# 1pathplanningzzj/pointnet_refine

Hardware: AMD Instinct MI355X
Metric: lane segments/sec (fwd+bwd) at B=4096,N=1024; HBM GB/s vs roofline (higher is better)
Workload: dtype f32 (large GEMMs: 2xfp16-split MFMA, 3 products, fp32 accumulate); 1 GPU; LineRefineNet training step (fwd + deep-supervision L1 + bwd + Adam), B=4096/GPU, N=1024, M=32, C=4; global_batch=4096, points=1024, parallelism=dp1, decoder_chunk=4096

## Files before the change

### include/pointnet_refine_hip.h

```cpp
#ifndef POINTNET_REFINE_HIP_H
#define POINTNET_REFINE_HIP_H

#include <stddef.h>
#include <stdint.h>

#ifdef __cplusplus
extern "C" {
#endif

#define PRH_OK 0
#define PRH_ERR_ARG (-1)
#define PRH_ERR_WORKSPACE (-2)
#define PRH_ERR_HIP (-3)

#define PRH_MAX_LAYERS 8

typedef struct {
  const float* w;
  const float* b;
  const float* gamma;
  const float* beta;
  float* running_mean;
  float* running_var;
  int64_t* num_batches_tracked;
// ... 47 lines not shown
                         int training, float* d_fused, const float* d_gfeat, int d_fused_scratch,
                         const prh_encoder_saved* saved, const prh_encoder_grads* grads,
                         float* d_ctx, void* workspace, size_t workspace_bytes, int device,
                         void* stream);

typedef struct {
  uint16_t* z_cat;
  uint16_t* z_fus;
  uint16_t* gate;
  float* bn_scale;
  float* bn_shift;
  float* bn_mean;
  float* bn_rstd;
  int32_t* argmax;
} prh_encoder_saved_bf16;
size_t prh_encoder_bf16_workspace_bytes(int B, int N, int in_channel, int out_dim, int backward);
int prh_encoder_forward_bf16(const prh_encoder_params* prm, const float* ctx, int B, int N, int training,
                             float momentum, float eps, uint16_t* fused, float* gfeat,
                             const prh_encoder_saved_bf16* saved, void* workspace, size_t workspace_bytes,
                             int device, void* stream);
int prh_encoder_backward_bf16(const prh_encoder_params* prm, const float* ctx, int B, int N, int training,
                              const uint16_t* d_fused, const float* d_gfeat, const prh_encoder_saved_bf16* saved,
                              const prh_encoder_grads* grads, float* d_ctx, void* workspace,
                              size_t workspace_bytes, int device, void* stream);
size_t prh_linear_bf16_workspace_bytes(int rows, int k, int n, int backward);
int prh_linear_forward_bf16(const uint16_t* x, long ldx, const float* w, const float* b, float* y, int rows, int k,
                            int n, int relu, void* workspace, size_t workspace_bytes, int device, void* stream);
int prh_linear_backward_bf16(const uint16_t* x, long ldx, const float* w, const float* dy, uint16_t* dx, float* dw,
                             float* db, int rows, int k, int n, void* workspace, size_t workspace_bytes, int device,
                             void* stream);

int prh_cast_perm_bf16(const float* src, long ld, uint16_t* dst, long rows, int device, void* stream);
int prh_posmem_images(const float* xyz, long ldx, const float* w0, const float* b0, const float* w2, const float* b2,
                      const float* memory, long ldm, long rows, uint16_t* x16, uint16_t* y16, int device, void* stream);
int prh_attn_fold_forward(const float* q, long ldq, const uint16_t* x16, const uint16_t* y16, const float* wk, long ldwk,
                          const float* wv, long ldwv, const float* bv, float* o, long ldo, int B, int M, int N, int H,
                          float scale, int device, void* stream);
int prh_linear_forward_out16(const float* x, long ldx, const float* w, const float* b, uint16_t* y, int rows, int k,
                             int n, void* workspace, size_t workspace_bytes, int device, void* stream);
int prh_linear_backward_dy16(const float* x, long ldx, const float* w, const uint16_t* dy, float* dx, float* dw,
                             float* db, int rows, int k, int n, void* workspace, size_t workspace_bytes, int device,
                             void* stream);
int prh_attn_forward_kv16(const float* q, long ldq, const uint16_t* k, long ldk, const uint16_t* v, long ldv, float* o,
                          long ldo, float* lse, int B, int M, int N, int H, float scale, float dropout_p,
                          unsigned seed, int device, void* stream);
int prh_attn_backward_kv16(const float* q, long ldq, const uint16_t* k, long ldk, const uint16_t* v, long ldv,
                           const float* o, long ldo, const float* lse, const float* dout, long lddo, float* dq,
                           long lddq, uint16_t* dk, long lddk, uint16_t* dv, long lddv, int B, int M, int N, int H,
                           float scale, float dropout_p, unsigned seed, int device, void* stream);

size_t prh_encoder_fused_image_bytes(int planes, int in_channel);
int prh_encoder_fused_prepare(const prh_encoder_params* prm, float eps, const float* proj_w, const float* proj_b,
                              int planes, void* image, size_t image_bytes, int device, void* stream);
size_t prh_encoder_fused_workspace_bytes(int B, int N, int planes);
int prh_encoder_fused_forward(const void* image, int planes, int in_channel, int has_proj, const float* ctx, int B,
                              int N, float* memory, float* fused, float* gfeat, unsigned* saturated, void* workspace,
                              size_t workspace_bytes, int device, void* stream);

size_t prh_linear_forward_workspace_bytes(int rows, int k, int n);
int prh_linear_forward(const float* x, long ldx, const float* w, const float* b, float* y,
                       int rows, int k, int n, int relu, void* workspace, size_t workspace_bytes,
                       int device, void* stream);

int prh_linear_forward_ex(const float* x, long ldx, const float* w, const float* b, float* y,
                          int rows, int k, int n, int relu, const float* x_amax, void* workspace,
                          size_t workspace_bytes, int device, void* stream);

int prh_linear_forward_full(const float* x, long ldx, const float* w, const float* b, const float* resid,
                            long ldres, float* y, int rows, int k, int n, int relu, const float* x_amax,
                            const float* w_amax, float dropout_p, unsigned dropout_seed, void* workspace,
                            size_t workspace_bytes, int device, void* stream);

int prh_linear_forward_amax(const float* x, long ldx, const float* w, const float* b, const float* resid,
                            long ldres, float* y, int rows, int k, int n, int relu, const float* x_amax,
                            const float* w_amax, float dropout_p, unsigned dropout_seed, float* y_amax_out,
                            void* workspace, size_t workspace_bytes, int device, void* stream);

size_t prh_operand_absmax_workspace_bytes(void);
int prh_operand_absmax(const float* x, long ld, long rows, int cols, float* out, void* workspace,
                       size_t workspace_bytes, int device, void* stream);
int prh_relu_mask_absmax(const float* dy, const float* y, float* out, long n, float scale, float* amax_out,
                         void* workspace, size_t workspace_bytes, int device, void* stream);
int prh_linear_uses_operand_maxima(int rows, int k, int n);

int prh_pos_hidden_forward(const float* xyz, long ld, const float* w0, const float* b0, float* h,
                           long rows, int hidden, int device, void* stream);
size_t prh_pos_hidden_forward_workspace_bytes(void);
int prh_pos_hidden_forward_amax(const float* xyz, long ld, const float* w0, const float* b0, float* h,
                                long rows, int hidden, float* h_amax_out, void* workspace, size_t workspace_bytes,
                                int device, void* stream);
size_t prh_pos_hidden_backward_workspace_bytes(long rows, int hidden);
int prh_pos_hidden_backward(const float* xyz, long ld, const float* h, const float* dh, const float* w0,
                            float* dxyz, float* dw0, float* db0, long rows, int hidden, void* workspace,
                            size_t workspace_bytes, int device, void* stream);

int prh_linear_small_forward(const float* x, const float* w, const float* b, float* y, long rows, int k,
                             int n, int device, void* stream);
size_t prh_linear_small_backward_workspace_bytes(long rows, int k, int n);
int prh_linear_small_backward(const float* x, const float* w, const float* dy, float* dx, float* dw,
                              float* db, long rows, int k, int n, void* workspace, size_t workspace_bytes,
                              int device, void* stream);

size_t prh_linear_backward_workspace_bytes(int rows, int k, int n);
int prh_linear_backward(const float* x, long ldx, const float* w, const float* dy, float* dx,
                        float* dw, float* db, int rows, int k, int n, void* workspace,
                        size_t workspace_bytes, int device, void* stream);

int prh_linear_backward_ex(const float* x, long ldx, const float* w, const float* dy, float* dx,
                           float* dw, float* db, int rows, int k, int n, const float* x_amax,
                           const float* dy_amax, void* workspace, size_t workspace_bytes, int device,
                           void* stream);
int prh_linear_backward_full(const float* x, long ldx, const float* w, const float* dy, float* dx,
                             float* dw, float* db, int rows, int k, int n, const float* x_amax,
                             const float* dy_amax, const float* w_amax, void* workspace,
                             size_t workspace_bytes, int device, void* stream);
int prh_linear_backward_amax(const float* x, long ldx, const float* w, const float* dy, float* dx,
                             float* dw, float* db, int rows, int k, int n, const float* x_amax,
                             const float* dy_amax, const float* w_amax, int dx_accumulate, float* dx_amax_out,
                             void* workspace, size_t workspace_bytes, int device, void* stream);

size_t prh_mlp_stack_workspace_bytes(int P, int n_layers, const prh_bn_layer* layers);
int prh_mlp_stack_forward(const prh_bn_layer* layers, int n_layers, int relu_last,
                          const float* x, int P, int training, float momentum, float eps,
                          float* z_cat, float* y, float* bn_scale, float* bn_shift,
                          float* bn_mean, float* bn_rstd, void* workspace,
                          size_t workspace_bytes, int device, void* stream);
int prh_mlp_stack_backward(const prh_bn_layer* layers, int n_layers, int relu_last,
                           const float* x, int P, int training, const float* dy,
                           const float* z_cat, const float* bn_scale, const float* bn_shift,
                           const float* bn_mean, const float* bn_rstd,
                           const prh_bn_layer_grad* grads, float* dx, void* workspace,
                           size_t workspace_bytes, int device, void* stream);

int prh_attn_forward(const float* q, long ldq, const float* k, long ldk, const float* v, long ldv,
                     float* o, long ldo, float* lse, int B, int M, int N, int H, float scale,
                     float dropout_p, unsigned seed, int device, void* stream);
int prh_attn_backward(const float* q, long ldq, const float* k, long ldk, const float* v, long ldv,
                      const float* o, long ldo, const float* lse, const float* dout, long lddo,
                      float* dq, long lddq, float* dk, long lddk, float* dv, long lddv, int B, int M,
                      int N, int H, float scale, float dropout_p, unsigned seed, int device,
                      void* stream);

size_t prh_context_workspace_bytes(int npts, int n_lines, int max_candidates);
int prh_context_build(const float* cloud, int npts, const float* dense, int n_dense, const float* line,
                      int m, int n_lines, float radius, float decay_scale, int n_samples,
                      int max_candidates, unsigned long long seed, float* out, int32_t* counts,
                      float* dbg_weights, void* workspace, size_t workspace_bytes, int device,
                      void* stream);

size_t prh_context_ragged_workspace_bytes(int n_lines, long long n_items);
int prh_context_ragged_count(const float* points, const long long* slice_offsets, int n_slices, const float* dense,
                             int n_dense, const int* line_slice, const unsigned long long* slice_seed, int n_lines,
                             float radius, int32_t* counts, long long* cand_offsets, void* workspace,
                             size_t workspace_bytes, int device, void* stream);
int prh_context_ragged_select(const float* points, const long long* slice_offsets, int n_slices, const float* dense,
                              int n_dense, const float* line, int m, const int* line_slice, int n_lines, float radius,
                              float decay_scale, int n_samples, const int32_t* counts, const long long* cand_offsets,
                              int line0, int line1, int* cand, unsigned* keys, long long cand_capacity, float* out,
                              void* workspace, size_t workspace_bytes, int device, void* stream);

int prh_line_metrics(const double* noisy, const double* refined, int n_lines, int m, const double* gt,
                     const long long* gt_offsets, int n_gt, const int* gt_index, int* info, double* resampled,
                     double* metrics, int device, void* stream);
size_t prh_shift_sweep_workspace_bytes(int n_pred, int n_gt, int n_shifts);
int prh_shift_sweep(const double* pred, int n_pred, const double* gt, int n_gt, const double* shifts, int n_shifts,
                    double* out, void* workspace, size_t workspace_bytes, int device, void* stream);

size_t prh_shift_sweep_ragged_workspace_bytes(const long long* pred_offsets, const long long* shift_offsets,
                                              int n_problems);
int prh_shift_sweep_ragged(const double* pred, const long long* pred_offsets, const double* gt,
                           const long long* gt_offsets, int n_gt_sets, const int* gt_index, const double* shifts,
                           const long long* shift_offsets, int n_problems, double* out, void* workspace,
                           size_t workspace_bytes, int device, void* stream);

size_t prh_drive_slice_workspace_bytes(int npts, int n_slices);
int prh_drive_slice_count(const float* cloud, int npts, const double* poses, int n_slices, double segment_len,
                          double radius, long long* offsets, void* workspace, size_t workspace_bytes, int device,
                          void* stream);
int prh_drive_slice_write(const float* cloud, int npts, const double* poses, int n_slices, double segment_len,
                          double radius, const long long* offsets, double* points, long long* source_index,
                          long long capacity, void* workspace, size_t workspace_bytes, int device, void* stream);
size_t prh_drive_clip_workspace_bytes(int n_slices);
int prh_drive_clip_count(const double* lines, const long long* line_offsets, int n_lines, const double* poses,
                         int n_slices, double segment_len, int* counts, void* workspace, size_t workspace_bytes,
                         int device, void* stream);
int prh_drive_clip_write(const double* lines, const long long* line_offsets, int n_lines, const double* poses,
                         int n_slices, double segment_len, const long long* out_offsets, double* out,
                         void* workspace, size_t workspace_bytes, int device, void* stream);
size_t prh_drive_noise_workspace_bytes(int n_lines);
int prh_drive_noise(const double* lines, const long long* line_offsets, const int* vertex_line, long long n_verts,
                    int n_lines, const int* line_ids, const double* scales, int n_scales, unsigned long long seed,
                    int draw, double* draws_u, double* draws_j, double* out, void* workspace,
                    size_t workspace_bytes, int device, void* stream);

int prh_pcd_group_rows(void);
size_t prh_pcd_format_workspace_bytes(long long n_rows);
int prh_pcd_format_count(const void* points, int is_fp64, long long n_rows, unsigned char* row_bytes,
                         int* group_bytes, long long* status, void* workspace, size_t workspace_bytes, int device,
                         void* stream);
int prh_pcd_format_write(const void* points, int is_fp64, long long n_rows, const unsigned char* row_bytes,
                         const long long* group_offsets, const long long* offsets, int n_slices,
                         unsigned char* text, long long capacity, long long* byte_offsets, int device,
// ... 178 lines not shown
```

### pointnet_refine_amd/_lib.py

```python
from __future__ import annotations

import ctypes as C
import os
import subprocess
import threading

_HERE = os.path.dirname(os.path.abspath(__file__))
_ROOT = os.path.dirname(_HERE)
LIB_PATH = os.environ.get("PRH_LIB_PATH") or os.path.join(_HERE, "libpointnet_refine_hip.so")
_CSRC = os.path.join(_HERE, "csrc")
_SOURCES = [os.path.join(_CSRC, "prh_lib.hip")] + (sorted(
    os.path.join(_CSRC, f) for f in os.listdir(_CSRC) if f.endswith((".hpp", ".h", ".hip")) and f != "prh_lib.hip")
    if os.path.isdir(_CSRC) else [])
_HEADER = os.path.join(_ROOT, "include", "pointnet_refine_hip.h")

PRH_MAX_LAYERS = 8


class BnLayer(C.Structure):
    _fields_ = [("w", C.c_void_p), ("b", C.c_void_p), ("gamma", C.c_void_p), ("beta", C.c_void_p),
                ("running_mean", C.c_void_p), ("running_var", C.c_void_p),
                ("num_batches_tracked", C.c_void_p), ("cin", C.c_int), ("cout", C.c_int)]


class BnLayerGrad(C.Structure):
    _fields_ = [("dw", C.c_void_p), ("db", C.c_void_p), ("dgamma", C.c_void_p), ("dbeta", C.c_void_p)]


class EncoderParams(C.Structure):
    _fields_ = [("in_channel", C.c_int), ("out_dim", C.c_int), ("conv", BnLayer * 5),
                ("fusion", BnLayer), ("gate_w1", C.c_void_p), ("gate_b1", C.c_void_p),
                ("gate_w2", C.c_void_p), ("gate_b2", C.c_void_p)]


class EncoderGrads(C.Structure):
    _fields_ = [("conv", BnLayerGrad * 5), ("fusion", BnLayerGrad), ("d_gate_w1", C.c_void_p),
                ("d_gate_b1", C.c_void_p), ("d_gate_w2", C.c_void_p), ("d_gate_b2", C.c_void_p)]


class EncoderSaved(C.Structure):
    _fields_ = [("z_cat", C.c_void_p), ("z_fus", C.c_void_p), ("gate", C.c_void_p),
                ("bn_scale", C.c_void_p), ("bn_shift", C.c_void_p), ("bn_mean", C.c_void_p),
                ("bn_rstd", C.c_void_p), ("argmax", C.c_void_p), ("op_amax", C.c_void_p)]


class EncoderSavedBf16(C.Structure):
    _fields_ = [("z_cat", C.c_void_p), ("z_fus", C.c_void_p), ("gate", C.c_void_p),
                ("bn_scale", C.c_void_p), ("bn_shift", C.c_void_p), ("bn_mean", C.c_void_p),
                ("bn_rstd", C.c_void_p), ("argmax", C.c_void_p)]


EXPORTS = [
    "prh_encoder_workspace_bytes", "prh_encoder_forward", "prh_encoder_backward",
    "prh_encoder_bf16_workspace_bytes", "prh_encoder_forward_bf16", "prh_encoder_backward_bf16",
    "prh_linear_bf16_workspace_bytes", "prh_linear_forward_bf16", "prh_linear_backward_bf16",
    "prh_linear_forward_out16", "prh_linear_backward_dy16", "prh_attn_forward_kv16", "prh_attn_backward_kv16",
    "prh_encoder_fused_image_bytes", "prh_encoder_fused_prepare", "prh_encoder_fused_workspace_bytes",
    "prh_encoder_fused_forward",
    "prh_linear_forward_workspace_bytes", "prh_linear_forward", "prh_linear_forward_ex",
    "prh_linear_forward_full", "prh_linear_forward_amax", "prh_operand_absmax_workspace_bytes", "prh_operand_absmax",
    "prh_linear_uses_operand_maxima", "prh_linear_backward_full", "prh_linear_backward_amax", "prh_pos_hidden_forward",
    "prh_pos_hidden_forward_workspace_bytes", "prh_pos_hidden_forward_amax", "prh_pos_hidden_backward_workspace_bytes",
    "prh_pos_hidden_backward", "prh_linear_small_forward", "prh_linear_small_backward_workspace_bytes",
    "prh_linear_small_backward",
    "prh_linear_backward_workspace_bytes", "prh_linear_backward", "prh_linear_backward_ex",
    "prh_mlp_stack_workspace_bytes", "prh_mlp_stack_forward", "prh_mlp_stack_backward",
    "prh_test_gemm_nt", "prh_test_gemm_tn_workspace_bytes", "prh_test_gemm_tn",
    "prh_test_gemm_tn_side_workspace_bytes", "prh_test_gemm_tn_side", "prh_test_xcc_map",
    "prh_profile_enable", "prh_profile_count", "prh_profile_reset", "prh_profile_read",
    "prh_attn_forward", "prh_attn_backward", "prh_attn_backward_ex",
    "prh_context_workspace_bytes", "prh_context_build",
    "prh_context_ragged_workspace_bytes", "prh_context_ragged_count", "prh_context_ragged_select",
    "prh_line_metrics", "prh_shift_sweep_workspace_bytes", "prh_shift_sweep",
    "prh_shift_sweep_ragged_workspace_bytes", "prh_shift_sweep_ragged",
    "prh_drive_slice_workspace_bytes", "prh_drive_slice_count", "prh_drive_slice_write",
    "prh_drive_clip_workspace_bytes", "prh_drive_clip_count", "prh_drive_clip_write",
    "prh_drive_noise_workspace_bytes", "prh_drive_noise",
    "prh_match_clip_workspace_bytes", "prh_match_clip_count", "prh_match_clip_write",
    "prh_match_costs_workspace_bytes", "prh_match_costs", "prh_match_max_side", "prh_match_assign",
    "prh_bev_bounds_workspace_bytes", "prh_bev_bounds", "prh_bev_raster", "prh_bev_select_workspace_bytes",
    "prh_bev_select", "prh_bev_tone", "prh_bev_colorize", "prh_bev_crop", "prh_bev_tile", "prh_bev_draw_count",
    "prh_bev_draw_workspace_bytes", "prh_bev_draw",
    "prh_view_bounds_workspace_bytes", "prh_view_bounds", "prh_view_clear", "prh_view_max_views", "prh_view_splat",
    "prh_view_lines", "prh_view_resolve",
    "prh_fuse_max_points", "prh_fuse_tile", "prh_fuse_project_workspace_bytes", "prh_fuse_project",
    "prh_fuse_gather_workspace_bytes", "prh_fuse_gather",
    "prh_link_tile", "prh_link_pairs_per_block", "prh_link_pairs_workspace_bytes", "prh_link_pairs_count",
    "prh_link_pairs_write", "prh_link_stats",
    "prh_link_cum", "prh_link_edges_blocks", "prh_link_edges", "prh_link_edges_compact", "prh_link_label_round",
    "prh_link_tree_init", "prh_link_tree_level",
    "prh_support_max_cells", "prh_support_accumulate",
    "prh_pcd_group_rows", "prh_pcd_format_workspace_bytes", "prh_pcd_format_count", "prh_pcd_format_write",
    "prh_pcd_index_blocks", "prh_pcd_index_count", "prh_pcd_index_write", "prh_pcd_parse_workspace_bytes",
    "prh_pcd_parse", "prh_pcd_unpack14",
    "prh_l1_loss_workspace_bytes", "prh_l1_loss", "prh_adam_step",
    "prh_add_dropout_layernorm_forward", "prh_add_dropout_layernorm_workspace_bytes",
    "prh_add_dropout_layernorm_backward",
    "prh_relu_mask_absmax", "prh_cast_perm_bf16", "prh_posmem_images", "prh_attn_fold_forward", "prh_set_gemm_mode", "prh_get_gemm_mode", "prh_set_dropout_seed_source",
    "prh_last_error", "prh_version",
]

_lock = threading.Lock()
_lib = None


def needs_build() -> bool:
    if not os.path.exists(LIB_PATH):
        return True
    t = os.path.getmtime(LIB_PATH)
    return any(os.path.exists(s) and os.path.getmtime(s) > t for s in _SOURCES + [_HEADER])


def build(force: bool = False, verbose: bool = False) -> str:
    if not force and not needs_build():
        return LIB_PATH
    hipcc = os.environ.get("HIPCC", "/opt/rocm/bin/hipcc")
    cmd = [hipcc, "--offload-arch=gfx950", "-O3", "-std=c++17", "-shared", "-fPIC",
           "-o", LIB_PATH, _SOURCES[0]]
    if verbose:
        print(" ".join(cmd))
    subprocess.run(cmd, check=True)
    return LIB_PATH


def _bind(lib):
    vp, i, f, sz, lg = C.c_void_p, C.c_int, C.c_float, C.c_size_t, C.c_long
    lib.prh_last_error.restype = C.c_char_p
    lib.prh_version.restype = C.c_char_p
    lib.prh_encoder_workspace_bytes.restype = sz
    lib.prh_encoder_workspace_bytes.argtypes = [i, i, i, i, i]
    lib.prh_encoder_forward.restype = i
    lib.prh_encoder_forward.argtypes = [C.POINTER(EncoderParams), vp, i, i, i, f, f, vp, vp,
                                        C.POINTER(EncoderSaved), vp, sz, i, vp]
    lib.prh_encoder_backward.restype = i
    lib.prh_encoder_backward.argtypes = [C.POINTER(EncoderParams), vp, i, i, i, vp, vp, i,
                                         C.POINTER(EncoderSaved), C.POINTER(EncoderGrads), vp, vp,
                                         sz, i, vp]
    lib.prh_encoder_bf16_workspace_bytes.restype = sz
    lib.prh_encoder_bf16_workspace_bytes.argtypes = [i, i, i, i, i]
    lib.prh_encoder_forward_bf16.restype = i
    lib.prh_encoder_forward_bf16.argtypes = [C.POINTER(EncoderParams), vp, i, i, i, f, f, vp, vp,
                                             C.POINTER(EncoderSavedBf16), vp, sz, i, vp]
    lib.prh_encoder_backward_bf16.restype = i
    lib.prh_encoder_backward_bf16.argtypes = [C.POINTER(EncoderParams), vp, i, i, i, vp, vp,
                                              C.POINTER(EncoderSavedBf16), C.POINTER(EncoderGrads), vp, vp,
                                              sz, i, vp]
    lib.prh_linear_bf16_workspace_bytes.restype = sz
    lib.prh_linear_bf16_workspace_bytes.argtypes = [i, i, i, i]
    lib.prh_linear_forward_bf16.restype = i
    lib.prh_linear_forward_bf16.argtypes = [vp, lg, vp, vp, vp, i, i, i, i, vp, sz, i, vp]
    lib.prh_linear_backward_bf16.restype = i
    lib.prh_linear_backward_bf16.argtypes = [vp, lg, vp, vp, vp, vp, vp, i, i, i, vp, sz, i, vp]
    lib.prh_linear_forward_out16.restype = i
    lib.prh_linear_forward_out16.argtypes = [vp, lg, vp, vp, vp, i, i, i, vp, sz, i, vp]
    lib.prh_linear_backward_dy16.restype = i
    lib.prh_linear_backward_dy16.argtypes = [vp, lg, vp, vp, vp, vp, vp, i, i, i, vp, sz, i, vp]
    lib.prh_attn_forward_kv16.restype = i
    lib.prh_attn_forward_kv16.argtypes = [vp, lg, vp, lg, vp, lg, vp, lg, vp, i, i, i, i, f, f, C.c_uint, i, vp]
    lib.prh_attn_backward_kv16.restype = i
    lib.prh_attn_backward_kv16.argtypes = [vp, lg, vp, lg, vp, lg, vp, lg, vp, vp, lg, vp, lg, vp, lg, vp, lg,
                                           i, i, i, i, f, f, C.c_uint, i, vp]
    lib.prh_encoder_fused_image_bytes.restype = sz
    lib.prh_encoder_fused_image_bytes.argtypes = [i, i]
    lib.prh_encoder_fused_prepare.restype = i
    lib.prh_encoder_fused_prepare.argtypes = [C.POINTER(EncoderParams), f, vp, vp, i, vp, sz, i, vp]
    lib.prh_encoder_fused_workspace_bytes.restype = sz
    lib.prh_encoder_fused_workspace_bytes.argtypes = [i, i, i]
    lib.prh_encoder_fused_forward.restype = i
    lib.prh_encoder_fused_forward.argtypes = [vp, i, i, i, vp, i, i, vp, vp, vp, vp, vp, sz, i, vp]
    lib.prh_linear_forward.restype = i
    lib.prh_linear_forward.argtypes = [vp, lg, vp, vp, vp, i, i, i, i, vp, sz, i, vp]
    lib.prh_linear_forward_ex.restype = i
    lib.prh_linear_forward_ex.argtypes = [vp, lg, vp, vp, vp, i, i, i, i, vp, vp, sz, i, vp]
    lib.prh_linear_forward_full.restype = i
    lib.prh_linear_forward_full.argtypes = [vp, lg, vp, vp, vp, lg, vp, i, i, i, i, vp, vp, f, C.c_uint, vp, sz, i, vp]
    lib.prh_linear_forward_amax.restype = i
    lib.prh_linear_forward_amax.argtypes = [vp, lg, vp, vp, vp, lg, vp, i, i, i, i, vp, vp, f, C.c_uint, vp, vp, sz, i, vp]
    lib.prh_linear_backward_amax.restype = i
    lib.prh_linear_backward_amax.argtypes = [vp, lg, vp, vp, vp, vp, vp, i, i, i, vp, vp, vp, i, vp, vp, sz, i, vp]
    lib.prh_pos_hidden_forward_workspace_bytes.restype = sz
    lib.prh_pos_hidden_forward_workspace_bytes.argtypes = []
    lib.prh_pos_hidden_forward_amax.restype = i
    lib.prh_pos_hidden_forward_amax.argtypes = [vp, lg, vp, vp, vp, lg, i, vp, vp, sz, i, vp]
    lib.prh_operand_absmax_workspace_bytes.restype = sz
    lib.prh_operand_absmax_workspace_bytes.argtypes = []
    lib.prh_operand_absmax.restype = i
    lib.prh_operand_absmax.argtypes = [vp, lg, lg, i, vp, vp, sz, i, vp]
    lib.prh_linear_uses_operand_maxima.restype = i
    lib.prh_linear_uses_operand_maxima.argtypes = [i, i, i]
    lib.prh_linear_backward_full.restype = i
    lib.prh_linear_backward_full.argtypes = [vp, lg, vp, vp, vp, vp, vp, i, i, i, vp, vp, vp, vp, sz, i, vp]
    lib.prh_pos_hidden_forward.restype = i
    lib.prh_pos_hidden_forward.argtypes = [vp, lg, vp, vp, vp, lg, i, i, vp]
    lib.prh_pos_hidden_backward_workspace_bytes.restype = sz
    lib.prh_pos_hidden_backward_workspace_bytes.argtypes = [lg, i]
    lib.prh_pos_hidden_backward.restype = i
    lib.prh_pos_hidden_backward.argtypes = [vp, lg, vp, vp, vp, vp, vp, vp, lg, i, vp, sz, i, vp]
    lib.prh_linear_small_forward.restype = i
    lib.prh_linear_small_forward.argtypes = [vp, vp, vp, vp, lg, i, i, i, vp]
    lib.prh_linear_small_backward_workspace_bytes.restype = sz
    lib.prh_linear_small_backward_workspace_bytes.argtypes = [lg, i, i]
    lib.prh_linear_small_backward.restype = i
    lib.prh_linear_small_backward.argtypes = [vp, vp, vp, vp, vp, vp, lg, i, i, vp, sz, i, vp]
    lib.prh_linear_backward_ex.restype = i
    lib.prh_linear_backward_ex.argtypes = [vp, lg, vp, vp, vp, vp, vp, i, i, i, vp, vp, vp, sz, i, vp]
    lib.prh_linear_forward_workspace_bytes.restype = sz
    lib.prh_linear_forward_workspace_bytes.argtypes = [i, i, i]
    lib.prh_linear_backward_workspace_bytes.restype = sz
    lib.prh_linear_backward_workspace_bytes.argtypes = [i, i, i]
    lib.prh_linear_backward.restype = i
    lib.prh_linear_backward.argtypes = [vp, lg, vp, vp, vp, vp, vp, i, i, i, vp, sz, i, vp]
    lib.prh_mlp_stack_workspace_bytes.restype = sz
    lib.prh_mlp_stack_workspace_bytes.argtypes = [i, i, C.POINTER(BnLayer)]
    lib.prh_mlp_stack_forward.restype = i
    lib.prh_mlp_stack_forward.argtypes = [C.POINTER(BnLayer), i, i, vp, i, i, f, f, vp, vp, vp, vp,
                                          vp, vp, vp, sz, i, vp]
    lib.prh_mlp_stack_backward.restype = i
    lib.prh_mlp_stack_backward.argtypes = [C.POINTER(BnLayer), i, i, vp, i, i, vp, vp, vp, vp, vp,
                                           vp, C.POINTER(BnLayerGrad), vp, vp, sz, i, vp]
    lib.prh_attn_forward.restype = i
    lib.prh_attn_forward.argtypes = [vp, lg, vp, lg, vp, lg, vp, lg, vp, i, i, i, i, f, f, C.c_uint, i, vp]
    lib.prh_attn_backward.restype = i
    lib.prh_attn_backward.argtypes = [vp, lg, vp, lg, vp, lg, vp, lg, vp, vp, lg, vp, lg, vp, lg, vp, lg,
                                      i, i, i, i, f, f, C.c_uint, i, vp]
    lib.prh_context_workspace_bytes.restype = C.c_size_t
    lib.prh_context_workspace_bytes.argtypes = [i, i, i]
    lib.prh_context_build.restype = i
    lib.prh_context_build.argtypes = [vp, i, vp, i, vp, i, i, f, f, i, i, C.c_ulonglong, vp, vp, vp, vp,
                                      C.c_size_t, i, vp]
    lib.prh_context_ragged_workspace_bytes.restype = sz
    lib.prh_context_ragged_workspace_bytes.argtypes = [i, C.c_longlong]
    lib.prh_context_ragged_count.restype = i
    lib.prh_context_ragged_count.argtypes = [vp, vp, i, vp, i, vp, vp, i, f, vp, vp, vp, sz, i, vp]
    lib.prh_context_ragged_select.restype = i
    lib.prh_context_ragged_select.argtypes = [vp, vp, i, vp, i, vp, i, vp, i, f, f, i, vp, vp, i, i, vp, vp,
                                              C.c_longlong, vp, vp, sz, i, vp]
    lib.prh_line_metrics.restype = i
    lib.prh_line_metrics.argtypes = [vp, vp, i, i, vp, vp, i, vp, vp, vp, vp, i, vp]
    lib.prh_shift_sweep_workspace_bytes.restype = sz
    lib.prh_shift_sweep_workspace_bytes.argtypes = [i, i, i]
    lib.prh_shift_sweep.restype = i
    lib.prh_shift_sweep.argtypes = [vp, i, vp, i, vp, i, vp, vp, sz, i, vp]
    lib.prh_shift_sweep_ragged_workspace_bytes.restype = sz
    lib.prh_shift_sweep_ragged_workspace_bytes.argtypes = [vp, vp, i]
    lib.prh_shift_sweep_ragged.restype = i
    lib.prh_shift_sweep_ragged.argtypes = [vp, vp, vp, vp, i, vp, vp, vp, i, vp, vp, sz, i, vp]
    ll, dbl = C.c_longlong, C.c_double
    lib.prh_drive_slice_workspace_bytes.restype = sz
    lib.prh_drive_slice_workspace_bytes.argtypes = [i, i]
    lib.prh_drive_slice_count.restype = i
    lib.prh_drive_slice_count.argtypes = [vp, i, vp, i, dbl, dbl, vp, vp, sz, i, vp]
    lib.prh_drive_slice_write.restype = i
    lib.prh_drive_slice_write.argtypes = [vp, i, vp, i, dbl, dbl, vp, vp, vp, ll, vp, sz, i, vp]
    lib.prh_drive_clip_workspace_bytes.restype = sz
    lib.prh_drive_clip_workspace_bytes.argtypes = [i]
    lib.prh_drive_clip_count.restype = i
    lib.prh_drive_clip_count.argtypes = [vp, vp, i, vp, i, dbl, vp, vp, sz, i, vp]
    lib.prh_drive_clip_write.restype = i
    lib.prh_drive_clip_write.argtypes = [vp, vp, i, vp, i, dbl, vp, vp, vp, sz, i, vp]
    lib.prh_drive_noise_workspace_bytes.restype = sz
    lib.prh_drive_noise_workspace_bytes.argtypes = [i]
    lib.prh_drive_noise.restype = i
# ... 188 lines not shown
```

### pointnet_refine_amd/csrc/prh_gemm.hpp

```cpp
#pragma once
#include <hip/hip_runtime.h>
#include <type_traits>
#include <stdint.h>

namespace prh {

typedef float f32x16 __attribute__((ext_vector_type(16)));

enum { PRO_NONE = 0, PRO_BNRELU = 1, PRO_BNBWD = 2, PRO_GATE1 = 3 };
enum { EPI_BIAS = 0, EPI_BIAS_STATS = 1, EPI_GATE = 2, EPI_DGRAD = 3 };

enum {
  F_RELU_OUT = 1,
  F_ACCUM = 2,
  F_MASK = 4,
  F_STATS = 8,
  F_STORE_GATE = 16,
  F_E1_ROWVEC = 32,
  F_RESID = 64,
  F_DROPOUT = 256,
  F_POOL = 128,
};

struct NTParams {
// ... 271 lines not shown
                                              int mrows, int rb, int lane, const float* biasp) {
  const int q = lane >> 4, l15 = lane & 15;
#pragma unroll
  for (int nb = 0; nb < 4; ++nb) {
    const int col = cbase + nb * 16 + l15;
    const bool cok = col < p.N;
    const float bias = (biasp != nullptr && cok) ? biasp[col] : 0.f;
    float s = 0.f;
#pragma unroll
    for (int mb = 0; mb < MB; ++mb)
#pragma unroll
      for (int r = 0; r < 4; ++r)
        if (mb * 16 + q * 4 + r < mrows) s += acc[mb][nb][r] + bias;
    s += __shfl_xor(s, 16);
    s += __shfl_xor(s, 32);
    const int nrows = mrows < 0 ? 0 : (mrows > MB * 16 ? MB * 16 : mrows);
    const float mean = nrows > 0 ? s / (float)nrows : 0.f;
    float m2 = 0.f;
#pragma unroll
    for (int mb = 0; mb < MB; ++mb)
#pragma unroll
      for (int r = 0; r < 4; ++r) {
        const float dlt = acc[mb][nb][r] + bias - mean;
        if (mb * 16 + q * 4 + r < mrows) m2 = fmaf(dlt, dlt, m2);
      }
    m2 += __shfl_xor(m2, 16);
    m2 += __shfl_xor(m2, 32);
    if (q == 0 && cok) {
      p.ws_a[(size_t)rb * p.N + col] = s;
      p.ws_b[(size_t)rb * p.N + col] = m2;
    }
    if (p.ws_c != nullptr) {
      float mx = -3.0e38f, mn = 3.0e38f;
#pragma unroll
      for (int mb = 0; mb < MB; ++mb)
#pragma unroll
        for (int r = 0; r < 4; ++r)
          if (mb * 16 + q * 4 + r < mrows) {
            mx = fmaxf(mx, acc[mb][nb][r] + bias); mn = fminf(mn, acc[mb][nb][r] + bias);
          }
      mx = fmaxf(fmaxf(mx, __shfl_xor(mx, 16)), 0.f - 3.0e38f);
      mx = fmaxf(mx, __shfl_xor(mx, 32));
      mn = fminf(mn, __shfl_xor(mn, 16));
      mn = fminf(mn, __shfl_xor(mn, 32));
      if (q == 0 && cok) {
        p.ws_c[(size_t)rb * p.N + col] = mx;
        p.ws_d[(size_t)rb * p.N + col] = mn;
      }
    }
  }
}

__device__ __forceinline__ unsigned pack_bf16x2(float a, float b) {
  typedef float v2f __attribute__((ext_vector_type(2)));
  typedef __bf16 v2b __attribute__((ext_vector_type(2)));
  v2f v = {a, b};
  v2b h = __builtin_convertvector(v, v2b);
  return __builtin_bit_cast(unsigned, h);
}
__device__ __forceinline__ float bf16_lo(unsigned u) { return __uint_as_float(u << 16); }
__device__ __forceinline__ float bf16_hi(unsigned u) { return __uint_as_float(u & 0xffff0000u); }
__device__ __forceinline__ float bf16_round(float x) { return bf16_lo(pack_bf16x2(x, 0.f)); }
template <bool H>
__device__ __forceinline__ float4 ld4e(const char* base, int off) {
  if (H) {
    const uint2 u = *reinterpret_cast<const uint2*>(base + (size_t)off * 2);
    return make_float4(bf16_lo(u.x), bf16_hi(u.x), bf16_lo(u.y), bf16_hi(u.y));
  }
  return *reinterpret_cast<const float4*>(base + (size_t)off * 4);
}
template <bool H>
__device__ __forceinline__ void st4e(char* base, int off, float4 v) {
  if (H) *reinterpret_cast<uint2*>(base + (size_t)off * 2) = make_uint2(pack_bf16x2(v.x, v.y), pack_bf16x2(v.z, v.w));
  else *reinterpret_cast<float4*>(base + (size_t)off * 4) = v;
}

typedef char* __restrict__ epi_wptr_r;
typedef const char* __restrict__ epi_rptr_r;
template <int EPI, int MT, class ACC, bool C16, bool AMAX = false>
__device__ __forceinline__ void nt_epilogue_vec_r2(ACC& acc, const NTParams& p, int rbase_,
                                                int cbase, int rb, int lane, float* scratch,
                                                bool bias_done = false,
                                                float* wave_amax = nullptr) {
  static_assert(!AMAX || (EPI == EPI_BIAS && !C16), "output maximum: EPI_BIAS with fp32 storage");
  typedef typename std::conditional<AMAX, char*, epi_wptr_r>::type wptr;
  typedef typename std::conditional<AMAX, const char*, epi_rptr_r>::type rptr;
  const int rbase = __builtin_amdgcn_readfirstlane(rbase_);
  const float* biasp = bias_done ? nullptr : p.bias;
  constexpr int ES = C16 ? 2 : 4;
  const bool rowvec = EPI == EPI_DGRAD && (p.flags & F_E1_ROWVEC) != 0;
  const int ees = (C16 && !rowvec) ? 2 : 4;
  wptr Cb = reinterpret_cast<char*>(p.C) + (size_t)rbase * p.ldc * ES;
  rptr Eb = p.E1 != nullptr ? reinterpret_cast<const char*>(p.E1) + (size_t)rbase * p.lde1 * ees : nullptr;
  const int ldc = (int)p.ldc, lde1 = (int)p.lde1;
  const int mrows = p.M - rbase;
  const int rr = lane >> 4, c4 = (lane & 15) * 4;
  const int col4 = cbase + c4;
  const bool c4ok = col4 < p.N;
  float4 bias4 = zero4(), es4 = zero4(), et4 = zero4();
  if (c4ok) {
    if (biasp != nullptr) bias4 = ldg4(biasp + col4);
    if ((EPI == EPI_DGRAD && (p.flags & F_MASK) != 0) || EPI == EPI_GATE) {
      es4 = ldg4(p.es + col4);
      et4 = ldg4(p.et + col4);
    }
  }
  char* __restrict__ C2b = (EPI == EPI_GATE && p.C2 != nullptr) ? reinterpret_cast<char*>(p.C2) + (size_t)rbase * p.ldc2 * ES : nullptr;
  const int ldc2 = (int)p.ldc2;

  if (EPI == EPI_BIAS_STATS) epi_col_stats(acc, p, cbase, mrows, rb, lane, biasp);

  const bool mask = (p.flags & F_MASK) != 0, accum = (p.flags & F_ACCUM) != 0;
  const bool stats = EPI == EPI_DGRAD && (p.flags & F_STATS) != 0;
  const bool resid = EPI == EPI_BIAS && (p.flags & F_RESID) != 0;
  const unsigned dseed = (EPI == EPI_BIAS && (p.flags & F_DROPOUT) != 0) ? epi_seed(p) : 0u;
  const bool need_z = (EPI == EPI_DGRAD && (mask || stats)) || EPI == EPI_GATE || resid;
  float4 s1 = zero4(), s2 = zero4();
  const bool pool = EPI == EPI_GATE && (p.flags & F_POOL) != 0;
  float pmx[4] = {-1.f, -1.f, -1.f, -1.f}, psm[4] = {0.f, 0.f, 0.f, 0.f};
  int pix[4] = {0, 0, 0, 0};
  const int col4c = col4 < p.N ? col4 : (p.N - 4);
  rptr Cl = mrows > 0 ? Cb : reinterpret_cast<const char*>(p.C);
  rptr El = mrows > 0 ? Eb : reinterpret_cast<const char*>(p.E1);
  const bool acc_old = EPI == EPI_DGRAD && accum;
  float amx = 0.f;
  constexpr int NB = 2 * MT;
  float4 zz[2][4], oo[2][4];
  auto issue = [&](int b, float4 (&z)[4], float4 (&o)[4]) {
    const char* Em = El; const char* Cm = Cl;
    asm volatile("" : "+s"(Em), "+s"(Cm) : : "memory");
    int lrc[4];
#pragma unroll
    for (int i = 0; i < 4; ++i) {
      z[i] = zero4(); o[i] = zero4();
      int r = (b >> 1) * 32 + ((b & 1) * 4 + i) * 4 + rr;
      r = r < mrows ? r : mrows - 1;
      lrc[i] = r < 0 ? 0 : r;
    }
    if (need_z) {
      if (rowvec) {
#pragma unroll
        for (int i = 0; i < 4; ++i) {
          const float s = *reinterpret_cast<const float*>(Em + (size_t)(lrc[i] * lde1) * 4);
          z[i] = make_float4(s, s, s, s);
        }
      } else {
#pragma unroll
        for (int i = 0; i < 4; ++i) z[i] = ld4e<C16>(Em, lrc[i] * lde1 + col4c);
      }
    }
    if (acc_old) {
#pragma unroll
      for (int i = 0; i < 4; ++i) o[i] = ld4e<C16>(Cm, lrc[i] * ldc + col4c);
    }
  };
  issue(0, zz[0], oo[0]);
#pragma unroll
  for (int b = 0; b < NB; ++b) {
    const int mt = b >> 1, hb = b & 1;
    if (b + 1 < NB) issue(b + 1, zz[(b + 1) & 1], oo[(b + 1) & 1]);
    if (hb == 0) epi_block_to_scratch(acc, mt, scratch, lane);
#pragma unroll
    for (int i = 0; i < 4; ++i) {
      const int it = hb * 4 + i;
      const int lrow = it * 4 + rr;
      const int lr = mt * 32 + lrow;
      const bool ok = lr < mrows && c4ok;
      float4 v = *reinterpret_cast<const float4*>(scratch + lrow * EPI_LDW + c4);
      v.x += bias4.x; v.y += bias4.y; v.z += bias4.z; v.w += bias4.w;
      const float4 z = zz[b & 1][i];
      const float4 o = oo[b & 1][i];
      if (EPI == EPI_DGRAD) {
        v.x += o.x; v.y += o.y; v.z += o.z; v.w += o.w;
        if (mask) {
          v.x = fmaf(z.x, es4.x, et4.x) > 0.f ? v.x : 0.f;
          v.y = fmaf(z.y, es4.y, et4.y) > 0.f ? v.y : 0.f;
          v.z = fmaf(z.z, es4.z, et4.z) > 0.f ? v.z : 0.f;
          v.w = fmaf(z.w, es4.w, et4.w) > 0.f ? v.w : 0.f;
        }
        if (C16) {
          v.x = bf16_round(v.x); v.y = bf16_round(v.y); v.z = bf16_round(v.z); v.w = bf16_round(v.w);
        }
        const float4 q = ok ? v : zero4();
        s1.x += q.x; s1.y += q.y; s1.z += q.z; s1.w += q.w;
        s2.x = fmaf(q.x, z.x, s2.x); s2.y = fmaf(q.y, z.y, s2.y);
        s2.z = fmaf(q.z, z.z, s2.z); s2.w = fmaf(q.w, z.w, s2.w);
      } else if (EPI == EPI_GATE) {
        float4 m;
        m.x = 0.5f + 0.5f / (1.f + __expf(-v.x)); m.y = 0.5f + 0.5f / (1.f + __expf(-v.y));
        m.z = 0.5f + 0.5f / (1.f + __expf(-v.z)); m.w = 0.5f + 0.5f / (1.f + __expf(-v.w));
        v.x = fmaxf(fmaf(z.x, es4.x, et4.x), 0.f) * m.x; v.y = fmaxf(fmaf(z.y, es4.y, et4.y), 0.f) * m.y;
        v.z = fmaxf(fmaf(z.z, es4.z, et4.z), 0.f) * m.z; v.w = fmaxf(fmaf(z.w, es4.w, et4.w), 0.f) * m.w;
        if (ok && (p.flags & F_STORE_GATE) != 0) st4e<C16>(C2b, lr * ldc2 + col4, m);
        if (pool && ok) {
          if (C16) { v.x = bf16_round(v.x); v.y = bf16_round(v.y); v.z = bf16_round(v.z); v.w = bf16_round(v.w); }
          const float vv[4] = {v.x, v.y, v.z, v.w};
#pragma unroll
          for (int e = 0; e < 4; ++e) {
            if (vv[e] > pmx[e]) { pmx[e] = vv[e]; pix[e] = lr; }
            psm[e] += vv[e];
          }
        }
      } else {
        if (resid) { v.x += z.x; v.y += z.y; v.z += z.z; v.w += z.w; }
        if ((p.flags & F_RELU_OUT) != 0) {
          v.x = fmaxf(v.x, 0.f); v.y = fmaxf(v.y, 0.f); v.z = fmaxf(v.z, 0.f); v.w = fmaxf(v.w, 0.f);
        }
        if (EPI == EPI_BIAS && (p.flags & F_DROPOUT) != 0) {
          const unsigned rw = (unsigned)(rbase + lr), c0 = (unsigned)col4;
          v.x = epi_keep(dseed, rw, c0, p.drop_thresh) ? v.x * p.drop_scale : 0.f;
          v.y = epi_keep(dseed, rw, c0 + 1, p.drop_thresh) ? v.y * p.drop_scale : 0.f;
          v.z = epi_keep(dseed, rw, c0 + 2, p.drop_thresh) ? v.z * p.drop_scale : 0.f;
          v.w = epi_keep(dseed, rw, c0 + 3, p.drop_thresh) ? v.w * p.drop_scale : 0.f;
        }
      }
      if (ok) st4e<C16>(Cb, lr * ldc + col4, v);
      if (AMAX && ok) amx = fmaxf(fmaxf(amx, fmaxf(fabsf(v.x), fabsf(v.y))), fmaxf(fabsf(v.z), fabsf(v.w)));
    }
    if (EPI == EPI_DGRAD)
      asm volatile("" : "+v"(s1.x), "+v"(s1.y), "+v"(s1.z), "+v"(s1.w), "+v"(s2.x), "+v"(s2.y), "+v"(s2.z), "+v"(s2.w));
  }
  if (pool) {
#pragma unroll
    for (int e = 0; e < 4; ++e)
#pragma unroll
      for (int o = 16; o <= 32; o <<= 1) {
        const float ov = __shfl_xor(pmx[e], o);
        const int oi = __shfl_xor(pix[e], o);
        psm[e] += __shfl_xor(psm[e], o);
        if (ov > pmx[e] || (ov == pmx[e] && oi < pix[e])) { pmx[e] = ov; pix[e] = oi; }
      }
    if (lane < 16 && c4ok) {
      *reinterpret_cast<float4*>(p.ws_a + (size_t)rb * p.N + col4) = make_float4(pmx[0], pmx[1], pmx[2], pmx[3]);
      *reinterpret_cast<float4*>(p.ws_b + (size_t)rb * p.N + col4) = make_float4(psm[0], psm[1], psm[2], psm[3]);
      *reinterpret_cast<int4*>(p.ws_c + (size_t)rb * p.N + col4) = make_int4(pix[0], pix[1], pix[2], pix[3]);
    }
  }
  if (stats) {
    s1.x += __shfl_xor(s1.x, 16); s1.y += __shfl_xor(s1.y, 16); s1.z += __shfl_xor(s1.z, 16); s1.w += __shfl_xor(s1.w, 16);
    s2.x += __shfl_xor(s2.x, 16); s2.y += __shfl_xor(s2.y, 16); s2.z += __shfl_xor(s2.z, 16); s2.w += __shfl_xor(s2.w, 16);
    s1.x += __shfl_xor(s1.x, 32); s1.y += __shfl_xor(s1.y, 32); s1.z += __shfl_xor(s1.z, 32); s1.w += __shfl_xor(s1.w, 32);
    s2.x += __shfl_xor(s2.x, 32); s2.y += __shfl_xor(s2.y, 32); s2.z += __shfl_xor(s2.z, 32); s2.w += __shfl_xor(s2.w, 32);
    if (lane < 16 && c4ok) {
      *reinterpret_cast<float4*>(p.ws_a + (size_t)rb * p.N + col4) = s1;
      *reinterpret_cast<float4*>(p.ws_b + (size_t)rb * p.N + col4) = s2;
    }
  }
  if (AMAX) {
#pragma unroll
    for (int o = 32; o > 0; o >>= 1) amx = fmaxf(amx, __shfl_xor(amx, o));
    *wave_amax = amx;
  }
}

template <int EPI, int MT, class ACC, bool C16 = false, bool AMAX = false>
__device__ __forceinline__ void nt_epilogue_vec(ACC& acc, const NTParams& p, int rbase_,
                                                int cbase, int rb, int lane, float* scratch,
                                                bool bias_done = false,
                                                float* wave_amax = nullptr) {
  if constexpr (!C16) {
    nt_epilogue_vec_r2<EPI, MT, ACC, false, AMAX>(acc, p, rbase_, cbase, rb, lane, scratch, bias_done, wave_amax);
    return;
  }
  const int rbase = __builtin_amdgcn_readfirstlane(rbase_);
  const float* biasp = bias_done ? nullptr : p.bias;
  constexpr int ES = C16 ? 2 : 4;
  const bool rowvec = EPI == EPI_DGRAD && (p.flags & F_E1_ROWVEC) != 0;
  const int ees = (C16 && !rowvec) ? 2 : 4;
  char* __restrict__ Cb = reinterpret_cast<char*>(p.C) + (size_t)rbase * p.ldc * ES;
  const char* __restrict__ Eb = p.E1 != nullptr ? reinterpret_cast<const char*>(p.E1) + (size_t)rbase * p.lde1 * ees : nullptr;
  const int ldc = (int)p.ldc, lde1 = (int)p.lde1;
  const int mrows = p.M - rbase;
  const int rr = lane >> 4, c4 = (lane & 15) * 4;
  const int col4 = cbase + c4;
  const bool c4ok = col4 < p.N;
  float4 bias4 = zero4(), es4 = zero4(), et4 = zero4();
  if (c4ok) {
    if (biasp != nullptr) bias4 = ldg4(biasp + col4);
    if ((EPI == EPI_DGRAD && (p.flags & F_MASK) != 0) || EPI == EPI_GATE) {
      es4 = ldg4(p.es + col4);
      et4 = ldg4(p.et + col4);
    }
  }
  char* __restrict__ C2b = (EPI == EPI_GATE && p.C2 != nullptr) ? reinterpret_cast<char*>(p.C2) + (size_t)rbase * p.ldc2 * ES : nullptr;
  const int ldc2 = (int)p.ldc2;

  if (EPI == EPI_BIAS_STATS) epi_col_stats(acc, p, cbase, mrows, rb, lane, biasp);

  const bool mask = (p.flags & F_MASK) != 0, accum = (p.flags & F_ACCUM) != 0;
  const bool stats = EPI == EPI_DGRAD && (p.flags & F_STATS) != 0;
  const bool resid = EPI == EPI_BIAS && (p.flags & F_RESID) != 0;
  const unsigned dseed = (EPI == EPI_BIAS && (p.flags & F_DROPOUT) != 0) ? epi_seed(p) : 0u;
  const bool need_z = (EPI == EPI_DGRAD && (mask || stats)) || EPI == EPI_GATE || resid;
  float4 s1 = zero4(), s2 = zero4();
  const bool pool = EPI == EPI_GATE && (p.flags & F_POOL) != 0;
  float pmx[4] = {-1.f, -1.f, -1.f, -1.f}, psm[4] = {0.f, 0.f, 0.f, 0.f};
  int pix[4] = {0, 0, 0, 0};
  const bool acc_old = EPI == EPI_DGRAD && accum;
  const int vrows = mrows < 0 ? 0 : (mrows > 32 * MT ? 32 * MT : mrows);
  auto mkrs = [&](const void* base, long ld, int es_, int width) {
    const long ext = (base != nullptr && vrows > 0) ? ((long)(vrows - 1) * ld + width) * es_ : 0;
    return __builtin_amdgcn_make_buffer_rsrc(const_cast<void*>(base), 0, (int)ext, 0x00020000);
// ... 402 lines not shown
```

### pointnet_refine_amd/csrc/prh_gemm_h2.hpp

```cpp
#pragma once
#include "prh_gemm_s3.hpp"

namespace prh {

constexpr int H2_BK = 32;
constexpr int H2_PLANE = 256 * H2_BK * 2;
constexpr int H2_OPER = 2 * H2_PLANE;
constexpr int H2_STAGE = 2 * H2_OPER;
constexpr int H2_LDS = 2 * H2_STAGE;

__device__ __forceinline__ int h2_off(int row, int k) {
  return row * 64 + ((((k >> 3) ^ (-(row >> 2))) & 3) << 4) + ((k & 7) << 1);
}

inline size_t h2_weight_bytes(int N, int K) {
  return S3_WHDR + (size_t)((N + 255) / 256) * ((K + H2_BK - 1) / H2_BK) * H2_OPER;
}

__global__ __launch_bounds__(256) void prep_weights_h2_kernel(const float* __restrict__ W, int N,
                                                              int K, long ldw, char* __restrict__ out,
                                                              const float* __restrict__ amax) {
  const int KT = (K + H2_BK - 1) / H2_BK;
  const int NT_ = (N + 255) / 256;
  const long total = (long)NT_ * 256 * KT * 4;
  const long i = (long)blockIdx.x * blockDim.x + threadIdx.x;
  if (i >= total) return;
  const int chunk = (int)(i & 3);
  long t = i >> 2;
  const int k_tile = (int)(t % KT); t /= KT;
  const int row = (int)(t & 255);
  const int n_tile = (int)(t >> 8);
  const int n = n_tile * 256 + row;
  const float S = pow2_scale(load_amax(amax));
  float v[8];
#pragma unroll
  for (int j = 0; j < 8; ++j) {
    const int k = k_tile * H2_BK + chunk * 8 + j;
    v[j] = (n < N && k < K) ? W[(size_t)n * ldw + k] * S : 0.f;
  }
  uint4 h, l;
  split2h(v[0], v[1], h.x, l.x);
  split2h(v[2], v[3], h.y, l.y);
  split2h(v[4], v[5], h.z, l.z);
  split2h(v[6], v[7], h.w, l.w);
  char* base = out + ((size_t)n_tile * KT + k_tile) * H2_OPER + h2_off(row, chunk * 8);
  *reinterpret_cast<uint4*>(base) = h;
  *reinterpret_cast<uint4*>(base + H2_PLANE) = l;
}

template <int I0 = 0, int I1 = 8>
__device__ __forceinline__ void h2_compute(f32x4 (&acc)[8][4], const char* st, int wm, int wn, int l15,
                                           int kc) {
  f16x8 wh[4], wl[4];
#pragma unroll
  for (int j = 0; j < 4; ++j) {
    const char* q = st + H2_OPER + h2_off(wn + j * 16 + l15, kc * 8);
    wh[j] = *reinterpret_cast<const f16x8*>(q);
    wl[j] = *reinterpret_cast<const f16x8*>(q + H2_PLANE);
  }
#pragma unroll
  for (int i = I0; i < I1; ++i) {
    const char* q = st + h2_off(wm + i * 16 + l15, kc * 8);
    const f16x8 ah = *reinterpret_cast<const f16x8*>(q);
    const f16x8 al = *reinterpret_cast<const f16x8*>(q + H2_PLANE);
#pragma unroll
    for (int j = 0; j < 4; ++j) {
      acc[i][j] = __builtin_amdgcn_mfma_f32_16x16x32_f16(al, wh[j], acc[i][j], 0, 0, 0);
      acc[i][j] = __builtin_amdgcn_mfma_f32_16x16x32_f16(ah, wl[j], acc[i][j], 0, 0, 0);
      acc[i][j] = __builtin_amdgcn_mfma_f32_16x16x32_f16(ah, wh[j], acc[i][j], 0, 0, 0);
    }
  }
}

template <int PRO, int EPI, bool PP = false, bool AMAX = false>
__global__ __launch_bounds__(512, 2) void gemm_nt_h2_kernel(const NTParams p,
                                                            const char* __restrict__ Wp) {
  static_assert(PRO == PRO_NONE || PRO == PRO_BNRELU || PRO == PRO_GATE1, "prologue not supported");
  static_assert(!AMAX || (PRO == PRO_NONE && EPI == EPI_BIAS), "output maximum: plain EPI_BIAS launches only");
  extern __shared__ __attribute__((aligned(16))) char smem[];
#ifdef PRH_STAMP
  unsigned t_acc[4] = {0u, 0u, 0u, 0u};
  unsigned long long t_prev = __builtin_amdgcn_s_memtime();
#endif
  const int tid = threadIdx.x, lane = tid & 63, wave = tid >> 6;
  const int l15 = lane & 15, kc = lane >> 4;
  const int wm = (wave >> 2) * 128, wn = (wave & 3) * 64;
  const int vb = xcd_remap(blockIdx.x, gridDim.x);
  const int tile_n = vb % p.tiles_n, tile_m = vb / p.tiles_n;
  const int m0 = tile_m * 256, n0 = tile_n * 256;
  const int KT = (p.K + H2_BK - 1) / H2_BK;

  const int sc = (tid & 7) * 4;
  const int sr = tid >> 3;
  const int KP = (KT + 2) * H2_BK;
  float* coef = reinterpret_cast<float*>(smem + H2_LDS);
  const float sA = pow2_scale(load_amax(p.amaxA));
  const float unscale = 1.f / (sA * pow2_scale(load_amax(p.amaxW)));

  f32x4 acc[8][4];
#pragma unroll
  for (int i = 0; i < 8; ++i)
#pragma unroll
    for (int j = 0; j < 4; ++j)
#pragma unroll
      for (int r = 0; r < 4; ++r) acc[i][j][r] = 0.f;

  float4 ra[2][4];
  const char* wsrc = Wp + (size_t)tile_n * KT * H2_OPER + tid * 16;
  const unsigned lds0 = (unsigned)(unsigned long)((__attribute__((address_space(3))) char*)smem);
  const unsigned wdst = __builtin_amdgcn_readfirstlane(lds0 + H2_OPER + wave * 1024);
  auto dma_w = [&](int kt, int stage) {
    const char* q = wsrc + (size_t)(kt < KT ? kt : KT - 1) * H2_OPER;
#pragma unroll
    for (int pc = 0; pc < 4; ++pc) glds16(q + pc * 8192, wdst + stage * H2_STAGE + pc * 8192);
  };
  constexpr int NA = PRO == PRO_GATE1 ? 0 : 4;
  int arows = p.M - m0; arows = arows > 256 ? 256 : arows;
  const __amdgpu_buffer_rsrc_t rsA = __builtin_amdgcn_make_buffer_rsrc(
      (void*)(p.A + (size_t)m0 * p.lda), 0,
      PRO == PRO_GATE1 ? 0 : (int)(((size_t)(arows - 1) * p.lda + p.K) * 4), 0x00020000);
  int voA[4];
  float gi[4] = {0.f, 0.f, 0.f, 0.f};
#pragma unroll
  for (int j = 0; j < 4; ++j) {
    voA[j] = ((sr + 64 * j) * (int)p.lda + sc) * 4;
    if (PRO == PRO_GATE1) {
      const int row = m0 + sr + 64 * j;
      gi[j] = row < p.M ? p.A[(size_t)row * p.lda] : 0.f;
    }
  }
  auto load_tile = [&](int kt, float4 (&r)[4]) {
    if (PRO == PRO_GATE1) return;
    const int so = kt * (H2_BK * 4);
#pragma unroll
    for (int j = 0; j < 4; ++j)
      r[j] = __builtin_bit_cast(float4, __builtin_amdgcn_raw_buffer_load_b128(rsA, voA[j] + so, 0, 0));
  };
  auto store_tile = [&](int kt, char* st, const float4 (&r_)[4]) {
    const int k = kt * H2_BK + sc;
    const bool kok = k < p.K || PRO != PRO_NONE;
    float4 ka = zero4(), kb = zero4();
    if (PRO != PRO_NONE) {
      ka = *reinterpret_cast<const float4*>(coef + k);
      kb = *reinterpret_cast<const float4*>(coef + KP + k);
    }
#pragma unroll
    for (int j = 0; j < 4; ++j) {
      const int r = sr + 64 * j;
      float4 v;
      if (PRO == PRO_GATE1) v = pro_apply<PRO>(make_float4(gi[j], 0.f, 0.f, 0.f), zero4(), ka, kb, zero4());
      else v = pro_apply<PRO>(r_[j], zero4(), ka, kb, zero4());
      v.x = kok ? v.x : 0.f; v.y = kok ? v.y : 0.f; v.z = kok ? v.z : 0.f; v.w = kok ? v.w : 0.f;
      if (PRO == PRO_NONE) { v.x *= sA; v.y *= sA; v.z *= sA; v.w *= sA; }
      uint2 h, l;
      split2h(v.x, v.y, h.x, l.x);
      split2h(v.z, v.w, h.y, l.y);
      char* q = st + h2_off(r, sc);
      *reinterpret_cast<uint2*>(q) = h;
      *reinterpret_cast<uint2*>(q + H2_PLANE) = l;
    }
  };
// ... 478 lines not shown
```

### pointnet_refine_amd/csrc/prh_kernels.hpp

```cpp
#pragma once
#include <hip/hip_runtime.h>
#include <stdint.h>

namespace prh {

constexpr int BN_SLICES = 32;

__global__ __launch_bounds__(256) void bn_stage1_kernel(const float* __restrict__ ws_a,
                                                        const float* __restrict__ ws_b, int R,
                                                        long ld, int N, int tile_rows, int P,
                                                        int forward, double* __restrict__ out) {
  __shared__ double red[3][8][33];
  const int c = threadIdx.x & 31, g = threadIdx.x >> 5;
  const int col = blockIdx.x * 32 + c, sl = blockIdx.y;
  const int per = (R + BN_SLICES - 1) / BN_SLICES;
  const int r0 = sl * per, r1 = (r0 + per < R) ? r0 + per : R;
  const bool ok = col < N;
  double a = 0.0, b = 0.0, n = 0.0;
  if (ok)
    for (int i = r0 + g; i < r1; i += 8) {
      a += (double)ws_a[(size_t)i * ld + col];
      if (forward) {
        int ni = P - i * tile_rows;
        ni = ni > tile_rows ? tile_rows : (ni < 0 ? 0 : ni);
// ... 62 lines not shown
    running_var[col] = (float)((1.0 - momentum) * (double)running_var[col] + momentum * unb);
  }
}

__global__ __launch_bounds__(256) void act_amax_kernel(const float* __restrict__ ws_c,
                                                       const float* __restrict__ ws_d, int R, long ld, int N,
                                                       const float* __restrict__ scale,
                                                       const float* __restrict__ shift,
                                                       float* __restrict__ part) {
  __shared__ float red[256];
  const int c = threadIdx.x & 31, g = threadIdx.x >> 5;
  const int sl = blockIdx.y;
  const int per = (R + BN_SLICES - 1) / BN_SLICES;
  const int r0 = sl * per, r1 = (r0 + per < R) ? r0 + per : R;
  float a = 0.f;
  for (int col = blockIdx.x * 32 + c; col < N; col += gridDim.x * 32) {
    float mx = -3.0e38f, mn = 3.0e38f;
    for (int i = r0 + g; i < r1; i += 8) {
      mx = fmaxf(mx, ws_c[(size_t)i * ld + col]);
      mn = fminf(mn, ws_d[(size_t)i * ld + col]);
    }
    if (mx >= mn) {
      const float sc = scale[col], sh = shift[col];
      a = fmaxf(a, fmaxf(fmaf(mx, sc, sh), fmaf(mn, sc, sh)));
    }
  }
  red[threadIdx.x] = a;
  __syncthreads();
  for (int s = 128; s > 0; s >>= 1) {
    if (threadIdx.x < s) red[threadIdx.x] = fmaxf(red[threadIdx.x], red[threadIdx.x + s]);
    __syncthreads();
  }
  if (threadIdx.x == 0) part[blockIdx.y * gridDim.x + blockIdx.x] = red[0];
}
__global__ void max_of_kernel(const float* __restrict__ v, int n, float* __restrict__ out) {
  float m = 0.f;
  for (int i = 0; i < n; ++i) m = fmaxf(m, v[i]);
  *out = m;
}

__global__ void bn_eval_coeffs_kernel(const float* gamma, const float* beta, const float* rm,
                                      const float* rv, float eps, int N, float* mean_out,
                                      float* rstd_out, float* scale_out, float* shift_out) {
  const int c = blockIdx.x * blockDim.x + threadIdx.x;
  if (c >= N) return;
  const float rstd = 1.0f / sqrtf(rv[c] + eps);
  const float sc = gamma[c] * rstd;
  mean_out[c] = rm[c];
  rstd_out[c] = rstd;
  scale_out[c] = sc;
  shift_out[c] = beta[c] - rm[c] * sc;
}

__global__ void bn_bwd_finalize_kernel(const double* __restrict__ sl, int P, int N,
                                       const float* __restrict__ gamma,
                                       const float* __restrict__ mean,
                                       const float* __restrict__ rstd, int training, float* ca,
                                       float* cb, float* cc, float* dgamma, float* dbeta,
                                       float* dbias) {
  const int col = blockIdx.x * blockDim.x + threadIdx.x;
  if (col >= N) return;
  double Sdy = 0.0, Sdyz = 0.0;
  for (int s = 0; s < BN_SLICES; ++s) {
    const double* r = sl + ((size_t)s * 3) * N;
    Sdy += r[col];
    Sdyz += r[(size_t)N + col];
  }
  const double mu = mean[col], rs = rstd[col], gm = gamma[col];
  const double dg = (Sdyz - mu * Sdy) * rs;
  if (dgamma != nullptr) dgamma[col] = (float)dg;
  if (dbeta != nullptr) dbeta[col] = (float)Sdy;
  double a = gm * rs, b = 0.0, cst = 0.0;
  if (training) {
    const double m1 = Sdy / (double)P, m2 = dg / (double)P;
    b = -a * m2 * rs;
    cst = a * (m2 * mu * rs - m1);
  }
  ca[col] = (float)a;
  cb[col] = (float)b;
  cc[col] = (float)cst;
  if (dbias != nullptr) dbias[col] = (float)(a * Sdy + b * (double)P * mu + cst * (double)P);
}

__global__ __launch_bounds__(1024) void partials_reduce_kernel(
    const float* __restrict__ ws_a, const float* __restrict__ ws_b, int R2, int N, float* out_a,
    float* out_b) {
  __shared__ double red[2][32][33];
  const int c = threadIdx.x & 31, g = threadIdx.x >> 5;
  const int col = blockIdx.x * 32 + c;
  const bool ok = col < N;
  double s1 = 0.0, s2 = 0.0;
  if (ok)
    for (int i = g; i < R2; i += 32) {
      s1 += (double)ws_a[(size_t)i * N + col];
      if (ws_b != nullptr) s2 += (double)ws_b[(size_t)i * N + col];
    }
  red[0][g][c] = s1;
  red[1][g][c] = s2;
  __syncthreads();
  if (g == 0 && ok) {
    double a = 0.0, b = 0.0;
    for (int j = 0; j < 32; ++j) {
      a += red[0][j][c];
      b += red[1][j][c];
    }
    if (out_a != nullptr) out_a[col] = (float)a;
    if (out_b != nullptr) out_b[col] = (float)b;
  }
}

__global__ __launch_bounds__(256) void pool_kernel(const float* __restrict__ F, int N, int C,
                                                   float* gfeat, int32_t* argmax) {
  __shared__ float smax[4][64];
  __shared__ int sidx[4][64];
  __shared__ float ssum[4][64];
  const int c = threadIdx.x & 63, g = threadIdx.x >> 6;
  const int col = blockIdx.x * 64 + c, b = blockIdx.y;
  float mx = -INFINITY, sum = 0.f;
  int ix = 0;
  if (col < C) {
    const float* base = F + (size_t)b * N * C + col;
    for (int n = g; n < N; n += 4) {
      const float v = base[(size_t)n * C];
      sum += v;
      if (v > mx) { mx = v; ix = n; }
    }
  }
  smax[g][c] = mx; sidx[g][c] = ix; ssum[g][c] = sum;
  __syncthreads();
  if (g == 0 && col < C) {
    for (int j = 1; j < 4; ++j) {
      const float v = smax[j][c];
      const int i2 = sidx[j][c];
      if (v > mx || (v == mx && i2 < ix)) { mx = v; ix = i2; }
      sum += ssum[j][c];
    }
    gfeat[(size_t)b * 2 * C + col] = mx;
    gfeat[(size_t)b * 2 * C + C + col] = sum / (float)N;
    if (argmax != nullptr) argmax[(size_t)b * C + col] = ix;
  }
}

__global__ __launch_bounds__(256) void pool_tiles_kernel(const float* __restrict__ pmax,
                                                         const float* __restrict__ psum,
                                                         const int* __restrict__ pidx, int tiles_per_seg,
                                                         int N, int C, float* gfeat, int32_t* argmax) {
  const int col = blockIdx.x * 256 + threadIdx.x, b = blockIdx.y;
  if (col >= C) return;
  float mx = -INFINITY, sum = 0.f;
  int ix = 0;
  for (int t = 0; t < tiles_per_seg; ++t) {
    const size_t o = ((size_t)b * tiles_per_seg + t) * C + col;
    const float v = pmax[o];
    if (v > mx) { mx = v; ix = t * 128 + pidx[o]; }
    sum += psum[o];
  }
  gfeat[(size_t)b * 2 * C + col] = mx;
  gfeat[(size_t)b * 2 * C + C + col] = sum / (float)N;
  if (argmax != nullptr) argmax[(size_t)b * C + col] = ix;
}

__global__ __launch_bounds__(256) void combine_bwd_kernel(
    const float* dF, const float* __restrict__ d_gfeat, const int32_t* __restrict__ argmax,
    const float* __restrict__ zf, float* gate, const float* __restrict__ s,
    const float* __restrict__ t, int P, int N, int C, float* dy_out, float* ws_a, float* ws_b) {
  __shared__ float r1[4][64], r2[4][64];
  const int c = threadIdx.x & 63, g = threadIdx.x >> 6;
  const int col = blockIdx.y * 64 + c;
  const int row0 = blockIdx.x * 64 + g * 16;
  float s1 = 0.f, s2 = 0.f;
  if (col < C) {
    const float sc = s[col], sh = t[col];
    for (int i = 0; i < 16; ++i) {
      const int row = row0 + i;
      if (row >= P) break;
      const size_t off = (size_t)row * C + col;
      float d = dF != nullptr ? dF[off] : 0.f;
      if (d_gfeat != nullptr) {
// ... 613 lines not shown
```

### pointnet_refine_amd/csrc/prh_lib.hip

```cpp
#include "../../include/pointnet_refine_hip.h"

#include <hip/hip_runtime.h>
#include <stdarg.h>
#include <stdio.h>
#include <string.h>

#include <mutex>
#include <vector>

#include <stdlib.h>

#include "prh_gemm.hpp"
#include "prh_attn.hpp"
#include "prh_attn16.hpp"
#include "prh_gemm_s3.hpp"
#include "prh_gemm_h2.hpp"
#include "prh_b16.hpp"
#include "prh_small.hpp"
#include "prh_attnfold.hpp"
#include "prh_fused.hpp"
#include "prh_context.hpp"
#include "prh_metrics.hpp"
#include "prh_drive.hpp"
#include "prh_match.hpp"
// ... 55 lines not shown
    r = &g_prof.recs[g_prof.used++];
    snprintf(r->name, sizeof(r->name), "%s", name);
    r->flops = flops; r->bytes = bytes;
    (void)hipEventRecord(r->e0, st);
  }
  ~ProfScope() { if (r) (void)hipEventRecord(r->e1, st); }
};

inline size_t align_up(size_t x, size_t a) { return (x + a - 1) / a * a; }
inline int cdiv(long a, long b) { return (int)((a + b - 1) / b); }

struct Arena {
  char* base; size_t size; size_t off = 0; bool ok = true;
  Arena(void* b, size_t s) : base((char*)b), size(s) {}
  Arena() : base(nullptr), size((size_t)-1) {}
  float* f(size_t n) {
    off = align_up(off, 256);
    const size_t bytes = n * sizeof(float);
    if (base != nullptr && off + bytes > size) { ok = false; return nullptr; }
    float* p = base ? (float*)(base + off) : nullptr;
    off += bytes;
    return p;
  }
};

const unsigned* g_seed_src = nullptr;
int g_gemm_mode = -1;
inline int gemm_mode() {
  if (g_gemm_mode < 0) {
    const char* e = getenv("PRH_GEMM");
    g_gemm_mode = PRH_GEMM_DEFAULT;
    if (e != nullptr && strcmp(e, "fp32") == 0) g_gemm_mode = 0;
    else if (e != nullptr && strcmp(e, "split") == 0) g_gemm_mode = 1;
    else if (e != nullptr && strcmp(e, "bf16op") == 0) g_gemm_mode = 2;
    else if (e != nullptr && strcmp(e, "split16") == 0) g_gemm_mode = 3;
    else if (e != nullptr && (strcmp(e, "bf16") == 0 || strcmp(e, "bf16s") == 0)) g_gemm_mode = 4;
  }
  return g_gemm_mode;
}
struct Cores {
  int mode, core;
  bool split() const { return core != 0; }
  int attn_prec() const { return mode == 0 ? -1 : 0; }
  const char* tag() const { return core == 2 ? "b1" : (core == 3 ? "h2" : "s3"); }
};
inline Cores cores_of(int mode) { return Cores{mode, mode == 4 ? 2 : mode}; }
inline Cores stack_cores(int mode) { return mode == 4 ? Cores{4, 3} : cores_of(mode); }
bool g_h2_pp = [] { const char* e = getenv("PRH_H2_PP"); return e && strcmp(e, "1") == 0; }();

template <int PRO>
int measure_absmax(const float* A, long lda, const float* A2, long lda2, const float* pa,
                   const float* pb, const float* pc, long rows, int cols, float* slot, float* part,
                   hipStream_t st) {
  if (rows <= 0 || cols <= 0) {
    hipLaunchKernelGGL(absmax_final_kernel, dim3(1), dim3(256), 0, st, part, 0, slot);
    LAUNCH_CHECK();
    return PRH_OK;
  }
  const int vec = ((cols & 3) == 0 && (PRO == PRO_GATE1 || (lda & 3) == 0) &&
                   (PRO != PRO_BNBWD || (lda2 & 3) == 0)) ? 1 : 0;
  long blocks = cdiv(rows, 4L * 8);
  blocks = blocks < 1 ? 1 : (blocks > ABSMAX_MAX_BLOCKS ? ABSMAX_MAX_BLOCKS : blocks);
  hipLaunchKernelGGL((absmax_kernel<PRO>), dim3((unsigned)blocks), dim3(256), 0, st, A, lda, A2, lda2,
                     pa, pb, pc, rows, cols, vec, part);
  LAUNCH_CHECK();
  hipLaunchKernelGGL(absmax_final_kernel, dim3(1), dim3(256), 0, st, part, (int)blocks, slot);
  LAUNCH_CHECK();
  return PRH_OK;
}
inline bool nt_use_s3(Cores c, int M, int N, int K) {
  return c.split() && K >= 64 && K <= 4096 && N >= 128 && M >= 512 &&
         (long)cdiv(M, S3_BM) * cdiv(N, S3_BN) >= 32;
}
inline bool tn_use_s3(Cores c, int P, int Mo, int Ni) { return c.split() && Mo >= 128 && Ni >= 64 && P >= 8192; }

int materialize_dz(float* dy, long lddy, const float* z, long ldz, const float* ka, const float* kb,
                   const float* kc, long rows, int cols, float* hdr, hipStream_t st) {
  long blocks = cdiv(rows, 4L * 8);
  blocks = blocks < 1 ? 1 : (blocks > ABSMAX_MAX_BLOCKS ? ABSMAX_MAX_BLOCKS : blocks);
  hipLaunchKernelGGL(bn_bwd_apply_kernel, dim3((unsigned)blocks), dim3(256), 0, st, dy, lddy, z, ldz, ka,
                     kb, kc, rows, cols, hdr + 64);
  LAUNCH_CHECK();
  hipLaunchKernelGGL(absmax_final_kernel, dim3(1), dim3(256), 0, st, hdr + 64, (int)blocks, hdr);
  LAUNCH_CHECK();
  return PRH_OK;
}
inline bool dz_in_place(Cores c, int cols, long lddy, long ldz) {
  return c.core == 3 && (cols & 3) == 0 && (lddy & 3) == 0 && (ldz & 3) == 0;
}

struct StatInfo { int count = 0; int rows = 64; long ld = 0; long off = 0; };
inline int stat_tiles_max(int P) { return 2 * cdiv(P, BM); }

template <typename K, typename... More>
int allow_big_lds(K kernel, More... more) {
  HIP_TRY(hipFuncSetAttribute(reinterpret_cast<const void*>(kernel),
                              hipFuncAttributeMaxDynamicSharedMemorySize, 160 * 1024));
  if constexpr (sizeof...(more) > 0) return allow_big_lds(more...);
  else return PRH_OK;
}
inline size_t nt_s3_lds(int K, int pro) {
  const int KP = (cdiv(K, S3_BK) + 2) * S3_BK;
  return (size_t)S3_LDS + (pro == PRO_NONE ? 0 : (pro == PRO_BNBWD ? 3 : 2) * (size_t)KP * 4);
}
template <int PRO, int EPI, int PLANES>
void launch_nt_s3(const NTParams& p, long tiles, const char* img, hipStream_t st) {
  hipLaunchKernelGGL((gemm_nt_s3_kernel<PRO, EPI, PLANES>), dim3((unsigned)tiles), dim3(512), nt_s3_lds(p.K, PRO), st, p, img);
}
template <int PROA, int PROB, int PLANES>
void launch_tn_s3(const TNParams& p, long blocks, hipStream_t st) {
  hipLaunchKernelGGL((gemm_tn_s3_kernel<PROA, PROB, PLANES>), dim3((unsigned)blocks), dim3(512), S3_LDS, st, p);
}
static_assert(8 * 32 * EPI_LDW * 4 <= S3_LDS, "epilogue scratch must fit in the stage buffers");

template <int PRO, int EPI, bool A16, bool C16>
int launch_nt_b16(NTParams& p, hipStream_t st, StatInfo* si = nullptr) {
  if (p.M <= 0 || p.N <= 0) return PRH_OK;
  const bool rowvec = (p.flags & F_E1_ROWVEC) != 0;
  if ((p.K & 7) || (PRO != PRO_GATE1 && (p.lda & (A16 ? 7 : 3))) || (p.ldw & 3) || (p.N & 3) || (p.ldc & 3) ||
      (p.E1 != nullptr && !rowvec && (p.lde1 & 3)) || (p.C2 != nullptr && (p.ldc2 & 3)) || p.wprep == nullptr)
    return fail(PRH_ERR_ARG, "gemm_nt_b16: K %% 8, N %% 4 and aligned leading dimensions required (K=%d N=%d lda=%ld ldc=%ld)",
                p.K, p.N, p.lda, p.ldc);
  if (rowvec && C16) return fail(PRH_ERR_ARG, "gemm_nt_b16: a row-vector E1 comes with fp32 outputs");
  const int KT = cdiv(p.K, B16_BK), NTl = cdiv(p.N, 256);
  const size_t lds = (size_t)H2_LDS + (PRO == PRO_NONE ? 0 : 2 * (size_t)(KT + 2) * B16_BK * 4);
  if (lds > 160 * 1024) return fail(PRH_ERR_ARG, "gemm_nt_b16: K=%d too deep for the prologue coefficient image", p.K);
  const long th = (long)NTl * 256 * KT * 8;
  hipLaunchKernelGGL(prep_weights_b16_kernel, dim3((unsigned)cdiv(th, 256)), dim3(256), 0, st, p.W, p.N, p.K, p.ldw,
                     p.wprep + S3_WHDR);
  LAUNCH_CHECK();
  p.tiles_n = NTl;
  static const int attr = allow_big_lds(gemm_nt_b16_kernel<PRO, EPI, A16, C16>);
  if (attr != PRH_OK) return attr;
  char nm[64];
  snprintf(nm, sizeof(nm), "gemm_nt_b16<%d,%d> K=%d N=%d", PRO, EPI, p.K, p.N);
  const double ea = A16 ? 2.0 : 4.0, ec = C16 ? 2.0 : 4.0;
  const double by = ea * (double)p.M * p.K * (PRO == PRO_GATE1 ? 0 : 1) +
                    ec * (double)p.M * p.N * (EPI == EPI_GATE ? 3 : (EPI == EPI_DGRAD ? 2 : 1)) + 4.0 * (double)p.N * p.K;
  ProfScope ps(nm, 2.0 * p.M * (double)p.N * p.K, by, st);
  if constexpr (PRO == PRO_NONE && A16) {
    if ((p.K % B16_BK) == 0 && (reinterpret_cast<uintptr_t>(p.A) & 15) == 0) {
      static const int attr_d = allow_big_lds(gemm_nt_b16d_kernel<EPI, C16>);
      if (attr_d != PRH_OK) return attr_d;
      hipLaunchKernelGGL((gemm_nt_b16d_kernel<EPI, C16>), dim3((unsigned)(NTl * cdiv(p.M, 256))), dim3(512), (size_t)B16D_LDS, st,
                         p, (const char*)(p.wprep + S3_WHDR));
      LAUNCH_CHECK();
      if (si) { si->count = 2 * cdiv(p.M, 256); si->rows = 128; }
      return PRH_OK;
    }
  }
  hipLaunchKernelGGL((gemm_nt_b16_kernel<PRO, EPI, A16, C16>), dim3((unsigned)(NTl * cdiv(p.M, 256))), dim3(512), lds, st,
                     p, (const char*)(p.wprep + S3_WHDR));
  LAUNCH_CHECK();
  if (si) { si->count = 2 * cdiv(p.M, 256); si->rows = 128; }
  return PRH_OK;
}
inline bool nt_b16_generic_ok(const NTParams& p) {
  return p.wprep != nullptr && (p.K & 7) == 0 && p.K >= 64 && p.K <= 8192 && (p.lda & 3) == 0 && (p.N & 3) == 0 &&
         (p.ldc & 3) == 0 && (p.E1 == nullptr || (p.lde1 & 3) == 0) && p.M >= 512 && p.N >= 64 &&
         (long)cdiv(p.M, 256) * cdiv(p.N, 256) >= 16;
}

struct TNPlan16 { int tiles_m, tiles_n, splits, rows_per_split; };
inline TNPlan16 tn_plan_b16(int P, int Mo, int Ni, long maxld) {
  TNPlan16 pl;
  pl.tiles_m = cdiv(Mo, 256); pl.tiles_n = cdiv(Ni, 256);
// ... 84 lines not shown
  p.tiles_n = cdiv(p.N, TN * 32);
  const long tiles = (long)p.tiles_n * cdiv(p.M, TM * 32);
  char nm[64];
  snprintf(nm, sizeof(nm), "gemm_small<%d%d%d,%s,%d> K=%d N=%d", TM, TN, KS, NN ? "nn" : "nt", EPI, p.K, p.N);
  const double by = 4.0 * ((double)p.M * p.K + (double)p.M * p.N * ((p.flags & F_RESID) || EPI == EPI_DGRAD ? 2 : 1) + (double)p.N * p.K);
  ProfScope ps(nm, 2.0 * p.M * (double)p.N * p.K, by, st);
  hipLaunchKernelGGL((gemm_small_kernel<TM, TN, KS, NN, EPI>), dim3((unsigned)tiles), dim3(256), (small_lds<TM, TN, KS>()), st, p);
  LAUNCH_CHECK();
  return PRH_OK;
}
template <bool NN, int EPI = EPI_BIAS>
int launch_small(NTParams& p, hipStream_t st) {
  p.flags &= ~F_POOL;
  const bool n64 = !NN || (p.N & 63) == 0;
  if (n64 && (long)cdiv(p.M, 64) * cdiv(p.N, 64) >= 192) return launch_small_cfg<2, 2, 1, NN, EPI>(p, st);
  if (n64 && (long)cdiv(p.M, 32) * cdiv(p.N, 64) >= 192) return launch_small_cfg<1, 2, 2, NN, EPI>(p, st);
  return launch_small_cfg<1, 1, 4, NN, EPI>(p, st);
}
constexpr int TN_SMALL_MAX_P = 16384;
inline bool small_tn_dims_ok(int P, int Mo, int Ni) {
  return P >= 64 && P <= TN_SMALL_MAX_P && (P & 63) == 0 && (Mo & 63) == 0 && (Ni & 63) == 0;
}
inline void small_tn_plan(int P, int Mo, int Ni, int& splits, int& rps) {
  const int tiles = (Mo / 64) * (Ni / 64), chunks = P / 64;
  int s = cdiv(512, tiles);
  s = s > chunks ? chunks : (s < 1 ? 1 : s);
  rps = cdiv(chunks, s) * 64;
  splits = cdiv(P, rps);
}

inline size_t nt_amax_part_floats(int M, int N) {
  const size_t t = (size_t)cdiv(M < 1 ? 1 : M, S3_BM) * cdiv(N < 1 ? 1 : N, S3_BN);
  return (t > (size_t)ABSMAX_MAX_BLOCKS ? t : (size_t)ABSMAX_MAX_BLOCKS) + 64;
}
template <int PRO, int EPI>
int launch_nt_core(Cores c, NTParams& p, hipStream_t st, StatInfo* si, float* amax_part, long* amax_tiles) {
  if (p.M <= 0 || p.N <= 0) return PRH_OK;
  if ((p.K & 3) || (PRO != PRO_GATE1 && (p.lda & 3)) || (p.ldw & 3) ||
      (PRO == PRO_BNBWD && (p.lda2 & 3)))
    return fail(PRH_ERR_ARG, "gemm_nt: K/lda/ldw must be multiples of 4 (K=%d lda=%ld ldw=%ld)",
                p.K, p.lda, p.ldw);
  if constexpr (PRO == PRO_NONE && EPI == EPI_BIAS) {
    if (c.mode == 4 && c.core == 2 && nt_b16_generic_ok(p)) return launch_nt_b16<PRO_NONE, EPI_BIAS, false, false>(p, st, si);
  }
  const bool want_pool = (p.flags & F_POOL) != 0;
  p.flags &= ~F_POOL;
  char nm[64];
  const double by = 4.0 * ((double)p.M * p.K * (PRO == PRO_BNBWD ? 2 : (PRO == PRO_GATE1 ? 0 : 1)) +
                           (double)p.M * p.N * (EPI == EPI_GATE ? 3 : (EPI == EPI_DGRAD ? 2 : 1)) +
                           (double)p.N * p.K);
  {
    if (p.wprep != nullptr && nt_use_s3(c, p.M, p.N, p.K) && p.lda <= 65536 && p.lda2 <= 65536 &&
        !(EPI == EPI_GATE && ((p.N | (int)p.ldc | (int)p.lde1 | (int)p.ldc2) & 3) != 0)) {
      const int KT = cdiv(p.K, S3_BK), NTl = cdiv(p.N, S3_BN);
      const long th = (long)NTl * 256 * KT * 2;
      float* hdr = reinterpret_cast<float*>(p.wprep);
      const char* img = p.wprep + S3_WHDR;
      if (c.core == 3) {
        if (p.amaxW == nullptr) {
          TRY_RC((measure_absmax<PRO_NONE>(p.W, p.ldw, nullptr, 0, nullptr, nullptr, nullptr, p.N, p.K, hdr, hdr + 64, st)));
          p.amaxW = hdr;
        }
        if (p.amaxA == nullptr) {
          TRY_RC((measure_absmax<PRO>(p.A, p.lda, p.A2, p.lda2, p.pa, p.pb, p.pc, p.M, p.K, hdr + 1, hdr + 64, st)));
          p.amaxA = hdr + 1;
        }
      }
      if constexpr (PRO == PRO_NONE || PRO == PRO_BNRELU || PRO == PRO_GATE1) {
        const bool vec_ok = ((p.N | (int)p.ldc) & 3) == 0 && (p.E1 == nullptr || ((int)p.lde1 & 3) == 0) &&
                            (p.flags & F_E1_ROWVEC) == 0 && (p.C2 == nullptr || ((int)p.ldc2 & 3) == 0);
        const int KT2 = cdiv(p.K, H2_BK);
        const size_t lds = (size_t)H2_LDS + (PRO == PRO_NONE ? 0 : 2 * (size_t)(KT2 + 2) * H2_BK * 4);
        if (c.core == 3 && vec_ok && lds <= 160 * 1024) {
          const long th2 = (long)NTl * 256 * KT2 * 4;
          hipLaunchKernelGGL(prep_weights_h2_kernel, dim3((unsigned)cdiv(th2, 256)), dim3(256), 0, st, p.W,
                             p.N, p.K, p.ldw, p.wprep + S3_WHDR, p.amaxW);
          LAUNCH_CHECK();
          p.tiles_n = NTl;
          if (want_pool) p.flags |= F_POOL;
          static const int attr_h2 = allow_big_lds(gemm_nt_h2_kernel<PRO, EPI>, gemm_nt_h2_kernel<PRO, EPI, true>);
          if (attr_h2 != PRH_OK) return attr_h2;
          snprintf(nm, sizeof(nm), "gemm_nt_h2<%d,%d> K=%d N=%d", PRO, EPI, p.K, p.N);
          ProfScope ps(nm, 2.0 * p.M * (double)p.N * p.K, by, st);
          if constexpr (PRO == PRO_NONE && EPI == EPI_BIAS) {
            if (amax_part != nullptr) {
              static const int attr_am = allow_big_lds(gemm_nt_h2_kernel<PRO, EPI, false, true>);
              if (attr_am != PRH_OK) return attr_am;
              const long wgs = (long)NTl * cdiv(p.M, 256);
              p.ws_a = amax_part;
              hipLaunchKernelGGL((gemm_nt_h2_kernel<PRO, EPI, false, true>), dim3((unsigned)wgs), dim3(512), lds, st, p, img);
              LAUNCH_CHECK();
              *amax_tiles = wgs;
              return PRH_OK;
            }
          }
          if (g_h2_pp)
            hipLaunchKernelGGL((gemm_nt_h2_kernel<PRO, EPI, true>), dim3((unsigned)(NTl * cdiv(p.M, 256))), dim3(512),
                               lds, st, p, img);
          else
            hipLaunchKernelGGL((gemm_nt_h2_kernel<PRO, EPI>), dim3((unsigned)(NTl * cdiv(p.M, 256))), dim3(512),
                               lds, st, p, img);
          LAUNCH_CHECK();
          if (si) { si->count = 2 * cdiv(p.M, S3_BM); si->rows = 128; }
          return PRH_OK;
        }
      }
      hipLaunchKernelGGL(prep_weights_s3_kernel, dim3((unsigned)cdiv(th, 256)), dim3(256), 0, st,
                         p.W, p.N, p.K, p.ldw, 0, p.wprep + S3_WHDR, c.core == 3 ? p.amaxW : nullptr);
      LAUNCH_CHECK();
      p.tiles_n = NTl;
      const long tiles = (long)NTl * cdiv(p.M, S3_BM);
      static const int attr_rc = allow_big_lds(gemm_nt_s3_kernel<PRO, EPI, 3>, gemm_nt_s3_kernel<PRO, EPI, 1>,
                                               gemm_nt_s3_kernel<PRO, EPI, 2>);
      if (attr_rc != PRH_OK) return attr_rc;
      snprintf(nm, sizeof(nm), "gemm_nt_%s<%d,%d> K=%d N=%d", c.core == 3 ? "h2g1" : c.tag(), PRO, EPI, p.K, p.N);
      ProfScope ps(nm, 2.0 * p.M * (double)p.N * p.K, by, st);
      switch (c.core) {
        case 2: launch_nt_s3<PRO, EPI, 1>(p, tiles, img, st); break;
        case 3: launch_nt_s3<PRO, EPI, 2>(p, tiles, img, st); break;
        default: launch_nt_s3<PRO, EPI, 3>(p, tiles, img, st);
      }
      LAUNCH_CHECK();
      if (si) { si->count = 2 * cdiv(p.M, S3_BM); si->rows = 128; }
      return PRH_OK;
    }
  }
  if constexpr (PRO == PRO_NONE && EPI == EPI_BIAS) {
    if (small_nt_ok(p, false)) return launch_small<false>(p, st);
  }
  p.tiles_n = cdiv(p.N, BN);
  const long tiles = (long)p.tiles_n * cdiv(p.M, BM);
  snprintf(nm, sizeof(nm), "gemm_nt<%d,%d> K=%d N=%d", PRO, EPI, p.K, p.N);
  ProfScope ps(nm, 2.0 * p.M * (double)p.N * p.K, by, st);
  if (p.N <= 64)
    hipLaunchKernelGGL((gemm_nt_kernel<PRO, EPI, true>), dim3((unsigned)tiles), dim3(256), 0, st, p);
  else
    hipLaunchKernelGGL((gemm_nt_kernel<PRO, EPI>), dim3((unsigned)tiles), dim3(256), 0, st, p);
  LAUNCH_CHECK();
  if (si) { si->count = 2 * cdiv(p.M, BM); si->rows = 64; }
  return PRH_OK;
}

template <int PRO, int EPI>
int launch_nt(Cores c, NTParams& p, hipStream_t st, StatInfo* si = nullptr, float* amax_out = nullptr,
              float* amax_part = nullptr) {
  long tiles = 0;
  TRY_RC((launch_nt_core<PRO, EPI>(c, p, st, si, amax_part, &tiles)));
  if (amax_out == nullptr) return PRH_OK;
  if (tiles > 0) {
    hipLaunchKernelGGL(absmax_final_kernel, dim3(1), dim3(256), 0, st, (const float*)amax_part, (int)tiles, amax_out);
    LAUNCH_CHECK();
    return PRH_OK;
  }
  return measure_absmax<PRO_NONE>(p.C, p.ldc, nullptr, 0, nullptr, nullptr, nullptr, p.M, p.N, amax_out, amax_part, st);
}

constexpr int TN_S3_MAX_LD = 4096;
struct TNPlan { int tiles_m, tiles_n, splits, rows_per_split; bool s3; };
inline TNPlan tn_plan(Cores c, int P, int Mo, int Ni, bool allow_s3, long maxld = TN_S3_MAX_LD) {
  TNPlan pl;
  pl.s3 = allow_s3 && tn_use_s3(c, P, Mo, Ni);
  const int tile = pl.s3 ? 256 : 128, bk = pl.s3 ? S3_BK : BK;
  pl.tiles_m = cdiv(Mo, tile);
  pl.tiles_n = cdiv(Ni, tile);
  const int tiles = pl.tiles_m * pl.tiles_n;
  int s = cdiv(pl.s3 ? (P >= 262144 ? 768 : 256) : 1024, tiles);
  if (pl.s3) {
// ... 586 lines not shown
}
const char* prh_version(void) { return "pointnet_refine_hip 0.3 (gfx950: fp32 MFMA 32x32x2 + split-fp16 / split-bf16 MFMA 32x32x16 cores)"; }

size_t prh_linear_forward_workspace_bytes(int rows, int k, int n) {
  return align_up(s3_weight_bytes(n, k) + 512, 256) + nt_amax_part_floats(rows, n) * sizeof(float) + 256;
}

int prh_linear_forward_ex(const float* x, long ldx, const float* w, const float* b, float* y,
                          int rows, int k, int n, int relu, const float* x_amax, void* workspace,
                          size_t workspace_bytes, int device, void* stream) {
  return prh_linear_forward_full(x, ldx, w, b, nullptr, 0, y, rows, k, n, relu, x_amax, nullptr, 0.f, 0u, workspace,
                                 workspace_bytes, device, stream);
}
int prh_linear_forward_full(const float* x, long ldx, const float* w, const float* b, const float* resid,
                            long ldres, float* y, int rows, int k, int n, int relu, const float* x_amax,
                            const float* w_amax, float dropout_p, unsigned dropout_seed, void* workspace,
                            size_t workspace_bytes, int device, void* stream) {
  return prh_linear_forward_amax(x, ldx, w, b, resid, ldres, y, rows, k, n, relu, x_amax, w_amax, dropout_p,
                                 dropout_seed, nullptr, workspace, workspace_bytes, device, stream);
}
int prh_linear_forward_amax(const float* x, long ldx, const float* w, const float* b, const float* resid,
                            long ldres, float* y, int rows, int k, int n, int relu, const float* x_amax,
                            const float* w_amax, float dropout_p, unsigned dropout_seed, float* y_amax_out,
                            void* workspace, size_t workspace_bytes, int device, void* stream) {
  if (!x || !w || !y || rows < 0 || k <= 0 || n <= 0 || (resid != nullptr && ldres < n))
    return fail(PRH_ERR_ARG, "linear_forward_full: bad argument");
  if (y_amax_out != nullptr && (workspace == nullptr || workspace_bytes < prh_linear_forward_workspace_bytes(rows, k, n)))
    return fail(PRH_ERR_WORKSPACE, "linear_forward_amax: workspace too small (%zu bytes)", workspace_bytes);
  if (!(dropout_p >= 0.f && dropout_p < 1.f)) return fail(PRH_ERR_ARG, "linear_forward_full: dropout_p must be in [0,1)");
  HIP_TRY(hipSetDevice(device));
  NTParams p; memset(&p, 0, sizeof(p));
  p.A = x; p.lda = ldx; p.W = w; p.ldw = k; p.C = y; p.ldc = n;
  p.M = rows; p.N = n; p.K = k; p.bias = b; p.flags = (relu ? F_RELU_OUT : 0) | (resid ? F_RESID : 0);
  p.E1 = resid; p.lde1 = ldres;
  if (dropout_p > 0.f) {
    p.flags |= F_DROPOUT;
    p.drop_seed = dropout_seed; p.drop_thresh = (unsigned)((double)dropout_p * 4294967296.0);
    p.drop_scale = 1.f / (1.f - dropout_p); p.seed_src = g_seed_src;
  }
  p.amaxW = w_amax;
  if (workspace != nullptr && workspace_bytes >= s3_weight_bytes(n, k) + 256)
    p.wprep = (char*)(((uintptr_t)workspace + 255) & ~(uintptr_t)255);
  p.amaxA = x_amax;
  float* part = nullptr;
  if (y_amax_out != nullptr)
    part = reinterpret_cast<float*>((((uintptr_t)workspace + 255) & ~(uintptr_t)255) + align_up(s3_weight_bytes(n, k) + 512, 256));
  return launch_nt<PRO_NONE, EPI_BIAS>(cores_of(gemm_mode()), p, (hipStream_t)stream, nullptr, y_amax_out, part);
}
int prh_linear_forward(const float* x, long ldx, const float* w, const float* b, float* y,
                       int rows, int k, int n, int relu, void* workspace, size_t workspace_bytes,
                       int device, void* stream) {
  return prh_linear_forward_ex(x, ldx, w, b, y, rows, k, n, relu, nullptr, workspace, workspace_bytes, device,
                               stream);
}

size_t prh_operand_absmax_workspace_bytes(void) { return (size_t)ABSMAX_MAX_BLOCKS * sizeof(float) + 256; }
int prh_operand_absmax(const float* x, long ld, long rows, int cols, float* out, void* workspace,
                       size_t workspace_bytes, int device, void* stream) {
  if (!x || !out || rows < 0 || cols <= 0 || ld < cols) return fail(PRH_ERR_ARG, "operand_absmax: bad argument");
  HIP_TRY(hipSetDevice(device));
  Arena a(workspace, workspace_bytes);
  float* part = a.f(ABSMAX_MAX_BLOCKS);
  if (!a.ok) return fail(PRH_ERR_WORKSPACE, "operand_absmax: workspace too small (%zu bytes)", workspace_bytes);
  TRY_RC((measure_absmax<PRO_NONE>(x, ld, nullptr, 0, nullptr, nullptr, nullptr, rows, cols, out, part,
                                   (hipStream_t)stream)));
  return PRH_OK;
}
int prh_relu_mask_absmax(const float* dy, const float* y, float* out, long n, float scale, float* amax_out, void* workspace,
                         size_t workspace_bytes, int device, void* stream) {
  if (!dy || !y || !out || !amax_out || n < 0 || (n & 3)) return fail(PRH_ERR_ARG, "relu_mask_absmax: bad argument");
  HIP_TRY(hipSetDevice(device));
  Arena a(workspace, workspace_bytes);
  float* part = a.f(ABSMAX_MAX_BLOCKS);
  if (!a.ok) return fail(PRH_ERR_WORKSPACE, "relu_mask_absmax: workspace too small (%zu bytes)", workspace_bytes);
  hipStream_t st = (hipStream_t)stream;
  long blocks = cdiv(n / 4, 256L * 4);
  blocks = blocks < 1 ? 1 : (blocks > ABSMAX_MAX_BLOCKS ? ABSMAX_MAX_BLOCKS : blocks);
  hipLaunchKernelGGL(relu_mask_amax_kernel, dim3((unsigned)blocks), dim3(256), 0, st, dy, y, out, (size_t)(n / 4), scale, part);
  LAUNCH_CHECK();
  hipLaunchKernelGGL(absmax_final_kernel, dim3(1), dim3(256), 0, st, (const float*)part, (int)blocks, amax_out);
  LAUNCH_CHECK();
  return PRH_OK;
}
int prh_linear_uses_operand_maxima(int rows, int k, int n) {
  const Cores c = cores_of(gemm_mode());
  return (c.mode == 3 && (nt_use_s3(c, rows, n, k) || nt_use_s3(c, rows, k, n) || tn_use_s3(c, rows, n, k))) ? 1 : 0;
}

static int pos_hidden_blocks(long P, int H) {
  const long rpp = 256 / (H / 4);
  long nb = (P + rpp * 16 - 1) / (rpp * 16);
  return (int)(nb < 1 ? 1 : (nb > 1024 ? 1024 : nb));
}
static bool pos_hidden_ok(int H) { return H >= 4 && H <= 1024 && (H & (H - 1)) == 0; }
int prh_pos_hidden_forward(const float* xyz, long ld, const float* w0, const float* b0, float* h,
                           long rows, int hidden, int device, void* stream) {
  if (!xyz || !w0 || !h || rows < 0 || ld < 3) return fail(PRH_ERR_ARG, "pos_hidden_forward: bad argument");
  if (!pos_hidden_ok(hidden))
    return fail(PRH_ERR_ARG, "pos_hidden_forward: hidden=%d must be a power of two in [4, 1024]", hidden);
  HIP_TRY(hipSetDevice(device));
  if (rows == 0) return PRH_OK;
  const long rpp = 256 / (hidden / 4);
  long nb = (rows + rpp * 4 - 1) / (rpp * 4);
  if (nb > 8192) nb = 8192;
  hipLaunchKernelGGL(pos_hidden_fwd_kernel, dim3((unsigned)nb), dim3(256), 0, (hipStream_t)stream, xyz, ld,
                     w0, b0, h, rows, hidden);
  LAUNCH_CHECK();
  return PRH_OK;
}
size_t prh_pos_hidden_forward_workspace_bytes(void) { return (size_t)8192 * sizeof(float) + 256; }
int prh_pos_hidden_forward_amax(const float* xyz, long ld, const float* w0, const float* b0, float* h,
                                long rows, int hidden, float* h_amax_out, void* workspace, size_t workspace_bytes,
                                int device, void* stream) {
  if (h_amax_out == nullptr) return prh_pos_hidden_forward(xyz, ld, w0, b0, h, rows, hidden, device, stream);
  if (!xyz || !w0 || !h || rows < 0 || ld < 3) return fail(PRH_ERR_ARG, "pos_hidden_forward: bad argument");
  if (!pos_hidden_ok(hidden))
    return fail(PRH_ERR_ARG, "pos_hidden_forward: hidden=%d must be a power of two in [4, 1024]", hidden);
  HIP_TRY(hipSetDevice(device));
  Arena a(workspace, workspace_bytes);
  float* part = a.f(8192);
  if (!a.ok || workspace == nullptr) return fail(PRH_ERR_WORKSPACE, "pos_hidden_forward_amax: workspace too small (%zu bytes)", workspace_bytes);
  hipStream_t st = (hipStream_t)stream;
  const long rpp = 256 / (hidden / 4);
  long nb = (rows + rpp * 4 - 1) / (rpp * 4);
  if (nb > 8192) nb = 8192;
  if (rows > 0) {
    hipLaunchKernelGGL(pos_hidden_fwd_amax_kernel, dim3((unsigned)nb), dim3(256), 0, st, xyz, ld, w0, b0, h, rows,
                       hidden, part);
    LAUNCH_CHECK();
  }
  hipLaunchKernelGGL(absmax_final_kernel, dim3(1), dim3(256), 0, st, (const float*)part, (int)(rows > 0 ? nb : 0), h_amax_out);
  LAUNCH_CHECK();
  return PRH_OK;
}
size_t prh_pos_hidden_backward_workspace_bytes(long rows, int hidden) {
  if (!pos_hidden_ok(hidden)) return 0;
  return (size_t)pos_hidden_blocks(rows, hidden) * 4 * hidden * sizeof(float) + 256;
}
int prh_pos_hidden_backward(const float* xyz, long ld, const float* h, const float* dh, const float* w0,
                            float* dxyz, float* dw0, float* db0, long rows, int hidden, void* workspace,
                            size_t workspace_bytes, int device, void* stream) {
  if (!xyz || !h || !dh || rows < 0 || ld < 3) return fail(PRH_ERR_ARG, "pos_hidden_backward: bad argument");
  if (dxyz != nullptr && (w0 == nullptr || hidden > 256))
    return fail(PRH_ERR_ARG, "pos_hidden_backward: point gradients need w0 and hidden <= 256 (hidden=%d)", hidden);
  if (!pos_hidden_ok(hidden))
    return fail(PRH_ERR_ARG, "pos_hidden_backward: hidden=%d must be a power of two in [4, 1024]", hidden);
  HIP_TRY(hipSetDevice(device));
  Arena a(workspace, workspace_bytes);
  const int nb = pos_hidden_blocks(rows, hidden);
  float* part = a.f((size_t)nb * 4 * hidden);
  if (!a.ok) return fail(PRH_ERR_WORKSPACE, "pos_hidden_backward: workspace too small (%zu bytes)", workspace_bytes);
  hipStream_t st = (hipStream_t)stream;
  hipLaunchKernelGGL(dxyz != nullptr ? pos_hidden_bwd_kernel<true> : pos_hidden_bwd_kernel<false>, dim3((unsigned)nb),
                     dim3(256), 0, st, xyz, ld, h, dh, part, rows, hidden, w0, dxyz);
  LAUNCH_CHECK();
  hipLaunchKernelGGL(pos_hidden_final_kernel, dim3((unsigned)cdiv(4 * hidden, 16)), dim3(256), 0, st,
                     (const float*)part, nb, hidden, dw0, db0);
  LAUNCH_CHECK();
  return PRH_OK;
}

static bool linear_small_ok(int k, int n) {
  const int lpr = k / 4;
  return n >= 1 && n <= 4 && (k & 3) == 0 && lpr >= 1 && lpr <= 64 && (lpr & (lpr - 1)) == 0;
}
static int linear_small_blocks(long rows, int k) {
  const long rpp = 256 / (k / 4);
  long nb = (rows + rpp * 8 - 1) / (rpp * 8);
  return (int)(nb < 1 ? 1 : (nb > 1024 ? 1024 : nb));
}
int prh_linear_small_forward(const float* x, const float* w, const float* b, float* y, long rows, int k,
                             int n, int device, void* stream) {
  if (!x || !w || !y || rows < 0) return fail(PRH_ERR_ARG, "linear_small_forward: bad argument");
  if (!linear_small_ok(k, n))
    return fail(PRH_ERR_ARG, "linear_small_forward: needs n <= 4 and k/4 a power of two <= 64 (k=%d n=%d)", k, n);
  HIP_TRY(hipSetDevice(device));
  if (rows == 0) return PRH_OK;
  const long rpp = 256 / (k / 4);
  long nb = (rows + rpp * 4 - 1) / (rpp * 4);
  if (nb > 4096) nb = 4096;
  hipStream_t st = (hipStream_t)stream;
  switch (n) {
    case 1: hipLaunchKernelGGL(linear_small_fwd_kernel<1>, dim3((unsigned)nb), dim3(256), 0, st, x, w, b, y, rows, k); break;
    case 2: hipLaunchKernelGGL(linear_small_fwd_kernel<2>, dim3((unsigned)nb), dim3(256), 0, st, x, w, b, y, rows, k); break;
    case 3: hipLaunchKernelGGL(linear_small_fwd_kernel<3>, dim3((unsigned)nb), dim3(256), 0, st, x, w, b, y, rows, k); break;
    default: hipLaunchKernelGGL(linear_small_fwd_kernel<4>, dim3((unsigned)nb), dim3(256), 0, st, x, w, b, y, rows, k); break;
  }
  LAUNCH_CHECK();
  return PRH_OK;
}
size_t prh_linear_small_backward_workspace_bytes(long rows, int k, int n) {
  if (!linear_small_ok(k, n)) return 0;
  return (size_t)linear_small_blocks(rows, k) * ((size_t)n * k + n) * sizeof(float) + 256;
}
int prh_linear_small_backward(const float* x, const float* w, const float* dy, float* dx, float* dw,
                              float* db, long rows, int k, int n, void* workspace, size_t workspace_bytes,
                              int device, void* stream) {
  if (!x || !w || !dy || rows < 0) return fail(PRH_ERR_ARG, "linear_small_backward: bad argument");
  if (!linear_small_ok(k, n))
    return fail(PRH_ERR_ARG, "linear_small_backward: needs n <= 4 and k/4 a power of two <= 64 (k=%d n=%d)", k, n);
  HIP_TRY(hipSetDevice(device));
  Arena a(workspace, workspace_bytes);
  const int nb = linear_small_blocks(rows, k);
  const int n_el = n * k + n;
  float* part = a.f((size_t)nb * n_el);
  if (!a.ok) return fail(PRH_ERR_WORKSPACE, "linear_small_backward: workspace too small (%zu bytes)", workspace_bytes);
  hipStream_t st = (hipStream_t)stream;
  switch (n) {
    case 1: hipLaunchKernelGGL(linear_small_bwd_kernel<1>, dim3((unsigned)nb), dim3(256), 0, st, x, w, dy, dx, part, rows, k); break;
    case 2: hipLaunchKernelGGL(linear_small_bwd_kernel<2>, dim3((unsigned)nb), dim3(256), 0, st, x, w, dy, dx, part, rows, k); break;
    case 3: hipLaunchKernelGGL(linear_small_bwd_kernel<3>, dim3((unsigned)nb), dim3(256), 0, st, x, w, dy, dx, part, rows, k); break;
    default: hipLaunchKernelGGL(linear_small_bwd_kernel<4>, dim3((unsigned)nb), dim3(256), 0, st, x, w, dy, dx, part, rows, k); break;
  }
  LAUNCH_CHECK();
  hipLaunchKernelGGL(partial_rows_final_kernel, dim3((unsigned)cdiv(n_el, 16)), dim3(256), 0, st,
                     (const float*)part, nb, n_el, dw, n * k, db);
  LAUNCH_CHECK();
  return PRH_OK;
}

size_t prh_linear_backward_workspace_bytes(int rows, int k, int n) {
  Arena a; LinearBwdWS w;
  linear_bwd_carve(cores_of(gemm_mode()), a, w, rows, k, n);
  return a.off + 256;
}

int prh_linear_backward_ex(const float* x, long ldx, const float* w, const float* dy, float* dx,
                           float* dw, float* db, int rows, int k, int n, const float* x_amax,
                           const float* dy_amax_in, void* workspace, size_t workspace_bytes, int device,
                           void* stream) {
  return prh_linear_backward_full(x, ldx, w, dy, dx, dw, db, rows, k, n, x_amax, dy_amax_in, nullptr, workspace,
                                  workspace_bytes, device, stream);
}
int prh_linear_backward_full(const float* x, long ldx, const float* w, const float* dy, float* dx,
                             float* dw, float* db, int rows, int k, int n, const float* x_amax,
                             const float* dy_amax_in, const float* w_amax, void* workspace,
                             size_t workspace_bytes, int device, void* stream) {
  return prh_linear_backward_amax(x, ldx, w, dy, dx, dw, db, rows, k, n, x_amax, dy_amax_in, w_amax, 0, nullptr,
                                  workspace, workspace_bytes, device, stream);
}
int prh_linear_backward_amax(const float* x, long ldx, const float* w, const float* dy, float* dx,
                             float* dw, float* db, int rows, int k, int n, const float* x_amax,
                             const float* dy_amax_in, const float* w_amax, int dx_accumulate, float* dx_amax_out,
                             void* workspace, size_t workspace_bytes, int device, void* stream) {
  if (!x || !w || !dy || rows < 0 || k <= 0 || n <= 0) return fail(PRH_ERR_ARG, "linear_backward: bad argument");
  if ((dx_accumulate || dx_amax_out != nullptr) && dx == nullptr)
    return fail(PRH_ERR_ARG, "linear_backward_amax: dx_accumulate / dx_amax_out need dx");
  if ((k & 3) || (n & 3)) return fail(PRH_ERR_ARG, "linear_backward: k=%d and n=%d must be multiples of 4", k, n);
  HIP_TRY(hipSetDevice(device));
  hipStream_t st = (hipStream_t)stream;
  const Cores c = cores_of(gemm_mode());
  Arena a(workspace, workspace_bytes);
  LinearBwdWS lw;
  linear_bwd_carve(c, a, lw, rows, k, n);
  if (!a.ok) return fail(PRH_ERR_WORKSPACE, "linear_backward: workspace too small (%zu bytes)", workspace_bytes);
  float *wT = lw.wT, *slab = lw.slab, *cslab = lw.cslab;
  const float* dy_amax = dy_amax_in;
  bool dx_done = false;
  const bool big16 = c.mode == 4 && rows >= 512 && (long)cdiv(rows, 256) * cdiv(k, 256) >= 16;
  if (dx != nullptr && !big16) {
    NTParams p; memset(&p, 0, sizeof(p));
    p.A = dy; p.lda = n; p.W = w; p.ldw = k; p.C = dx; p.ldc = k; p.M = rows; p.N = k; p.K = n;
    if (dx_accumulate) { p.flags = F_RESID; p.E1 = dx; p.lde1 = k; }
    if (small_nt_ok(p, true) && !(nt_use_s3(c, rows, k, n))) {
      TRY((launch_small<true>(p, st)));
      if (dx_amax_out != nullptr)
        TRY_RC((measure_absmax<PRO_NONE>(dx, k, nullptr, 0, nullptr, nullptr, nullptr, rows, k, dx_amax_out, lw.dxpart, st)));
      dx_done = true;
    }
  }
  if (dx != nullptr && !dx_done) {
    TRY(transpose(w, n, k, wT, st));
    NTParams p; memset(&p, 0, sizeof(p));
    p.A = dy; p.lda = n; p.W = wT; p.ldw = n; p.C = dx; p.ldc = k; p.M = rows; p.N = k; p.K = n;
    p.wprep = lw.wprep;
    p.amaxA = dy_amax;
    p.amaxW = w_amax;
    if (dx_accumulate) { p.flags = F_RESID; p.E1 = dx; p.lde1 = k; }
    TRY((launch_nt<PRO_NONE, EPI_BIAS>(c, p, st, nullptr, dx_amax_out,
                                      (dx_accumulate || dx_amax_out != nullptr) ? lw.dxpart : nullptr)));
    dy_amax = p.amaxA;
  }
  if (dw != nullptr || db != nullptr) {
    TNParams t; memset(&t, 0, sizeof(t));
    t.amaxA = dy_amax;
    t.amaxB = x_amax;
    t.A = dy; t.lda = n; t.B = x; t.ldb = ldx; t.P = rows; t.Mo = n; t.Ni = k;
    TRY((launch_tn<PRO_NONE, PRO_NONE>(c, t, slab, cslab, dw, (long)k, db, st)));
  }
  return PRH_OK;
}
int prh_linear_backward(const float* x, long ldx, const float* w, const float* dy, float* dx,
                        float* dw, float* db, int rows, int k, int n, void* workspace,
                        size_t workspace_bytes, int device, void* stream) {
  return prh_linear_backward_ex(x, ldx, w, dy, dx, dw, db, rows, k, n, nullptr, nullptr, workspace,
                                workspace_bytes, device, stream);
}

size_t prh_mlp_stack_workspace_bytes(int P, int n_layers, const prh_bn_layer* layers) {
  if (n_layers < 1 || n_layers > PRH_MAX_LAYERS) return 0;
  Arena a; MlpWS m;
  mlp_carve(stack_cores(gemm_mode()), a, m, P, layers, n_layers);
  return a.off + 256;
}

int prh_mlp_stack_forward(const prh_bn_layer* layers, int n_layers, int relu_last,
                          const float* x, int P, int training, float momentum, float eps,
                          float* z_cat, float* y, float* bn_scale, float* bn_shift,
                          float* bn_mean, float* bn_rstd, void* workspace,
                          size_t workspace_bytes, int device, void* stream) {
  TRY(check_stack(layers, n_layers));
  const Cores c = stack_cores(gemm_mode());
  if (!x || !z_cat || !y || !bn_scale || !bn_shift || !bn_mean || !bn_rstd || P <= 0)
    return fail(PRH_ERR_ARG, "mlp_stack_forward: bad argument");
  if (training && P < 2) return fail(PRH_ERR_ARG, "Expected more than 1 value per channel when training");
  HIP_TRY(hipSetDevice(device));
  hipStream_t st = (hipStream_t)stream;
  StackDims d = stack_dims(layers, n_layers);
  Arena a(workspace, workspace_bytes);
  MlpWS m;
  mlp_carve(c, a, m, P, layers, n_layers);
  if (!a.ok) return fail(PRH_ERR_WORKSPACE, "mlp_stack_forward: workspace too small (%zu bytes)", workspace_bytes);
  StackWS& w = m.w;
  const long ldz = d.off[n_layers];
  TRY(stack_forward(c, layers, n_layers, x, P, training, momentum, eps, z_cat, ldz, bn_scale,
                    bn_shift, bn_mean, bn_rstd, w, st));
  const int L = n_layers, co = layers[L - 1].cout;
  hipLaunchKernelGGL(bn_apply_kernel, dim3(cdiv(P, 64), cdiv(co, 64)), dim3(256), 0, st,
                     z_cat + d.off[L - 1], ldz, bn_scale + d.off[L - 1], bn_shift + d.off[L - 1], P,
                     co, relu_last, y, (long)co);
  LAUNCH_CHECK();
  return PRH_OK;
}

int prh_mlp_stack_backward(const prh_bn_layer* layers, int n_layers, int relu_last,
                           const float* x, int P, int training, const float* dy,
                           const float* z_cat, const float* bn_scale, const float* bn_shift,
                           const float* bn_mean, const float* bn_rstd,
                           const prh_bn_layer_grad* grads, float* dx, void* workspace,
                           size_t workspace_bytes, int device, void* stream) {
  TRY(check_stack(layers, n_layers));
  const Cores c = stack_cores(gemm_mode());
  if (!x || !dy || !z_cat || P <= 0) return fail(PRH_ERR_ARG, "mlp_stack_backward: bad argument");
  HIP_TRY(hipSetDevice(device));
  hipStream_t st = (hipStream_t)stream;
  StackDims d = stack_dims(layers, n_layers);
  const int L = n_layers;
  Arena a(workspace, workspace_bytes);
  MlpWS m;
  mlp_carve(c, a, m, P, layers, L);
  StackWS& w = m.w;
  StackBwdScratch& sc = m.sc;
  const long ldz = d.off[L];
  float* dy_cat = m.dy_cat;
  if (!a.ok) return fail(PRH_ERR_WORKSPACE, "mlp_stack_backward: workspace too small (%zu bytes)", workspace_bytes);
  if (d.cin0p != d.cin0) {
    TRY(copy_cols(x, d.cin0, d.cin0, w.xpad, d.cin0p, d.cin0p, (size_t)P, st));
    TRY(copy_cols(layers[0].w, d.cin0, d.cin0, w.w0pad, d.cin0p, d.cin0p, (size_t)layers[0].cout, st));
  }
  if (L > 1) HIP_TRY(hipMemsetAsync(dy_cat, 0, (size_t)P * ldz * sizeof(float), st));
  const int co = layers[L - 1].cout, o = d.off[L - 1];
  hipLaunchKernelGGL(bn_dy_stats_kernel, dim3(cdiv(P, 64), cdiv(co, 64)), dim3(256), 0, st, dy,
                     (long)co, z_cat + o, ldz, bn_scale + o, bn_shift + o, P, co, relu_last,
// ... 124 lines not shown
  EncWS ews;
  if (d_fused_scratch && (d_fused == nullptr || d_gfeat != nullptr))
    return fail(PRH_ERR_ARG, "encoder_backward: d_fused_scratch needs d_fused and no d_gfeat");
  enc_carve(c, a, ews, P, prm->conv, cat, od, d_fused_scratch ? 2 : 1);
  StackWS& w = ews.w;
  StackBwdScratch& sc = ews.sc;
  float *fslab = ews.fslab, *fcslab = ews.fcslab, *dy_cat = ews.dy_cat, *dU = ews.dU, *dyf = d_fused_scratch ? d_fused : ews.dyf;
  float *gsum_a = ews.gsum_a, *gsum_b = ews.gsum_b;
  if (!a.ok) return fail(PRH_ERR_WORKSPACE, "encoder_backward: workspace too small (%zu bytes)", workspace_bytes);
  StackDims d = stack_dims(prm->conv, 5);
  if (d.cin0p != d.cin0) {
    TRY(copy_cols(ctx, d.cin0, d.cin0, w.xpad, d.cin0p, d.cin0p, (size_t)P, st));
    TRY(copy_cols(prm->conv[0].w, d.cin0, d.cin0, w.w0pad, d.cin0p, d.cin0p, (size_t)prm->conv[0].cout, st));
  }

  hipLaunchKernelGGL(combine_bwd_kernel, dim3(cdiv(P, 64), cdiv(od, 64)), dim3(256), 0, st, d_fused,
                     d_gfeat, sv->argmax, sv->z_fus, sv->gate, sv->bn_scale + cat,
                     sv->bn_shift + cat, P, N, od, dyf, w.ws_a, w.ws_b);
  LAUNCH_CHECK();
  hipLaunchKernelGGL(bn_stage1_kernel, dim3(cdiv(od, 32), BN_SLICES), dim3(256), 0, st, w.ws_a, w.ws_b,
                     cdiv(P, 64), (long)od, od, 64, P, 0, w.stat2);
  LAUNCH_CHECK();
  hipLaunchKernelGGL(bn_bwd_finalize_kernel, dim3(cdiv(od, 128)), dim3(128), 0, st, w.stat2, P, od,
                     prm->fusion.gamma, sv->bn_mean + cat, sv->bn_rstd + cat,
                     training, sc.ca, sc.cb, sc.cc, gr->fusion.dgamma, gr->fusion.dbeta,
                     gr->fusion.db);
  LAUNCH_CHECK();
  float* dG = sv->gate;

  StatInfo si5;
  const float* dzf_amax = nullptr;
  const bool matf = dz_in_place(c, od, (long)od, (long)od);
  if (matf) {
    TRY(materialize_dz(dyf, (long)od, sv->z_fus, (long)od, sc.ca, sc.cb, sc.cc, P, od, sc.hdr[0], st));
    dzf_amax = sc.hdr[0];
  }
  HeldWgrad hf;
  if (gr->fusion.dw) {
    TNParams t; memset(&t, 0, sizeof(t));
    t.A = dyf; t.lda = od; t.A2 = sv->z_fus; t.lda2 = od; t.pa = sc.ca; t.pb = sc.cb; t.pc = sc.cc;
    t.B = sv->z_cat; t.ldb = cat; t.qa = sv->bn_scale; t.qb = sv->bn_shift;
    t.P = P; t.Mo = od; t.Ni = cat;
    t.amaxA = dzf_amax;
    if (training && c.mode == 3 && sv->op_amax != nullptr) t.amaxB = sv->op_amax + 5;
    if (matf && dz_in_place(c, od, (long)cat, (long)cat) &&
        tn_side_ok(c, t, side_job(dy_cat + d.off[4], (long)cat, sv->z_cat + d.off[4], (long)cat, sc, P, od, sc.hdr[1]))) {
      hf.on = true; hf.t = t; hf.slab = fslab; hf.colslab = fcslab; hf.out = gr->fusion.dw; hf.ldc = (long)cat;
    } else if (matf) TRY((launch_tn<PRO_NONE, PRO_BNRELU>(c, t, fslab, fcslab, gr->fusion.dw, (long)cat, nullptr, st)));
    else TRY((launch_tn<PRO_BNBWD, PRO_BNRELU>(c, t, fslab, fcslab, gr->fusion.dw, (long)cat, nullptr, st)));
    dzf_amax = t.amaxA;
  }
  {
    TRY(transpose(prm->fusion.w, od, cat, sc.wT, st));
    NTParams p; memset(&p, 0, sizeof(p));
    p.amaxA = dzf_amax;
    p.A = dyf; p.lda = od; p.A2 = sv->z_fus; p.lda2 = od; p.pa = sc.ca; p.pb = sc.cb; p.pc = sc.cc;
    p.W = sc.wT; p.ldw = od; p.M = P; p.N = cat; p.K = od;
    p.C = dy_cat; p.ldc = cat; p.E1 = sv->z_cat; p.lde1 = cat; p.es = sv->bn_scale; p.et = sv->bn_shift;
    p.wprep = w.wprep;
    p.ws_a = w.ws_a; p.ws_b = w.ws_b;
    p.flags = F_MASK | F_STATS;
    if (matf) TRY((launch_nt<PRO_NONE, EPI_DGRAD>(c, p, st, &si5)));
    else TRY((launch_nt<PRO_BNBWD, EPI_DGRAD>(c, p, st, &si5)));
    si5.ld = cat; si5.off = d.off[4];
  }
  float* dx = d_ctx;
  TRY(stack_backward(c, prm->conv, 5, ctx, P, training, dy_cat, (long)cat, sv->z_cat, (long)cat,
                     sv->bn_scale, sv->bn_shift, sv->bn_mean, sv->bn_rstd, gr->conv, dx, w, sc, si5,
                     st, sv->op_amax, &hf));

  {
    TNParams t; memset(&t, 0, sizeof(t));
    t.A = dG; t.lda = od; t.B = ctx + 3; t.ldb = C; t.qa = prm->gate_w1; t.qb = prm->gate_b1;
    t.P = P; t.Mo = od; t.Ni = 64;
    TRY((launch_tn<PRO_NONE, PRO_GATE1>(c, t, fslab, fcslab, gr->d_gate_w2, 64L, gr->d_gate_b2, st)));
    TRY(transpose(prm->gate_w2, od, 64, sc.wT, st));
    NTParams p; memset(&p, 0, sizeof(p));
    p.A = dG; p.lda = od; p.W = sc.wT; p.ldw = od; p.M = P; p.N = 64; p.K = od;
    p.C = dU; p.ldc = 64; p.E1 = ctx + 3; p.lde1 = C; p.es = prm->gate_w1; p.et = prm->gate_b1;
    p.ws_a = w.ws_a; p.ws_b = w.ws_b;
    p.flags = F_MASK | F_STATS | F_E1_ROWVEC;
    StatInfo sig;
    TRY((launch_nt<PRO_NONE, EPI_DGRAD>(c, p, st, &sig)));
    hipLaunchKernelGGL(partials_reduce_kernel, dim3(2), dim3(1024), 0, st, w.ws_a, w.ws_b,
                       sig.count, 64, gr->d_gate_b1 ? gr->d_gate_b1 : gsum_a,
                       gr->d_gate_w1 ? gr->d_gate_w1 : gsum_b);
    LAUNCH_CHECK();
    if (d_ctx != nullptr) {
      hipLaunchKernelGGL(gate1_dctx_kernel, dim3(cdiv(P, 4)), dim3(256), 0, st, dU, P, 64,
                         prm->gate_w1, d_ctx, (long)C);
      LAUNCH_CHECK();
    }
  }
  return PRH_OK;
}


size_t prh_encoder_bf16_workspace_bytes(int B, int N, int in_channel, int out_dim, int backward) {
  const int ch[6] = {in_channel, 64, 128, 256, 512, out_dim};
  Arena a; Enc16WS e;
  enc16_carve(a, e, B * N, ch, 64 + 128 + 256 + 512 + out_dim, out_dim, backward != 0);
  return a.off + 256;
}

int prh_encoder_forward_bf16(const prh_encoder_params* prm, const float* ctx, int B, int N, int training,
                             float momentum, float eps, uint16_t* fused, float* gfeat,
                             const prh_encoder_saved_bf16* sv, void* workspace, size_t workspace_bytes,
                             int device, void* stream) {
  TRY(check_encoder(prm));
  if (!ctx || !fused || !sv || !sv->z_cat || !sv->z_fus || !sv->bn_scale || !sv->bn_shift || !sv->bn_mean ||
      !sv->bn_rstd || B <= 0 || N <= 0)
    return fail(PRH_ERR_ARG, "encoder_forward_bf16: bad argument");
  if ((long)B * N > 1000000000L) return fail(PRH_ERR_ARG, "encoder_forward_bf16: B*N too large");
  const int P = B * N;
  if (training && P < 2) return fail(PRH_ERR_ARG, "Expected more than 1 value per channel when training");
  for (int l = 0; l < 5; ++l)
    if (prm->conv[l].cout % 8) return fail(PRH_ERR_ARG, "encoder_forward_bf16: channel widths must be multiples of 8");
  if (prm->out_dim % 8) return fail(PRH_ERR_ARG, "encoder_forward_bf16: out_dim must be a multiple of 8");
  HIP_TRY(hipSetDevice(device));
  hipStream_t st = (hipStream_t)stream;
  const int cat = enc_cat(prm), od = prm->out_dim, C = prm->in_channel, c0p = cin_pad8(C);
  const int ch[6] = {C, prm->conv[0].cout, prm->conv[1].cout, prm->conv[2].cout, prm->conv[3].cout, od};
  Arena a(workspace, workspace_bytes);
  Enc16WS w;
  enc16_carve(a, w, P, ch, cat, od, false);
  if (!a.ok) return fail(PRH_ERR_WORKSPACE, "encoder_forward_bf16: workspace too small (%zu bytes)", workspace_bytes);
  StackDims d = stack_dims(prm->conv, 5);
  u16* z_cat = sv->z_cat;
  const bool c1_fp32 = conv_in_fp32_ok(C, prm->conv[0].cout);
  if (!c1_fp32) {
    TRY(cast_b16(ctx, C, C, w.xpad, c0p, c0p, (size_t)P, st));
    TRY(copy_cols(prm->conv[0].w, C, C, w.w0pad, c0p, c0p, (size_t)prm->conv[0].cout, st));
  }
  for (int l = 0; l < 5; ++l) {
    const prh_bn_layer& ly = prm->conv[l];
    NTParams p; memset(&p, 0, sizeof(p));
    p.M = P; p.N = ly.cout; p.bias = ly.b; p.C = f16p(z_cat + d.off[l]); p.ldc = cat;
    p.ws_a = w.ws_a; p.ws_b = w.ws_b; p.wprep = w.wprep;
    StatInfo si;
    if (l == 0 && c1_fp32) {
      hipLaunchKernelGGL((conv_in_b16_kernel<64>), dim3(cdiv(P, 128)), dim3(256), 0, st, ctx, C, ly.w, ly.b, z_cat, (long)cat, P,
                         training, w.ws_a, w.ws_b);
      LAUNCH_CHECK();
      si.count = cdiv(P, 128); si.rows = 128;
    } else if (l == 0) {
      p.A = f16p(w.xpad); p.lda = c0p; p.W = w.w0pad; p.ldw = c0p; p.K = c0p;
      if (training) TRY((launch_nt_b16<PRO_NONE, EPI_BIAS_STATS, true, true>(p, st, &si)));
      else TRY((launch_nt_b16<PRO_NONE, EPI_BIAS, true, true>(p, st)));
    } else {
      p.A = f16p(z_cat + d.off[l - 1]); p.lda = cat; p.W = ly.w; p.ldw = ly.cin; p.K = ly.cin;
      p.pa = sv->bn_scale + d.off[l - 1]; p.pb = sv->bn_shift + d.off[l - 1];
      if (training) TRY((launch_nt_b16<PRO_BNRELU, EPI_BIAS_STATS, true, true>(p, st, &si)));
      else TRY((launch_nt_b16<PRO_BNRELU, EPI_BIAS, true, true>(p, st)));
    }
    TRY(bn_coeffs(ly, P, training, momentum, eps, w.ws_a, w.ws_b, w.stat2, si, sv->bn_mean + d.off[l],
                  sv->bn_rstd + d.off[l], sv->bn_scale + d.off[l], sv->bn_shift + d.off[l], st));
  }
  {
    NTParams p; memset(&p, 0, sizeof(p));
    p.A = f16p(z_cat); p.lda = cat; p.W = prm->fusion.w; p.ldw = cat; p.K = cat;
    p.pa = sv->bn_scale; p.pb = sv->bn_shift;
    p.M = P; p.N = od; p.bias = prm->fusion.b; p.C = f16p(sv->z_fus); p.ldc = od;
    p.ws_a = w.ws_a; p.ws_b = w.ws_b; p.wprep = w.wprep;
    StatInfo si;
    if (training) TRY((launch_nt_b16<PRO_BNRELU, EPI_BIAS_STATS, true, true>(p, st, &si)));
    else TRY((launch_nt_b16<PRO_BNRELU, EPI_BIAS, true, true>(p, st)));
    TRY(bn_coeffs(prm->fusion, P, training, momentum, eps, w.ws_a, w.ws_b, w.stat2, si, sv->bn_mean + cat,
                  sv->bn_rstd + cat, sv->bn_scale + cat, sv->bn_shift + cat, st));
  }
  {
// ... 65 lines not shown
  if (gr->fusion.dw) {
    TNParams t; memset(&t, 0, sizeof(t));
    t.A = f16p(w.dyf); t.lda = od; t.B = f16p(z_cat); t.ldb = cat; t.qa = sv->bn_scale; t.qb = sv->bn_shift;
    t.P = P; t.Mo = od; t.Ni = cat;
    TRY((launch_tn_b16<PRO_BNRELU>(t, w.slab, w.cslab, gr->fusion.dw, (long)cat, nullptr, st)));
  }
  StatInfo si;
  {
    TRY(transpose(prm->fusion.w, od, cat, w.wT, st));
    NTParams p; memset(&p, 0, sizeof(p));
    p.A = f16p(w.dyf); p.lda = od; p.W = w.wT; p.ldw = od; p.M = P; p.N = cat; p.K = od;
    p.C = f16p(w.dy_cat); p.ldc = cat; p.E1 = f16p(z_cat); p.lde1 = cat; p.es = sv->bn_scale; p.et = sv->bn_shift;
    p.wprep = w.wprep; p.ws_a = w.ws_a; p.ws_b = w.ws_b;
    p.flags = F_MASK | F_STATS;
    TRY((launch_nt_b16<PRO_NONE, EPI_DGRAD, true, true>(p, st, &si)));
    si.ld = cat; si.off = d.off[4];
  }
  for (int l = 4; l >= 0; --l) {
    const prh_bn_layer& ly = prm->conv[l];
    const int co = ly.cout, o = d.off[l];
    hipLaunchKernelGGL(bn_stage1_kernel, dim3(cdiv(co, 32), BN_SLICES), dim3(256), 0, st, w.ws_a + si.off, w.ws_b + si.off,
                       si.count, si.ld ? si.ld : (long)co, co, 64, P, 0, w.stat2);
    LAUNCH_CHECK();
    hipLaunchKernelGGL(bn_bwd_finalize_kernel, dim3(cdiv(co, 128)), dim3(128), 0, st, w.stat2, P, co, ly.gamma,
                       sv->bn_mean + o, sv->bn_rstd + o, training, w.ca, w.cb, w.cc, gr->conv[l].dgamma,
                       gr->conv[l].dbeta, gr->conv[l].db);
    LAUNCH_CHECK();
    TRY(bn_bwd_apply16(w.dy_cat + o, cat, z_cat + o, cat, w.ca, w.cb, w.cc, P, co, st));
    if (gr->conv[l].dw) {
      TNParams t; memset(&t, 0, sizeof(t));
      t.A = f16p(w.dy_cat + o); t.lda = cat; t.P = P; t.Mo = co;
      if (l == 0 && c1_fp32) {
        const int rpb = cdiv(cdiv(P, C1_WGRAD_BLOCKS), 4) * 4, nb = cdiv(P, rpb);
        hipLaunchKernelGGL((conv_in_wgrad_b16_kernel<64>), dim3(nb), dim3(256), 0, st, (const u16*)(w.dy_cat + o), (long)cat,
                           ctx, C, P, rpb, w.c1part);
        LAUNCH_CHECK();
        hipLaunchKernelGGL(slab_reduce_kernel, dim3(cdiv((long)co * C, 256)), dim3(256), 0, st, (const float*)w.c1part, nb, co, C,
                           gr->conv[0].dw, (long)C);
        LAUNCH_CHECK();
      } else if (l == 0) {
        t.B = f16p(w.xpad); t.ldb = c0p; t.Ni = c0p;
        float* out = c0p == C ? gr->conv[0].dw : w.wT;
        TRY((launch_tn_b16<PRO_NONE>(t, w.slab, w.cslab, out, (long)c0p, nullptr, st)));
        if (c0p != C) TRY(copy_cols(w.wT, c0p, C, gr->conv[0].dw, C, C, (size_t)co, st));
      } else {
        t.B = f16p(z_cat + d.off[l - 1]); t.ldb = cat; t.Ni = ly.cin;
        t.qa = sv->bn_scale + d.off[l - 1]; t.qb = sv->bn_shift + d.off[l - 1];
        TRY((launch_tn_b16<PRO_BNRELU>(t, w.slab, w.cslab, gr->conv[l].dw, (long)ly.cin, nullptr, st)));
      }
    }
    if (l > 0) {
      TRY(transpose(ly.w, co, ly.cin, w.wT, st));
      NTParams p; memset(&p, 0, sizeof(p));
      p.A = f16p(w.dy_cat + o); p.lda = cat; p.W = w.wT; p.ldw = co; p.M = P; p.N = ly.cin; p.K = co;
      p.C = f16p(w.dy_cat + d.off[l - 1]); p.ldc = cat;
      p.E1 = f16p(z_cat + d.off[l - 1]); p.lde1 = cat;
      p.es = sv->bn_scale + d.off[l - 1]; p.et = sv->bn_shift + d.off[l - 1];
      p.ws_a = w.ws_a; p.ws_b = w.ws_b; p.wprep = w.wprep;
      p.flags = F_ACCUM | F_MASK | F_STATS;
      TRY((launch_nt_b16<PRO_NONE, EPI_DGRAD, true, true>(p, st, &si)));
      si.ld = 0; si.off = 0;
    } else if (d_ctx != nullptr) {
      TRY(transpose(w.w0pad, co, c0p, w.wT, st));
      NTParams p; memset(&p, 0, sizeof(p));
      p.A = f16p(w.dy_cat + o); p.lda = cat; p.W = w.wT; p.ldw = co; p.M = P; p.N = C; p.K = co;
      p.C = d_ctx; p.ldc = C; p.wprep = w.wprep; p.flags = 0;
      if (C % 4) return fail(PRH_ERR_ARG, "encoder_backward_bf16: d_ctx needs in_channel %% 4 == 0");
      TRY((launch_nt_b16<PRO_NONE, EPI_DGRAD, true, false>(p, st)));
    }
  }
  {
    TNParams t; memset(&t, 0, sizeof(t));
    t.A = f16p(dG); t.lda = od; t.B = ctx + 3; t.ldb = C; t.qa = prm->gate_w1; t.qb = prm->gate_b1;
    t.P = P; t.Mo = od; t.Ni = 64;
    TRY((launch_tn_b16<PRO_GATE1>(t, w.slab, w.cslab, gr->d_gate_w2, 64L, gr->d_gate_b2, st)));
    TRY(transpose(prm->gate_w2, od, 64, w.wT, st));
    NTParams p; memset(&p, 0, sizeof(p));
    p.A = f16p(dG); p.lda = od; p.W = w.wT; p.ldw = od; p.M = P; p.N = 64; p.K = od;
    p.C = w.dU; p.ldc = 64; p.E1 = ctx + 3; p.lde1 = C; p.es = prm->gate_w1; p.et = prm->gate_b1;
    p.ws_a = w.ws_a; p.ws_b = w.ws_b; p.wprep = w.wprep;
    p.flags = F_MASK | F_STATS | F_E1_ROWVEC;
    StatInfo sig;
    TRY((launch_nt_b16<PRO_NONE, EPI_DGRAD, true, false>(p, st, &sig)));
    hipLaunchKernelGGL(partials_reduce_kernel, dim3(2), dim3(1024), 0, st, w.ws_a, w.ws_b, sig.count, 64,
                       gr->d_gate_b1 ? gr->d_gate_b1 : w.gsum_a, gr->d_gate_w1 ? gr->d_gate_w1 : w.gsum_b);
    LAUNCH_CHECK();
    if (d_ctx != nullptr) {
      hipLaunchKernelGGL(gate1_dctx_kernel, dim3(cdiv(P, 4)), dim3(256), 0, st, w.dU, P, 64, prm->gate_w1, d_ctx, (long)C);
      LAUNCH_CHECK();
    }
  }
  return PRH_OK;
}

size_t prh_linear_bf16_workspace_bytes(int rows, int k, int n, int backward) {
  Arena a; Lin16WS w;
  lin16_carve(a, w, rows, k, n, backward != 0);
  return a.off + 256;
}
int prh_linear_forward_bf16(const uint16_t* x, long ldx, const float* w, const float* b, float* y, int rows, int k,
                            int n, int relu, void* workspace, size_t workspace_bytes, int device, void* stream) {
  if (!x || !w || !y || rows < 0 || k <= 0 || n <= 0) return fail(PRH_ERR_ARG, "linear_forward_bf16: bad argument");
  HIP_TRY(hipSetDevice(device));
  Arena a(workspace, workspace_bytes); Lin16WS lw;
  lin16_carve(a, lw, rows, k, n, false);
  if (!a.ok) return fail(PRH_ERR_WORKSPACE, "linear_forward_bf16: workspace too small (%zu bytes)", workspace_bytes);
  NTParams p; memset(&p, 0, sizeof(p));
  p.A = f16p(x); p.lda = ldx; p.W = w; p.ldw = k; p.C = y; p.ldc = n; p.M = rows; p.N = n; p.K = k; p.bias = b;
  p.flags = relu ? F_RELU_OUT : 0; p.wprep = lw.wprep;
  return launch_nt_b16<PRO_NONE, EPI_BIAS, true, false>(p, (hipStream_t)stream);
}
int prh_linear_backward_bf16(const uint16_t* x, long ldx, const float* w, const float* dy, uint16_t* dx, float* dw,
                             float* db, int rows, int k, int n, void* workspace, size_t workspace_bytes, int device,
                             void* stream) {
  if (!x || !w || !dy || rows < 0 || k <= 0 || n <= 0) return fail(PRH_ERR_ARG, "linear_backward_bf16: bad argument");
  if ((k & 7) || (n & 7)) return fail(PRH_ERR_ARG, "linear_backward_bf16: k=%d and n=%d must be multiples of 8", k, n);
  HIP_TRY(hipSetDevice(device));
  hipStream_t st = (hipStream_t)stream;
  Arena a(workspace, workspace_bytes); Lin16WS lw;
  lin16_carve(a, lw, rows, k, n, true);
  if (!a.ok) return fail(PRH_ERR_WORKSPACE, "linear_backward_bf16: workspace too small (%zu bytes)", workspace_bytes);
  TRY(cast_b16(dy, n, n, lw.dy16, n, n, (size_t)rows, st));
  if (dx != nullptr) {
    TRY(transpose(w, n, k, lw.wT, st));
    NTParams p; memset(&p, 0, sizeof(p));
    p.A = f16p(lw.dy16); p.lda = n; p.W = lw.wT; p.ldw = n; p.C = f16p(dx); p.ldc = k; p.M = rows; p.N = k; p.K = n;
    p.wprep = lw.wprep;
    TRY((launch_nt_b16<PRO_NONE, EPI_BIAS, true, true>(p, st)));
  }
  if (dw != nullptr || db != nullptr) {
    TNParams t; memset(&t, 0, sizeof(t));
    t.A = f16p(lw.dy16); t.lda = n; t.B = f16p(x); t.ldb = ldx; t.P = rows; t.Mo = n; t.Ni = k;
    TRY((launch_tn_b16<PRO_NONE>(t, lw.slab, lw.cslab, dw, (long)k, db, st)));
  }
  return PRH_OK;
}

int prh_linear_forward_out16(const float* x, long ldx, const float* w, const float* b, uint16_t* y, int rows, int k,
                             int n, void* workspace, size_t workspace_bytes, int device, void* stream) {
  if (!x || !w || !y || rows < 0 || k <= 0 || n <= 0) return fail(PRH_ERR_ARG, "linear_forward_out16: bad argument");
  HIP_TRY(hipSetDevice(device));
  Arena a(workspace, workspace_bytes); Lin16WS lw;
  lin16_carve(a, lw, rows, k, n, false);
  if (!a.ok) return fail(PRH_ERR_WORKSPACE, "linear_forward_out16: workspace too small (%zu bytes)", workspace_bytes);
  NTParams p; memset(&p, 0, sizeof(p));
  p.A = x; p.lda = ldx; p.W = w; p.ldw = k; p.C = f16p(y); p.ldc = n; p.M = rows; p.N = n; p.K = k; p.bias = b;
  p.wprep = lw.wprep;
  return launch_nt_b16<PRO_NONE, EPI_BIAS, false, true>(p, (hipStream_t)stream);
}
int prh_linear_backward_dy16(const float* x, long ldx, const float* w, const uint16_t* dy, float* dx, float* dw,
                             float* db, int rows, int k, int n, void* workspace, size_t workspace_bytes, int device,
                             void* stream) {
  if (!x || !w || !dy || rows < 0 || k <= 0 || n <= 0) return fail(PRH_ERR_ARG, "linear_backward_dy16: bad argument");
  if ((k & 7) || (n & 7)) return fail(PRH_ERR_ARG, "linear_backward_dy16: k=%d and n=%d must be multiples of 8", k, n);
  HIP_TRY(hipSetDevice(device));
  hipStream_t st = (hipStream_t)stream;
  Arena a(workspace, workspace_bytes); Lin16WS lw;
  lin16_carve(a, lw, rows, k, n, true);
  if (!a.ok) return fail(PRH_ERR_WORKSPACE, "linear_backward_dy16: workspace too small (%zu bytes)", workspace_bytes);
  if (dx != nullptr) {
    TRY(transpose(w, n, k, lw.wT, st));
    NTParams p; memset(&p, 0, sizeof(p));
    p.A = f16p(dy); p.lda = n; p.W = lw.wT; p.ldw = n; p.C = dx; p.ldc = k; p.M = rows; p.N = k; p.K = n;
    p.wprep = lw.wprep;
    TRY((launch_nt_b16<PRO_NONE, EPI_BIAS, true, false>(p, st)));
  }
  if (dw != nullptr || db != nullptr) {
    TRY(cast_b16(x, ldx, k, lw.dy16, k, k, (size_t)rows, st));
    TNParams t; memset(&t, 0, sizeof(t));
// ... 1692 lines not shown
```

### pointnet_refine_amd/model.py

```python
from __future__ import annotations

import torch
import torch.nn as nn
import torch.nn.functional as F

from . import ops


def _warn_saturated(e):
    import warnings
    warnings.warn(f"{e} - falling back to the per-layer HIP kernels for this call", RuntimeWarning, stacklevel=3)


def _bn_buffers(bn: nn.BatchNorm1d):
    return [bn.running_mean, bn.running_var, bn.num_batches_tracked]


def _attn(q, k, v, heads, dropout_p):
    seed = int(torch.randint(0, 2 ** 31 - 1, (1,)).item()) if dropout_p > 0.0 else 0
    return ops.attention(q, k, v, heads, dropout_p, seed)


def _add_norm(x, r, norm, drop, training):
    if not norm.elementwise_affine:
# ... 60 lines not shown
        gfeat, fused = self.forward_pointmajor(x.transpose(2, 1).contiguous(), True)
        if fused.dtype != x.dtype:
            fused = fused.to(x.dtype)
        return gfeat, fused.transpose(2, 1)


class PositionalEncoding(nn.Module):

    def __init__(self, in_dim=3, out_dim=256):
        super().__init__()
        self.mlp = nn.Sequential(nn.Linear(in_dim, out_dim), nn.ReLU(), nn.Linear(out_dim, out_dim))

    def hidden(self, xyz):
        l0, l2 = self.mlp[0], self.mlp[2]
        if l0.in_features != 3 or not ops.pos_hidden_supported(l0.out_features) or l2.out_features % 4:
            raise RuntimeError(f"pointnet_refine_amd: PositionalEncoding({l0.in_features}, {l2.out_features}) is not "
                               "supported by the HIP path (3-wide points, power-of-two hidden width <= 1024)")
        return ops.pos_hidden_with_amax(xyz, l0.weight, l0.bias)

    def forward(self, xyz, resid=None):
        l2 = self.mlp[2]
        h, h_amax = self.hidden(xyz)
        if resid is None:
            return ops.linear(h, l2.weight, l2.bias, h_amax)
        y, y_amax = ops.linear_with_amax(h, l2.weight, l2.bias, h_amax, False, resid)
        ops.amax_note(y, y_amax)
        return y


class DetrTransformerDecoderLayer(nn.Module):

    def __init__(self, d_model=256, nhead=8, dim_feedforward=1024, dropout=0.1):
        super().__init__()
        for name in ("self_attn", "cross_attn"):
            self.add_module(name, nn.MultiheadAttention(d_model, nhead, dropout=dropout, batch_first=True))
        self.linear1 = nn.Linear(d_model, dim_feedforward)
        self.dropout = nn.Dropout(dropout)
        self.linear2 = nn.Linear(dim_feedforward, d_model)
        for k in (1, 2, 3):
            self.add_module(f"norm{k}", nn.LayerNorm(d_model))
        for k in (1, 2, 3):
            self.add_module(f"dropout{k}", nn.Dropout(dropout))
        self.activation = F.relu

    def with_pos_embed(self, tensor, pos):
        return tensor if pos is None else tensor + pos

    def forward(self, tgt, memory, query_pos=None, pos=None):
        ca, d = self.cross_attn, self.cross_attn.embed_dim
        k_proj = _lin(self.with_pos_embed(memory, pos), ca.in_proj_weight[d:2 * d], ca.in_proj_bias[d:2 * d])
        v_proj = _lin(memory, ca.in_proj_weight[2 * d:], ca.in_proj_bias[2 * d:])
        return self.forward_projected(tgt, k_proj, v_proj, query_pos=query_pos)

    def forward_projected(self, tgt, k_proj, v_proj, query_pos=None, kv_block=None):
        sa = self.self_attn
        d, h = sa.embed_dim, sa.num_heads
        B, M, _ = tgt.shape
        qk_in = self.with_pos_embed(tgt, query_pos)
        qk = _lin(qk_in, sa.in_proj_weight[:2 * d], sa.in_proj_bias[:2 * d])
        vv = _lin(tgt, sa.in_proj_weight[2 * d:], sa.in_proj_bias[2 * d:])
        pdrop_sa = sa.dropout if self.training else 0.0
        seed_sa = int(torch.randint(0, 2 ** 31 - 1, (1,)).item()) if pdrop_sa > 0.0 else 0
        o = ops.attention_self_packed(qk, vv, h, pdrop_sa, seed_sa)
        tgt2 = _lin(o, sa.out_proj.weight, sa.out_proj.bias)
        tgt = _add_norm(tgt, tgt2, self.norm1, self.dropout1, self.training)
        ca = self.cross_attn
        qp = _lin(self.with_pos_embed(tgt, query_pos), ca.in_proj_weight[:d], ca.in_proj_bias[:d])
        pdrop = ca.dropout if self.training else 0.0
        if kv_block is not None and kv_block[0] == "fold":
            o = ops.attention_folded(qp, k_proj, v_proj, ca.in_proj_weight[d:2 * d], ca.in_proj_weight[2 * d:],
                                     ca.in_proj_bias[2 * d:], h)
        elif kv_block is not None:
            token, arena, blk = kv_block
            seed = int(torch.randint(0, 2 ** 31 - 1, (1,)).item()) if pdrop > 0.0 else 0
            o = ops.attention_block(qp, k_proj, v_proj, token, arena, blk, h, pdrop, seed)
        else:
            o = _attn(qp, k_proj, v_proj, h, pdrop)
        tgt2 = _lin(o, ca.out_proj.weight, ca.out_proj.bias)
        tgt = _add_norm(tgt, tgt2, self.norm2, self.dropout2, self.training)
        if self.activation is not F.relu:
            raise RuntimeError("pointnet_refine_amd: the FFN activation is ReLU (src/model.py:95), fused into the GEMM epilogue")
        pd = self.dropout.p if self.training else 0.0
        seed = int(torch.randint(0, 2 ** 31 - 1, (1,)).item()) if pd > 0.0 else 0
        hid, hid_amax = ops.linear_with_amax(tgt, self.linear1.weight, self.linear1.bias, None, True, None, pd, seed)
        tgt2 = ops.linear(hid, self.linear2.weight, self.linear2.bias, hid_amax)
        tgt = _add_norm(tgt, tgt2, self.norm3, self.dropout3, self.training)
        return tgt


class LineRefineNet(nn.Module):

    def __init__(self, num_line_points=32, feature_dim=1024):
        super().__init__()
        d = self.d_model = 256
        L = self.num_decoder_layers = 6
        self.context_encoder = MultiScalePointNetEncoder(in_channel=4, out_dim=feature_dim)
        self.context_proj = nn.Linear(feature_dim, d)
        stack, widths = [], (3, 64, 128, d)
        for k in range(1, 4):
            stack += [nn.Conv1d(widths[k - 1], widths[k], kernel_size=1), nn.BatchNorm1d(widths[k])]
            if k < 3:
                stack.append(nn.ReLU())
        self.point_mlp = nn.Sequential(*stack)
        self.pos_emb = PositionalEncoding(in_dim=3, out_dim=d)
        self.decoder_layers = nn.ModuleList(
            DetrTransformerDecoderLayer(d_model=d, nhead=8, dim_feedforward=1024) for _ in range(L))
        self.reg_branches = nn.ModuleList(
            nn.Sequential(nn.Linear(d, 128), nn.ReLU(), nn.Linear(128, 3)) for _ in range(L))

    def encode_context(self, context, defer_check=False):
        enc = self.context_encoder
        if context.dim() != 3:
            raise RuntimeError(f"Expected 3D (batched) input, but got input of size: {list(context.shape)}")
        if enc._fused_ok(context) and tuple(self.context_proj.weight.shape) == (256, 1024):
            try:
                memory, _, _ = ops.encoder_eval_fused(context, enc._param_list(), enc._bn_buffer_list(), enc.bn1.eps,
                                                      self.context_proj.weight, self.context_proj.bias,
                                                      precision=enc.inference_precision, check=not defer_check)
                self._fused_pending = defer_check
                return memory
            except ops.FusedSaturation as e:
                _warn_saturated(e)
        _, fused, fused_amax = ops.encoder_with_amax(context, enc._param_list(), enc._bn_buffer_list(), False,
                                                     enc.training, enc.bn1.momentum, enc.bn1.eps)
        memory, mem_amax = ops.linear_with_amax(fused, self.context_proj.weight, self.context_proj.bias, fused_amax)
        ops.amax_note(memory, mem_amax)
        return memory

    def encode_line(self, noisy_line):
        B, M, _ = noisy_line.shape
        pm = self.point_mlp
        layers = [(pm[0].weight, pm[0].bias, pm[1].weight, pm[1].bias),
                  (pm[3].weight, pm[3].bias, pm[4].weight, pm[4].bias),
                  (pm[6].weight, pm[6].bias, pm[7].weight, pm[7].bias)]
        buffers = _bn_buffers(pm[1]) + _bn_buffers(pm[4]) + _bn_buffers(pm[7])
        y = ops.mlp_stack(noisy_line.reshape(B * M, -1), layers, buffers, relu_last=False,
                          training=self.training, momentum=pm[1].momentum, eps=pm[1].eps)
        return y.reshape(B, M, -1)

    fold_kv_inference = True

    def _fold_ok(self, memory, noisy_line):
        return (self.fold_kv_inference and not self.training and not torch.is_grad_enabled() and memory.is_cuda
                and ops.bf16_mode() and self.d_model == 256 and noisy_line.shape[1] <= 32
                and self.decoder_layers[0].cross_attn.num_heads == 8)

    def decode(self, context, noisy_line, memory, tgt):
        d = self.d_model
        layers = self.decoder_layers
        fold = self._fold_ok(memory, noisy_line)
        if fold:
            l0, l2 = self.pos_emb.mlp[0], self.pos_emb.mlp[2]
            if tuple(l0.weight.shape) == (256, 3) and tuple(l2.weight.shape) == (256, 256):
                k_all, v_all = ops.posmem_images(context[:, :, :3], memory, l0.weight, l0.bias, l2.weight, l2.bias)
            else:
                mempos = self.pos_emb(context[:, :, :3], resid=memory)
                k_all, v_all = ops.cast_perm_bf16(mempos), ops.cast_perm_bf16(memory)
        span = (not fold and ops.producer_maxima_on(memory.is_cuda) and memory.dtype == torch.float32
                and context.dtype == torch.float32)
        if not fold and not span:
            mempos = self.pos_emb(context[:, :, :3], resid=memory)
        cat = ops.cat_rows
        if d != 256:
            raise RuntimeError("pointnet_refine_amd: the decoder kernels are built for d_model = 256 (src/model.py:141)")
        if not fold:
            wk = cat([l.cross_attn.in_proj_weight[d:2 * d] for l in layers])
            bk = cat([l.cross_attn.in_proj_bias[d:2 * d] for l in layers])
            wv = cat([l.cross_attn.in_proj_weight[2 * d:] for l in layers])
# ... 58 lines not shown
```

### pointnet_refine_amd/ops.py

```python
from __future__ import annotations

import ctypes as C
import math
import threading
import weakref
from typing import List, Optional, Sequence

import torch

from . import _lib as L

_workspaces = {}


def _ws(device: torch.device, nbytes: int) -> torch.Tensor:
    key = (device.index, torch.cuda.current_stream(device).cuda_stream)
    t = _workspaces.get(key)
    if t is None or t.numel() < nbytes:
        _workspaces.pop(key, None)
        t = None
        t = torch.empty(int(nbytes * 1.05) + 4096, dtype=torch.uint8, device=device)
        _workspaces[key] = t
    return t

# ... 311 lines not shown
        x2 = x.reshape(-1, k)
        if not x2.is_contiguous():
            x2 = x2.contiguous()
        w = w.contiguous()
        rows = x2.shape[0]
        y = torch.empty((rows, n), dtype=torch.float32, device=x.device)
        ws = _ws(x.device, L.lib().prh_linear_bf16_workspace_bytes(rows, k, n, 0))
        L.check(L.lib().prh_linear_forward_bf16(_p(x2), k, _p(w), _p(b), _p(y), rows, k, n, 0, _p(ws), ws.numel(),
                                                x.device.index, _stream(x.device)), "prh_linear_forward_bf16")
        ctx.save_for_backward(x2, w)
        ctx.bf16_in, ctx.relu, ctx.has_resid, ctx.has_bias, ctx.xshape = True, False, False, b is not None, x.shape
        return y.reshape(*x.shape[:-1], n)

    @staticmethod
    def _backward_bf16(ctx, dy):
        x2, w = ctx.saved_tensors
        n, k = w.shape
        rows, dev = x2.shape[0], x2.device
        dy2 = dy.reshape(rows, n).float().contiguous()
        need_dx, need_dw, need_db = ctx.needs_input_grad[0], ctx.needs_input_grad[1], ctx.has_bias and ctx.needs_input_grad[2]
        dx = torch.empty_like(x2) if need_dx else None
        dw, tw = _grad_buf(ctx.w_sink, w.shape, dev, need_dw)
        db, tb = _grad_buf(ctx.b_sink, (n,), dev, need_db)
        ws = _ws(dev, L.lib().prh_linear_bf16_workspace_bytes(rows, k, n, 1))
        L.check(L.lib().prh_linear_backward_bf16(_p(x2), k, _p(w), _p(dy2), _p(dx), _p(dw), _p(db), rows, k, n, _p(ws),
                                                 ws.numel(), dev.index, _stream(dev)), "prh_linear_backward_bf16")
        return (dx.reshape(ctx.xshape) if need_dx else None), _grad_ret(dw, tw), _grad_ret(db, tb), None, None, None, None, None

    @staticmethod
    def backward(ctx, dy):
        if ctx.bf16_in:
            return LinearFn._backward_bf16(ctx, dy)
        if ctx.relu:
            x2, w, y = ctx.saved_tensors
        else:
            x2, w = ctx.saved_tensors
        n, k = w.shape
        rows = x2.shape[0]
        if n % 4:
            raise RuntimeError("pointnet_refine_amd.linear backward: out_features must be a multiple of 4")
        dy2 = dy.reshape(rows, n)
        hint = _hint_take(dy)
        dy_amax = hint if (hint is not None and dy2.data_ptr() == dy.data_ptr()) else None
        if not dy2.is_contiguous():
            dy2 = dy2.contiguous()
        dev = x2.device
        if ctx.relu:
            if dy2.dtype != torch.float32:
                dy2 = dy2.float()
            masked = torch.empty_like(dy2)
            dy_amax = torch.empty(1, dtype=torch.float32, device=dev)
            wsm = _ws(dev, L.lib().prh_operand_absmax_workspace_bytes())
            L.check(L.lib().prh_relu_mask_absmax(_p(dy2), _p(y), _p(masked), dy2.numel(), float(ctx.drop_scale), _p(dy_amax), _p(wsm),
                                                 wsm.numel(), dev.index, _stream(dev)), "prh_relu_mask_absmax")
            dy2 = masked
        need_dx, need_dw, need_db = ctx.needs_input_grad[0], ctx.needs_input_grad[1], ctx.has_bias and ctx.needs_input_grad[2]
        dx = torch.empty_like(x2) if need_dx else None
        dw, tw = _grad_buf(ctx.w_sink, w.shape, dev, need_dw)
        db, tb = _grad_buf(ctx.b_sink, (n,), dev, need_db)
        _linear_bwd(x2, w, dy2, ctx.x_amax, dy_amax, ctx.w_amax, dx, dw, db)
        dres = None
        if ctx.has_resid and ctx.needs_input_grad[5]:
            dres = dy2.reshape(*ctx.xshape[:-1], n)
        return (dx.reshape(ctx.xshape) if need_dx else None), _grad_ret(dw, tw), _grad_ret(db, tb), None, None, dres, None, None


def linear(x, w, b=None, x_amax=None, relu=False, resid=None, dropout_p=0.0, seed=0):
    return LinearFn.apply(x, w, b, x_amax, relu, resid, dropout_p, seed)


def producer_maxima_on(device_ok=True) -> bool:
    return bool(PRODUCER_MAXIMA and device_ok and L.lib().prh_get_gemm_mode() == 3)


def linear_with_amax(x, w, b=None, x_amax=None, relu=False, resid=None, dropout_p=0.0, seed=0):
    LinearFn.last_y_amax = None
    LinearFn.want_y_amax = producer_maxima_on(x.is_cuda) and x.dtype == torch.float32
    try:
        y = LinearFn.apply(x, w, b, x_amax, relu, resid, dropout_p, seed)
    finally:
        LinearFn.want_y_amax = False
    amax, LinearFn.last_y_amax = LinearFn.last_y_amax, None
    return y, amax


class LinearOut16Fn(torch.autograd.Function):

    @staticmethod
    def forward(ctx, x, w, b):
        ctx.w_sink, ctx.b_sink = _sink_view(w), _sink_view(b)
        _req_gpu_f32(x, "input")
        _req_gpu_f32(w, "weight")
        n, k = w.shape
        if x.shape[-1] != k or k % 8 or n % 8:
            raise RuntimeError("pointnet_refine_amd.linear_out16: in/out features must be multiples of 8")
        x2 = x.reshape(-1, k)
        if not x2.is_contiguous():
            x2 = x2.contiguous()
        w = w.contiguous()
        rows = x2.shape[0]
        y = torch.empty((rows, n), dtype=torch.bfloat16, device=x.device)
        ws = _ws(x.device, L.lib().prh_linear_bf16_workspace_bytes(rows, k, n, 0))
        L.check(L.lib().prh_linear_forward_out16(_p(x2), k, _p(w), _p(b), _p(y), rows, k, n, _p(ws), ws.numel(),
                                                 x.device.index, _stream(x.device)), "prh_linear_forward_out16")
        ctx.save_for_backward(x2, w)
        ctx.has_bias, ctx.xshape = b is not None, x.shape
        return y.reshape(*x.shape[:-1], n)

    @staticmethod
    def backward(ctx, dy):
        x2, w = ctx.saved_tensors
        n, k = w.shape
        rows, dev = x2.shape[0], x2.device
        dy2 = dy.reshape(rows, n)
        if dy2.dtype != torch.bfloat16 or not dy2.is_contiguous():
            dy2 = dy2.to(torch.bfloat16).contiguous()
        need_dx, need_dw, need_db = ctx.needs_input_grad[0], ctx.needs_input_grad[1], ctx.has_bias and ctx.needs_input_grad[2]
        dx = torch.empty_like(x2) if need_dx else None
        dw, tw = _grad_buf(ctx.w_sink, w.shape, dev, need_dw)
        db, tb = _grad_buf(ctx.b_sink, (n,), dev, need_db)
        ws = _ws(dev, L.lib().prh_linear_bf16_workspace_bytes(rows, k, n, 1))
        L.check(L.lib().prh_linear_backward_dy16(_p(x2), k, _p(w), _p(dy2), _p(dx), _p(dw), _p(db), rows, k, n, _p(ws),
                                                 ws.numel(), dev.index, _stream(dev)), "prh_linear_backward_dy16")
        return (dx.reshape(ctx.xshape) if need_dx else None), _grad_ret(dw, tw), _grad_ret(db, tb)


def linear_out16(x, w, b=None):
    return LinearOut16Fn.apply(x, w, b)


class PosHiddenFn(torch.autograd.Function):

    want_amax = False
    last_amax = None

    @staticmethod
    def forward(ctx, xyz, w0, b0):
        ctx.w_sink, ctx.b_sink = _sink_view(w0), _sink_view(b0)
        _req_gpu_f32(xyz, "input")
        _req_gpu_f32(w0, "weight")
        hdim = w0.shape[0]
        if xyz.shape[-1] != 3 or w0.shape[1] != 3:
            raise RuntimeError(f"pos_hidden: expected 3-wide points and a (H, 3) weight, got {tuple(xyz.shape)} and {tuple(w0.shape)}")
        rows = xyz.numel() // 3
        ld = xyz.stride(-2) if xyz.dim() >= 2 else 3
        ok = xyz.stride(-1) == 1 and ld >= 3
        for d in range(xyz.dim() - 2):
            ok = ok and xyz.stride(d) == xyz.stride(d + 1) * xyz.shape[d + 1]
        if not ok:
            xyz = xyz.contiguous()
            ld = 3
        w0 = w0.contiguous()
        h = torch.empty((*xyz.shape[:-1], hdim), dtype=torch.float32, device=xyz.device)
        want, PosHiddenFn.want_amax = PosHiddenFn.want_amax, False
        amax = torch.empty(1, dtype=torch.float32, device=xyz.device) if want else None
        ws = _ws(xyz.device, L.lib().prh_pos_hidden_forward_workspace_bytes()) if want else None
        L.check(L.lib().prh_pos_hidden_forward_amax(_p(xyz), ld, _p(w0), _p(b0), _p(h), rows, hdim, _p(amax), _p(ws),
                                                    ws.numel() if want else 0, xyz.device.index, _stream(xyz.device)),
                "prh_pos_hidden_forward")
        PosHiddenFn.last_amax = amax
        ctx.save_for_backward(xyz, h, w0)
        ctx.ld, ctx.has_bias = ld, b0 is not None
        return h

    @staticmethod
    def backward(ctx, dh):
# ... 955 lines not shown
```

Measured before the change: 9726 segments/s.

## Fuse FFN ReLU-mask backward into dgrad epilogue and split partials reduction

Adds an FFN autograd function that runs linear2's dgrad with a ReLU/dropout mask and output abs-max computed in the GEMM epilogue. This replaces the separate dgrad, mask and abs-max passes over the hidden activation. It also replaces the two-block partials reduction with a sliced two-stage reduction so more blocks take part. The cost is extra code paths and a fallback path when the masked kernel is not eligible.

After: 9784 segments/s (median of 6 runs). About the same (+0.6%).

```diff
diff --git a/include/pointnet_refine_hip.h b/include/pointnet_refine_hip.h
--- a/include/pointnet_refine_hip.h
+++ b/include/pointnet_refine_hip.h
@@ -153,6 +153,9 @@
 int prh_relu_mask_absmax(const float* dy, const float* y, float* out, long n, float scale, float* amax_out,
                          void* workspace, size_t workspace_bytes, int device, void* stream);
 int prh_linear_uses_operand_maxima(int rows, int k, int n);
+size_t prh_partials_reduce_workspace_bytes(int tiles, int n);
+int prh_partials_reduce(const float* a, const float* b, int tiles, int n, float* out_a, float* out_b,
+                        void* workspace, size_t workspace_bytes, int device, void* stream);
 
 int prh_pos_hidden_forward(const float* xyz, long ld, const float* w0, const float* b0, float* h,
                            long rows, int hidden, int device, void* stream);
@@ -189,6 +192,12 @@
                              float* dw, float* db, int rows, int k, int n, const float* x_amax,
                              const float* dy_amax, const float* w_amax, int dx_accumulate, float* dx_amax_out,
                              void* workspace, size_t workspace_bytes, int device, void* stream);
+int prh_linear_backward_masked_ok(int rows, int k, int n);
+int prh_linear_backward_masked(const float* x, long ldx, const float* w, const float* dy, float* dx,
+                               float* dw, float* db, int rows, int k, int n, const float* x_amax,
+                               const float* dy_amax, const float* w_amax, const float* mask_y, float mask_scale,
+                               float* dx_amax_out, void* workspace, size_t workspace_bytes, int device,
+                               void* stream);
 
 size_t prh_mlp_stack_workspace_bytes(int P, int n_layers, const prh_bn_layer* layers);
 int prh_mlp_stack_forward(const prh_bn_layer* layers, int n_layers, int relu_last,
diff --git a/pointnet_refine_amd/_lib.py b/pointnet_refine_amd/_lib.py
--- a/pointnet_refine_amd/_lib.py
+++ b/pointnet_refine_amd/_lib.py
@@ -60,6 +60,7 @@
     "prh_linear_forward_workspace_bytes", "prh_linear_forward", "prh_linear_forward_ex",
     "prh_linear_forward_full", "prh_linear_forward_amax", "prh_operand_absmax_workspace_bytes", "prh_operand_absmax",
     "prh_linear_uses_operand_maxima", "prh_linear_backward_full", "prh_linear_backward_amax", "prh_pos_hidden_forward",
+    "prh_linear_backward_masked_ok", "prh_linear_backward_masked", "prh_partials_reduce_workspace_bytes", "prh_partials_reduce",
     "prh_pos_hidden_forward_workspace_bytes", "prh_pos_hidden_forward_amax", "prh_pos_hidden_backward_workspace_bytes",
     "prh_pos_hidden_backward", "prh_linear_small_forward", "prh_linear_small_backward_workspace_bytes",
     "prh_linear_small_backward",
@@ -178,6 +179,14 @@
     lib.prh_linear_forward_amax.argtypes = [vp, lg, vp, vp, vp, lg, vp, i, i, i, i, vp, vp, f, C.c_uint, vp, vp, sz, i, vp]
     lib.prh_linear_backward_amax.restype = i
     lib.prh_linear_backward_amax.argtypes = [vp, lg, vp, vp, vp, vp, vp, i, i, i, vp, vp, vp, i, vp, vp, sz, i, vp]
+    lib.prh_linear_backward_masked_ok.restype = i
+    lib.prh_linear_backward_masked_ok.argtypes = [i, i, i]
+    lib.prh_linear_backward_masked.restype = i
+    lib.prh_linear_backward_masked.argtypes = [vp, lg, vp, vp, vp, vp, vp, i, i, i, vp, vp, vp, vp, f, vp, vp, sz, i, vp]
+    lib.prh_partials_reduce_workspace_bytes.restype = sz
+    lib.prh_partials_reduce_workspace_bytes.argtypes = [i, i]
+    lib.prh_partials_reduce.restype = i
+    lib.prh_partials_reduce.argtypes = [vp, vp, i, i, vp, vp, vp, sz, i, vp]
     lib.prh_pos_hidden_forward_workspace_bytes.restype = sz
     lib.prh_pos_hidden_forward_workspace_bytes.argtypes = []
     lib.prh_pos_hidden_forward_amax.restype = i
diff --git a/pointnet_refine_amd/csrc/prh_gemm.hpp b/pointnet_refine_amd/csrc/prh_gemm.hpp
--- a/pointnet_refine_amd/csrc/prh_gemm.hpp
+++ b/pointnet_refine_amd/csrc/prh_gemm.hpp
@@ -377,7 +377,8 @@
                                                 int cbase, int rb, int lane, float* scratch,
                                                 bool bias_done = false,
                                                 float* wave_amax = nullptr) {
-  static_assert(!AMAX || (EPI == EPI_BIAS && !C16), "output maximum: EPI_BIAS with fp32 storage");
+  static_assert(!AMAX || ((EPI == EPI_BIAS || EPI == EPI_DGRAD) && !C16), "output maximum: EPI_BIAS / masked dgrad with fp32 storage");
+  constexpr bool RMASK = AMAX && EPI == EPI_DGRAD;
   typedef typename std::conditional<AMAX, char*, epi_wptr_r>::type wptr;
   typedef typename std::conditional<AMAX, const char*, epi_rptr_r>::type rptr;
   const int rbase = __builtin_amdgcn_readfirstlane(rbase_);
@@ -395,7 +396,7 @@
   float4 bias4 = zero4(), es4 = zero4(), et4 = zero4();
   if (c4ok) {
     if (biasp != nullptr) bias4 = ldg4(biasp + col4);
-    if ((EPI == EPI_DGRAD && (p.flags & F_MASK) != 0) || EPI == EPI_GATE) {
+    if ((EPI == EPI_DGRAD && !RMASK && (p.flags & F_MASK) != 0) || EPI == EPI_GATE) {
       es4 = ldg4(p.es + col4);
       et4 = ldg4(p.et + col4);
     }
@@ -405,11 +406,11 @@
 
   if (EPI == EPI_BIAS_STATS) epi_col_stats(acc, p, cbase, mrows, rb, lane, biasp);
 
-  const bool mask = (p.flags & F_MASK) != 0, accum = (p.flags & F_ACCUM) != 0;
-  const bool stats = EPI == EPI_DGRAD && (p.flags & F_STATS) != 0;
+  const bool mask = (p.flags & F_MASK) != 0, accum = !RMASK && (p.flags & F_ACCUM) != 0;
+  const bool stats = EPI == EPI_DGRAD && !RMASK && (p.flags & F_STATS) != 0;
   const bool resid = EPI == EPI_BIAS && (p.flags & F_RESID) != 0;
   const unsigned dseed = (EPI == EPI_BIAS && (p.flags & F_DROPOUT) != 0) ? epi_seed(p) : 0u;
-  const bool need_z = (EPI == EPI_DGRAD && (mask || stats)) || EPI == EPI_GATE || resid;
+  const bool need_z = RMASK || (EPI == EPI_DGRAD && (mask || stats)) || EPI == EPI_GATE || resid;
   float4 s1 = zero4(), s2 = zero4();
   const bool pool = EPI == EPI_GATE && (p.flags & F_POOL) != 0;
   float pmx[4] = {-1.f, -1.f, -1.f, -1.f}, psm[4] = {0.f, 0.f, 0.f, 0.f};
@@ -465,7 +466,11 @@
       v.x += bias4.x; v.y += bias4.y; v.z += bias4.z; v.w += bias4.w;
       const float4 z = zz[b & 1][i];
       const float4 o = oo[b & 1][i];
-      if (EPI == EPI_DGRAD) {
+      if constexpr (RMASK) {
+        const float sc = p.drop_scale;
+        v.x = z.x > 0.f ? v.x * sc : 0.f; v.y = z.y > 0.f ? v.y * sc : 0.f;
+        v.z = z.z > 0.f ? v.z * sc : 0.f; v.w = z.w > 0.f ? v.w * sc : 0.f;
+      } else if (EPI == EPI_DGRAD) {
         v.x += o.x; v.y += o.y; v.z += o.z; v.w += o.w;
         if (mask) {
           v.x = fmaf(z.x, es4.x, et4.x) > 0.f ? v.x : 0.f;
@@ -512,7 +517,7 @@
       if (ok) st4e<C16>(Cb, lr * ldc + col4, v);
       if (AMAX && ok) amx = fmaxf(fmaxf(amx, fmaxf(fabsf(v.x), fabsf(v.y))), fmaxf(fabsf(v.z), fabsf(v.w)));
     }
-    if (EPI == EPI_DGRAD)
+    if (EPI == EPI_DGRAD && !RMASK)
       asm volatile("" : "+v"(s1.x), "+v"(s1.y), "+v"(s1.z), "+v"(s1.w), "+v"(s2.x), "+v"(s2.y), "+v"(s2.z), "+v"(s2.w));
   }
   if (pool) {
diff --git a/pointnet_refine_amd/csrc/prh_gemm_h2.hpp b/pointnet_refine_amd/csrc/prh_gemm_h2.hpp
--- a/pointnet_refine_amd/csrc/prh_gemm_h2.hpp
+++ b/pointnet_refine_amd/csrc/prh_gemm_h2.hpp
@@ -76,7 +76,8 @@
 __global__ __launch_bounds__(512, 2) void gemm_nt_h2_kernel(const NTParams p,
                                                             const char* __restrict__ Wp) {
   static_assert(PRO == PRO_NONE || PRO == PRO_BNRELU || PRO == PRO_GATE1, "prologue not supported");
-  static_assert(!AMAX || (PRO == PRO_NONE && EPI == EPI_BIAS), "output maximum: plain EPI_BIAS launches only");
+  static_assert(!AMAX || (PRO == PRO_NONE && (EPI == EPI_BIAS || EPI == EPI_DGRAD)),
+                "output maximum: plain EPI_BIAS launches, and the masked dgrad (EPI_DGRAD: nt_epilogue_vec_r2)");
   extern __shared__ __attribute__((aligned(16))) char smem[];
 #ifdef PRH_STAMP
   unsigned t_acc[4] = {0u, 0u, 0u, 0u};
diff --git a/pointnet_refine_amd/csrc/prh_kernels.hpp b/pointnet_refine_amd/csrc/prh_kernels.hpp
--- a/pointnet_refine_amd/csrc/prh_kernels.hpp
+++ b/pointnet_refine_amd/csrc/prh_kernels.hpp
@@ -168,18 +168,55 @@
   if (dbias != nullptr) dbias[col] = (float)(a * Sdy + b * (double)P * mu + cst * (double)P);
 }
 
-__global__ __launch_bounds__(1024) void partials_reduce_kernel(
-    const float* __restrict__ ws_a, const float* __restrict__ ws_b, int R2, int N, float* out_a,
-    float* out_b) {
+constexpr int PARTIALS_MAX_SLICES = 512;
+constexpr int PARTIALS_SLICE_ROWS = 64;
+inline int partials_slices(int R2, size_t mid_doubles, int N) {
+  long s = ((long)R2 + PARTIALS_SLICE_ROWS - 1) / PARTIALS_SLICE_ROWS;
+  const long cap = (long)(mid_doubles / ((size_t)2 * (size_t)N));
+  s = s > PARTIALS_MAX_SLICES ? PARTIALS_MAX_SLICES : s;
+  s = s > cap ? cap : s;
+  return s < 1 ? 1 : (int)s;
+}
+__global__ __launch_bounds__(256) void partials_reduce_kernel(
+    const float* __restrict__ ws_a, const float* __restrict__ ws_b, int R2, int N,
+    double* __restrict__ mid) {
+  __shared__ double red[2][8][33];
+  const int c = threadIdx.x & 31, g = threadIdx.x >> 5;
+  const int col = blockIdx.x * 32 + c, sl = blockIdx.y;
+  const int per = (R2 + (int)gridDim.y - 1) / (int)gridDim.y;
+  const long r0 = (long)sl * per;
+  const int r1 = (int)(r0 + per < (long)R2 ? r0 + per : (long)R2);
+  const bool ok = col < N;
+  double s1 = 0.0, s2 = 0.0;
+  if (ok)
+    for (int i = (int)r0 + g; i < r1; i += 8) {
+      s1 += (double)ws_a[(size_t)i * N + col];
+      if (ws_b != nullptr) s2 += (double)ws_b[(size_t)i * N + col];
+    }
+  red[0][g][c] = s1;
+  red[1][g][c] = s2;
+  __syncthreads();
+  if (g == 0 && ok) {
+    double a = 0.0, b = 0.0;
+    for (int j = 0; j < 8; ++j) {
+      a += red[0][j][c];
+      b += red[1][j][c];
+    }
+    mid[((size_t)sl * 2) * N + col] = a;
+    mid[((size_t)sl * 2 + 1) * N + col] = b;
+  }
+}
+__global__ __launch_bounds__(1024) void partials_final_kernel(const double* __restrict__ mid, int S,
+                                                              int N, float* out_a, float* out_b) {
   __shared__ double red[2][32][33];
   const int c = threadIdx.x & 31, g = threadIdx.x >> 5;
   const int col = blockIdx.x * 32 + c;
   const bool ok = col < N;
   double s1 = 0.0, s2 = 0.0;
   if (ok)
-    for (int i = g; i < R2; i += 32) {
-      s1 += (double)ws_a[(size_t)i * N + col];
-      if (ws_b != nullptr) s2 += (double)ws_b[(size_t)i * N + col];
+    for (int i = g; i < S; i += 32) {
+      s1 += mid[((size_t)i * 2) * N + col];
+      s2 += mid[((size_t)i * 2 + 1) * N + col];
     }
   red[0][g][c] = s1;
   red[1][g][c] = s2;
diff --git a/pointnet_refine_amd/csrc/prh_lib.hip b/pointnet_refine_amd/csrc/prh_lib.hip
--- a/pointnet_refine_amd/csrc/prh_lib.hip
+++ b/pointnet_refine_amd/csrc/prh_lib.hip
@@ -161,6 +161,16 @@
                      kb, kc, rows, cols, hdr + 64);
   LAUNCH_CHECK();
   hipLaunchKernelGGL(absmax_final_kernel, dim3(1), dim3(256), 0, st, hdr + 64, (int)blocks, hdr);
+  LAUNCH_CHECK();
+  return PRH_OK;
+}
+int partials_reduce(const float* ws_a, const float* ws_b, int R2, int N, float* out_a, float* out_b,
+                    double* mid, size_t mid_doubles, hipStream_t st) {
+  const int S = partials_slices(R2, mid_doubles, N);
+  hipLaunchKernelGGL(partials_reduce_kernel, dim3(cdiv(N, 32), S), dim3(256), 0, st, ws_a, ws_b, R2, N, mid);
+  LAUNCH_CHECK();
+  hipLaunchKernelGGL(partials_final_kernel, dim3(cdiv(N, 32)), dim3(1024), 0, st, (const double*)mid, S, N,
+                     out_a, out_b);
   LAUNCH_CHECK();
   return PRH_OK;
 }
@@ -411,7 +421,7 @@
           if (attr_h2 != PRH_OK) return attr_h2;
           snprintf(nm, sizeof(nm), "gemm_nt_h2<%d,%d> K=%d N=%d", PRO, EPI, p.K, p.N);
           ProfScope ps(nm, 2.0 * p.M * (double)p.N * p.K, by, st);
-          if constexpr (PRO == PRO_NONE && EPI == EPI_BIAS) {
+          if constexpr (PRO == PRO_NONE && (EPI == EPI_BIAS || EPI == EPI_DGRAD)) {
             if (amax_part != nullptr) {
               static const int attr_am = allow_big_lds(gemm_nt_h2_kernel<PRO, EPI, false, true>);
               if (attr_am != PRH_OK) return attr_am;
@@ -1164,6 +1174,20 @@
   LAUNCH_CHECK();
   return PRH_OK;
 }
+size_t prh_partials_reduce_workspace_bytes(int tiles, int n) {
+  (void)tiles;
+  return (size_t)PARTIALS_MAX_SLICES * 2 * (size_t)(n > 0 ? n : 1) * sizeof(double) + 256;
+}
+int prh_partials_reduce(const float* a, const float* b, int tiles, int n, float* out_a, float* out_b, void* workspace,
+                        size_t workspace_bytes, int device, void* stream) {
+  if (!a || tiles < 0 || n <= 0) return fail(PRH_ERR_ARG, "partials_reduce: bad argument");
+  HIP_TRY(hipSetDevice(device));
+  Arena ar(workspace, workspace_bytes);
+  const size_t mid_doubles = (size_t)PARTIALS_MAX_SLICES * 2 * (size_t)n;
+  double* mid = (double*)ar.f(mid_doubles * 2);
+  if (!ar.ok || workspace == nullptr) return fail(PRH_ERR_WORKSPACE, "partials_reduce: workspace too small (%zu bytes)", workspace_bytes);
+  return partials_reduce(a, b, tiles, n, out_a, out_b, mid, mid_doubles, (hipStream_t)stream);
+}
 int prh_linear_uses_operand_maxima(int rows, int k, int n) {
   const Cores c = cores_of(gemm_mode());
   return (c.mode == 3 && (nt_use_s3(c, rows, n, k) || nt_use_s3(c, rows, k, n) || tn_use_s3(c, rows, n, k))) ? 1 : 0;
@@ -1321,10 +1345,39 @@
   return prh_linear_backward_amax(x, ldx, w, dy, dx, dw, db, rows, k, n, x_amax, dy_amax_in, w_amax, 0, nullptr,
                                   workspace, workspace_bytes, device, stream);
 }
+inline bool dgrad_mask_ok(Cores c, int rows, int k, int n) {
+  return c.mode == 3 && c.core == 3 && rows > 0 && (k & 3) == 0 && (n & 3) == 0 && n <= 65536 &&
+         nt_use_s3(c, rows, k, n) && (size_t)H2_LDS <= 160 * 1024;
+}
+int prh_linear_backward_masked_ok(int rows, int k, int n) { return dgrad_mask_ok(cores_of(gemm_mode()), rows, k, n) ? 1 : 0; }
+static int linear_backward_impl(const float* x, long ldx, const float* w, const float* dy, float* dx,
+                                float* dw, float* db, int rows, int k, int n, const float* x_amax,
+                                const float* dy_amax_in, const float* w_amax, int dx_accumulate, float* dx_amax_out,
+                                const float* mask_y, float mask_scale,
+                                void* workspace, size_t workspace_bytes, int device, void* stream);
 int prh_linear_backward_amax(const float* x, long ldx, const float* w, const float* dy, float* dx,
                              float* dw, float* db, int rows, int k, int n, const float* x_amax,
                              const float* dy_amax_in, const float* w_amax, int dx_accumulate, float* dx_amax_out,
                              void* workspace, size_t workspace_bytes, int device, void* stream) {
+  return linear_backward_impl(x, ldx, w, dy, dx, dw, db, rows, k, n, x_amax, dy_amax_in, w_amax, dx_accumulate,
+                              dx_amax_out, nullptr, 1.f, workspace, workspace_bytes, device, stream);
+}
+int prh_linear_backward_masked(const float* x, long ldx, const float* w, const float* dy, float* dx,
+                               float* dw, float* db, int rows, int k, int n, const float* x_amax,
+                               const float* dy_amax_in, const float* w_amax, const float* mask_y, float mask_scale,
+                               float* dx_amax_out, void* workspace, size_t workspace_bytes, int device, void* stream) {
+  if (!mask_y || !dx || !dx_amax_out) return fail(PRH_ERR_ARG, "linear_backward_masked: mask_y, dx and dx_amax_out are required");
+  if (!dgrad_mask_ok(cores_of(gemm_mode()), rows, k, n))
+    return fail(PRH_ERR_ARG, "linear_backward_masked: no masked dgrad for rows=%d k=%d n=%d in this GEMM mode "
+                "(prh_linear_backward_masked_ok)", rows, k, n);
+  return linear_backward_impl(x, ldx, w, dy, dx, dw, db, rows, k, n, x_amax, dy_amax_in, w_amax, 0, dx_amax_out,
+                              mask_y, mask_scale, workspace, workspace_bytes, device, stream);
+}
+static int linear_backward_impl(const float* x, long ldx, const float* w, const float* dy, float* dx,
+                                float* dw, float* db, int rows, int k, int n, const float* x_amax,
+                                const float* dy_amax_in, const float* w_amax, int dx_accumulate, float* dx_amax_out,
+                                const float* mask_y, float mask_scale,
+                                void* workspace, size_t workspace_bytes, int device, void* stream) {
   if (!x || !w || !dy || rows < 0 || k <= 0 || n <= 0) return fail(PRH_ERR_ARG, "linear_backward: bad argument");
   if ((dx_accumulate || dx_amax_out != nullptr) && dx == nullptr)
     return fail(PRH_ERR_ARG, "linear_backward_amax: dx_accumulate / dx_amax_out need dx");
@@ -1340,7 +1393,7 @@
   const float* dy_amax = dy_amax_in;
   bool dx_done = false;
   const bool big16 = c.mode == 4 && rows >= 512 && (long)cdiv(rows, 256) * cdiv(k, 256) >= 16;
-  if (dx != nullptr && !big16) {
+  if (dx != nullptr && !big16 && mask_y == nullptr) {
     NTParams p; memset(&p, 0, sizeof(p));
     p.A = dy; p.lda = n; p.W = w; p.ldw = k; p.C = dx; p.ldc = k; p.M = rows; p.N = k; p.K = n;
     if (dx_accumulate) { p.flags = F_RESID; p.E1 = dx; p.lde1 = k; }
@@ -1359,8 +1412,17 @@
     p.amaxA = dy_amax;
     p.amaxW = w_amax;
     if (dx_accumulate) { p.flags = F_RESID; p.E1 = dx; p.lde1 = k; }
-    TRY((launch_nt<PRO_NONE, EPI_BIAS>(c, p, st, nullptr, dx_amax_out,
-                                      (dx_accumulate || dx_amax_out != nullptr) ? lw.dxpart : nullptr)));
+    if (mask_y != nullptr) {
+      p.E1 = mask_y; p.lde1 = k; p.drop_scale = mask_scale;
+      long tiles = 0;
+      TRY((launch_nt_core<PRO_NONE, EPI_DGRAD>(c, p, st, nullptr, lw.dxpart, &tiles)));
+      if (tiles <= 0) return fail(PRH_ERR_ARG, "linear_backward_masked: the launch did not reach the masked dgrad");
+      hipLaunchKernelGGL(absmax_final_kernel, dim3(1), dim3(256), 0, st, (const float*)lw.dxpart, (int)tiles, dx_amax_out);
+      LAUNCH_CHECK();
+    } else {
+      TRY((launch_nt<PRO_NONE, EPI_BIAS>(c, p, st, nullptr, dx_amax_out,
+                                        (dx_accumulate || dx_amax_out != nullptr) ? lw.dxpart : nullptr)));
+    }
     dy_amax = p.amaxA;
   }
   if (dw != nullptr || db != nullptr) {
@@ -1651,10 +1713,8 @@
     p.flags = F_MASK | F_STATS | F_E1_ROWVEC;
     StatInfo sig;
     TRY((launch_nt<PRO_NONE, EPI_DGRAD>(c, p, st, &sig)));
-    hipLaunchKernelGGL(partials_reduce_kernel, dim3(2), dim3(1024), 0, st, w.ws_a, w.ws_b,
-                       sig.count, 64, gr->d_gate_b1 ? gr->d_gate_b1 : gsum_a,
-                       gr->d_gate_w1 ? gr->d_gate_w1 : gsum_b);
-    LAUNCH_CHECK();
+    TRY(partials_reduce(w.ws_a, w.ws_b, sig.count, 64, gr->d_gate_b1 ? gr->d_gate_b1 : gsum_a,
+                        gr->d_gate_w1 ? gr->d_gate_w1 : gsum_b, w.stat2, (size_t)BN_SLICES * 3 * cat, st));
     if (d_ctx != nullptr) {
       hipLaunchKernelGGL(gate1_dctx_kernel, dim3(cdiv(P, 4)), dim3(256), 0, st, dU, P, 64,
                          prm->gate_w1, d_ctx, (long)C);
@@ -1886,9 +1946,8 @@
     p.flags = F_MASK | F_STATS | F_E1_ROWVEC;
     StatInfo sig;
     TRY((launch_nt_b16<PRO_NONE, EPI_DGRAD, true, false>(p, st, &sig)));
-    hipLaunchKernelGGL(partials_reduce_kernel, dim3(2), dim3(1024), 0, st, w.ws_a, w.ws_b, sig.count, 64,
-                       gr->d_gate_b1 ? gr->d_gate_b1 : w.gsum_a, gr->d_gate_w1 ? gr->d_gate_w1 : w.gsum_b);
-    LAUNCH_CHECK();
+    TRY(partials_reduce(w.ws_a, w.ws_b, sig.count, 64, gr->d_gate_b1 ? gr->d_gate_b1 : w.gsum_a,
+                        gr->d_gate_w1 ? gr->d_gate_w1 : w.gsum_b, w.stat2, (size_t)BN_SLICES * 3 * cat, st));
     if (d_ctx != nullptr) {
       hipLaunchKernelGGL(gate1_dctx_kernel, dim3(cdiv(P, 4)), dim3(256), 0, st, w.dU, P, 64, prm->gate_w1, d_ctx, (long)C);
       LAUNCH_CHECK();
diff --git a/pointnet_refine_amd/model.py b/pointnet_refine_amd/model.py
--- a/pointnet_refine_amd/model.py
+++ b/pointnet_refine_amd/model.py
@@ -166,8 +166,11 @@
             raise RuntimeError("pointnet_refine_amd: the FFN activation is ReLU (src/model.py:95), fused into the GEMM epilogue")
         pd = self.dropout.p if self.training else 0.0
         seed = int(torch.randint(0, 2 ** 31 - 1, (1,)).item()) if pd > 0.0 else 0
-        hid, hid_amax = ops.linear_with_amax(tgt, self.linear1.weight, self.linear1.bias, None, True, None, pd, seed)
-        tgt2 = ops.linear(hid, self.linear2.weight, self.linear2.bias, hid_amax)
+        if ops.producer_maxima_on(tgt.is_cuda) and tgt.dtype == torch.float32:
+            tgt2 = ops.ffn(tgt, self.linear1.weight, self.linear1.bias, self.linear2.weight, self.linear2.bias, pd, seed)
+        else:
+            hid, hid_amax = ops.linear_with_amax(tgt, self.linear1.weight, self.linear1.bias, None, True, None, pd, seed)
+            tgt2 = ops.linear(hid, self.linear2.weight, self.linear2.bias, hid_amax)
         tgt = _add_norm(tgt, tgt2, self.norm3, self.dropout3, self.training)
         return tgt
 
diff --git a/pointnet_refine_amd/ops.py b/pointnet_refine_amd/ops.py
--- a/pointnet_refine_amd/ops.py
+++ b/pointnet_refine_amd/ops.py
@@ -417,6 +417,74 @@
         LinearFn.want_y_amax = False
     amax, LinearFn.last_y_amax = LinearFn.last_y_amax, None
     return y, amax
+
+
+class FFNFn(torch.autograd.Function):
+
+    @staticmethod
+    def forward(ctx, x, w1, b1, w2, b2, dropout_p, seed, x_amax):
+        for t, nm in ((x, "input"), (w1, "weight"), (w2, "weight")):
+            _req_gpu_f32(t, nm)
+        f, k = w1.shape
+        n = w2.shape[0]
+        if x.shape[-1] != k or w2.shape[1] != f or (k | f | n) % 4:
+            raise RuntimeError(f"ffn: shapes {tuple(x.shape)}, {tuple(w1.shape)}, {tuple(w2.shape)} do not fit "
+                               "(widths multiples of 4)")
+        ctx.sinks = [_sink_view(t) for t in (w1, b1, w2, b2)]
+        x2 = x.reshape(-1, k)
+        x2 = x2 if x2.is_contiguous() else x2.contiguous()
+        w1, w2 = w1.contiguous(), w2.contiguous()
+        hid, x_amax, w1_amax, hid_amax = _linear_fwd(x2, w1, b1, None, True, x_amax, dropout_p, seed, True)
+        y, hid_amax, w2_amax, _ = _linear_fwd(hid, w2, b2, None, False, hid_amax, 0.0, 0)
+        ctx.save_for_backward(x2, hid, w1, w2)
+        ctx.amax = (x_amax, hid_amax, w1_amax, w2_amax)
+        ctx.drop_scale = 1.0 / (1.0 - dropout_p) if dropout_p > 0.0 else 1.0
+        ctx.has_bias = (b1 is not None, b2 is not None)
+        ctx.xshape = x.shape
+        return y.reshape(*x.shape[:-1], n)
+
+    @staticmethod
+    def backward(ctx, dy):
+        x2, hid, w1, w2 = ctx.saved_tensors
+        x_amax, hid_amax, w1_amax, w2_amax = ctx.amax
+        rows, dev = x2.shape[0], x2.device
+        f, k = w1.shape
+        n = w2.shape[0]
+        dy2 = dy.reshape(rows, n)
+        hint = _hint_take(dy)
+        dy_amax = hint if (hint is not None and dy2.data_ptr() == dy.data_ptr()) else None
+        if dy2.dtype != torch.float32:
+            dy2, dy_amax = dy2.float(), None
+        if not dy2.is_contiguous():
+            dy2 = dy2.contiguous()
+        ng = ctx.needs_input_grad
+        need = (ng[1], ctx.has_bias[0] and ng[2], ng[3], ctx.has_bias[1] and ng[4])
+        bufs = [_grad_buf(ctx.sinks[i], shp, dev, need[i]) for i, shp in enumerate((w1.shape, (f,), w2.shape, (n,)))]
+        lib = L.lib()
+        masked = torch.empty_like(hid)
+        m_amax = torch.empty(1, dtype=torch.float32, device=dev)
+        if lib.prh_linear_backward_masked_ok(rows, f, n):
+            ws = _ws(dev, lib.prh_linear_backward_workspace_bytes(rows, f, n))
+            L.check(lib.prh_linear_backward_masked(_p(hid), f, _p(w2), _p(dy2), _p(masked), _p(bufs[2][0]), _p(bufs[3][0]),
+                                                   rows, f, n, _p(hid_amax), _p(dy_amax), _p(w2_amax), _p(hid),
+                                                   float(ctx.drop_scale), _p(m_amax), _p(ws), ws.numel(), dev.index,
+                                                   _stream(dev)), "prh_linear_backward_masked")
+        else:
+            d_hid = torch.empty_like(hid)
+            _linear_bwd(hid, w2, dy2, hid_amax, dy_amax, w2_amax, d_hid, bufs[2][0], bufs[3][0])
+            wsm = _ws(dev, lib.prh_operand_absmax_workspace_bytes())
+            L.check(lib.prh_relu_mask_absmax(_p(d_hid), _p(hid), _p(masked), d_hid.numel(), float(ctx.drop_scale),
+                                             _p(m_amax), _p(wsm), wsm.numel(), dev.index, _stream(dev)),
+                    "prh_relu_mask_absmax")
+        dx = torch.empty_like(x2) if ng[0] else None
+        if dx is not None or bufs[0][0] is not None or bufs[1][0] is not None:
+            _linear_bwd(x2, w1, masked, x_amax, m_amax, w1_amax, dx, bufs[0][0], bufs[1][0])
+        grads = [_grad_ret(*bt) for bt in bufs]
+        return (dx.reshape(ctx.xshape) if dx is not None else None, *grads, None, None, None)
+
+
+def ffn(x, w1, b1, w2, b2, dropout_p=0.0, seed=0, x_amax=None):
+    return FFNFn.apply(x, w1, b1, w2, b2, dropout_p, seed, x_amax)
 
 
 class LinearOut16Fn(torch.autograd.Function):
```
